# Rikorose/DeepFilterNet

Hardware: NVIDIA H100
Metric: 48kHz audio-sec/sec (batched enhance) (higher is better)
Workload: dtype f32 (bf16x3 tensor-core contractions, fp32 accumulate; DSP and gates IEEE fp32)

## Files before the change

### deepfilternet_b200/csrc/dfb_common.cuh

```cuda
#pragma once
#include <cuda_runtime.h>
#include <stdint.h>

#include <atomic>
#include <cstdarg>
#include <cstdio>
#include <mutex>
#include <string>
#include <vector>

#include "../../include/dfb200.h"

namespace dfb {

extern thread_local std::string g_err;
extern std::atomic<int64_t> g_launches;

inline int fail(int code, const char *fmt, ...) {
    char buf[512];
    va_list ap;
    va_start(ap, fmt);
    vsnprintf(buf, sizeof buf, fmt, ap);
    va_end(ap);
    g_err = buf;
    return code;
}

#define DFB_CUDA(expr)                                                                          \
    do {                                                                                        \
        cudaError_t e__ = (expr);                                                               \
        if (e__ != cudaSuccess)                                                                 \
            return dfb::fail(DFB_ERR_CUDA, "%s failed: %s (%s:%d)", #expr, cudaGetErrorString(e__), \
                             __FILE__, __LINE__);                                               \
    } while (0)

#define DFB_LAUNCH_CHECK()                                                                      \
    do {                                                                                        \
        dfb::g_launches.fetch_add(1, std::memory_order_relaxed);                                \
        cudaError_t e__ = cudaGetLastError();                                                   \
        if (e__ != cudaSuccess)                                                                 \
            return dfb::fail(DFB_ERR_CUDA, "kernel launch failed: %s (%s:%d)",                  \
                             cudaGetErrorString(e__), __FILE__, __LINE__);                      \
    } while (0)

struct ProfScope {
    int slot = -1;
    cudaStream_t s;
    ProfScope(const char *name, cudaStream_t stream);
    ~ProfScope();
};
#define DFB_PROF(name, stream) dfb::ProfScope prof_scope__(name, stream)

struct PerDeviceOnce {
    std::mutex mu;
    std::atomic<unsigned long long> done{0};
    struct Guard {
        std::unique_lock<std::mutex> lk;
        PerDeviceOnce *o = nullptr;
        unsigned long long bit = 0;
        Guard() = default;
        Guard(Guard &&g) noexcept : lk(std::move(g.lk)), o(g.o), bit(g.bit) {}
        explicit operator bool() const { return lk.owns_lock(); }
        ~Guard() { if (lk.owns_lock()) o->done.fetch_or(bit, std::memory_order_release); }
    };
    Guard first() {
        int d = 0;
        cudaGetDevice(&d);
        const unsigned long long bit = 1ull << (d & 63);
        Guard g;
        if (done.load(std::memory_order_acquire) & bit) return g;
        g.lk = std::unique_lock<std::mutex>(mu);
        if (done.load(std::memory_order_acquire) & bit) { g.lk.unlock(); g.lk.release(); return g; }
        g.o = this; g.bit = bit;
        return g;
    }
};

int use_device(int device);

struct Arena {
    char *base = nullptr;
    size_t cap = 0, off = 0;
    int reserve(size_t bytes);
    void reset() { off = 0; }
    template <typename T>
    T *take(size_t n) {
        size_t b = (n * sizeof(T) + 255) & ~size_t(255);
        if (off + b > cap) return nullptr;
        T *p = reinterpret_cast<T *>(base + off);
        off += b;
        return p;
    }
    void release();
};

constexpr int kMaxErb = 64;

struct DspTables {
    const float *window;
    const float2 *tw_a_fwd;
    const float2 *tw_a_inv;
    const float2 *tw960;
    const int *erb_off;
    const float *erb_kinv;
    const unsigned char *band_of_bin;
    float wnorm;
    int fft, hop, F, E;
};

struct RaggedRow { int64_t in_off, len, out_off, out_len, Tf; };

struct ApplyParams {
    const float2 *spec;
    const float *m;
    const float *coefs;
    float *audio;
    float2 *spec_out;
    int64_t out_stride;
    int64_t out_offset;
    int64_t out_len;
    int Tf, mode, nb_df, order, lookahead;
    int spec_T, Tv, t_first;
    int mc_T;
    int frames_per_warp;
    int pf, mask_only;
    float pf_beta;
    const float *lsnr;
    float th_min, th_erb, th_df;
    const float *alpha;
    float atten_lim;
    const float *init_tail;
    float *final_tail;
    int carry;
    const RaggedRow *rows;
    int64_t w0;
    int t_emit;
};

}

struct dfb_state;
namespace dfb {
struct AnaWindow { int t_begin, nf, out_t0, Tbuf; int64_t row_stride; const RaggedRow *rows = nullptr; };
int launch_analysis(dfb_state *st, const float *d_audio, int64_t C, int64_t T, float *d_spec, float *d_erb_db,
                    cudaStream_t s, const float *d_init_mem = nullptr, const AnaWindow *w = nullptr);
int launch_feat_norm(const float *d_erb, int E, int64_t erb_stride, const float *d_spec, int Fd, int64_t spec_stride,
                     int64_t C, int64_t Tf, float alpha, const float *d_erb_state, const float *d_unit_state,
                     float *d_feat_erb, float *d_feat_spec, cudaStream_t s, int64_t Ts = 0, float *d_erb_state_out = nullptr,
                     float *d_unit_state_out = nullptr);
int launch_apply_synthesis(dfb_state *st, const ApplyParams &p, int64_t B, cudaStream_t s);
struct GruWindow { const float *h0; float *hT; int t0, Ts; };
int launch_gru_tc(cudaStream_t s, const float *xproj, const float *whh, const float *bhh, const float *res, float *hout,
                  unsigned short *hout_hi, unsigned short *hout_lo, int B, int T, long long *dbg = nullptr, int wide = 0,
                  int planes_res = 0, const GruWindow *w = nullptr, int H = 256);
int launch_gemm_bf16x3(cudaStream_t s, const void *x_hi, const void *x_lo, int64_t ldx, const void *w_hi, const void *w_lo,
                       const float *bias, float *y, int64_t ldy, int64_t M, int N, int K);
int launch_gl_bx(cudaStream_t s, const unsigned short *x_hi, const unsigned short *x_lo, int64_t ldx, const float *w_img,
                 const float *res, int64_t ldr, float *y, int64_t ldy, unsigned short *y_hi, unsigned short *y_lo, int64_t ldp,
                 int64_t M, int G, int Ig, int Hg, int act, float oscale, float ooffset);
bool gl_bx_geometry(int G, int Ig, int Hg, int *gpc_out, int *hgp_out, int *stages_out);
int launch_df_convp_tc(cudaStream_t s, const float *c0, const float *w_sw, const float *w2, const float *bias, float *coefs, int B, int T,
                       int Fd);
int launch_to_planes(cudaStream_t s, const float *x, int64_t ldx, int64_t M, int K, unsigned short *hi, unsigned short *lo);
}

struct dfb_state {
    int device, sr, fft, hop, nb_erb, min_nb_erb_freqs;
    std::vector<int64_t> erb;
    std::vector<float> window;
    void *d_tables = nullptr;
    dfb::DspTables tb{};
    dfb::Arena arena;
    cudaStream_t stream = nullptr;
    std::vector<float> analysis_mem, synthesis_mem;
};
```

### deepfilternet_b200/csrc/dfb_gl.cu

```cuda
#include <cuda.h>
#include <cuda_bf16.h>

#include <map>
#include <mutex>
#include <tuple>

#include "dfb_common.cuh"
#include "dfb_ptx.cuh"

namespace dfb {

constexpr int kGxThreads = 288, kGxMaxStages = 6, kGxBoxBytes = 128 * 128 ;
constexpr int kGxMaxChunks = 16;

struct GlBxParams {
    const unsigned short *w_img;
    const float *res; int64_t ldr;
    float *y; int64_t ldy;
    unsigned short *y_hi, *y_lo; int64_t ldp;
    int M, G, Ig, Hg, Hgp, gpc, act, stages;
    float oscale, ooffset;
};

__device__ __forceinline__ float gx_act(float x, int act) {
    if (act == 1) return fmaxf(x, 0.f);
    if (act == 2) return gt_tanh(x);
    return x;
}

__device__ __noinline__ void gl_store_chunk(const GlBxParams &p, int c, int g0, int cpg, int64_t mrow, int lane, float a00, float a01,
                                            float a02, float a03, float a10, float a11, float a12, float a13) {
    const float a[2][4] = {{a00, a01, a02, a03}, {a10, a11, a12, a13}};
    const int gl = c / cpg;
#pragma unroll
    for (int j = 0; j < 2; j++) {
        const int n = (c - gl * cpg) * 16 + j * 8 + 2 * (lane & 3);
        if (n >= p.Hg) continue;
        const int64_t col = (int64_t)(g0 + gl) * p.Hg + n;
        float2 rv[2];
#pragma unroll
        for (int h = 0; h < 2; h++) {
            const int64_t m = mrow + 8 * h;
            rv[h] = (p.res && m < p.M) ? *reinterpret_cast<const float2 *>(p.res + m * p.ldr + col) : make_float2(0.f, 0.f);
        }
#pragma unroll
        for (int h = 0; h < 2; h++) {
            const int64_t m = mrow + 8 * h;
            if (m >= p.M) continue;
            float2 x;
            x.x = gx_act(a[j][2 * h], p.act) * p.oscale + p.ooffset + rv[h].x;
            x.y = gx_act(a[j][2 * h + 1], p.act) * p.oscale + p.ooffset + rv[h].y;
            if (p.y) *reinterpret_cast<float2 *>(p.y + m * p.ldy + col) = x;
            if (p.y_hi) {
                uint32_t hv, lv;
                bf16x2_split(x.x, x.y, hv, lv);
                *reinterpret_cast<uint32_t *>(p.y_hi + m * p.ldp + col) = hv;
                *reinterpret_cast<uint32_t *>(p.y_lo + m * p.ldp + col) = lv;
            }
        }
    }
}

__global__ void __launch_bounds__(kGxThreads, 1)
k_gl_bx(const __grid_constant__ CUtensorMap tmXhi, const __grid_constant__ CUtensorMap tmXlo, const __grid_constant__ GlBxParams p) {
    extern __shared__ __align__(1024) unsigned char gx_smem_raw[];
    const uint32_t sb = (smem_u32(gx_smem_raw) + 1023u) & ~1023u;
    const int warp = threadIdx.x >> 5, lane = threadIdx.x & 31;
    const int slice = blockIdx.x, g0 = slice * p.gpc;
    const int nch = p.gpc * p.Hgp / 16;
    const int cpg = p.Hgp / 16;
    const int nboxes = p.gpc * p.Ig / 64;
    const int ntiles = (p.M + 127) / 128;
    const uint32_t gbytes = (uint32_t)p.Ig * p.Hgp * 2;
    const uint32_t wplane = gbytes * p.gpc;
    const uint32_t lbo = (uint32_t)(p.Hgp / 8) * 128u;
    const uint32_t s_x = sb;
    const uint32_t s_w = s_x + (uint32_t)p.stages * 2 * kGxBoxBytes;
    const uint32_t s_bar = (s_w + 2 * wplane + 127u) & ~127u;
    const uint32_t b_full = s_bar, b_empty = s_bar + 8 * kGxMaxStages, b_w = b_empty + 8 * kGxMaxStages;
    if (threadIdx.x == 0) {
        for (int s = 0; s < p.stages; s++) { mbar_init_a(b_full + 8 * s, 1); mbar_init_a(b_empty + 8 * s, 8); }
        mbar_init_a(b_w, 1);
        fence_barrier_init();
        mbar_expect_tx_a(b_w, 2 * wplane);
        const unsigned char *src = reinterpret_cast<const unsigned char *>(p.w_img);
        bulk_load(s_w, src + (size_t)g0 * gbytes, wplane, b_w);
        bulk_load(s_w + wplane, src + (size_t)p.G * gbytes + (size_t)g0 * gbytes, wplane, b_w);
    }
    __syncthreads();
    if (warp == 8) {
        if (lane == 0) {
            tma_prefetch_desc(&tmXhi); tma_prefetch_desc(&tmXlo);
            const int col0 = g0 * p.Ig;
            int it = 0;
            for (int tile = blockIdx.y; tile < ntiles; tile += gridDim.y)
                for (int b = 0; b < nboxes; b++, it++) {
                    const int s = it % p.stages, n = it / p.stages;
                    if (n > 0) mbar_wait_a(b_empty + 8 * s, (uint32_t)((n - 1) & 1));
                    mbar_expect_tx_a(b_full + 8 * s, 2 * kGxBoxBytes);
                    const uint32_t dst = s_x + (uint32_t)s * 2 * kGxBoxBytes;
                    asm volatile(
                        "cp.async.bulk.tensor.2d.shared::cluster.global.mbarrier::complete_tx::bytes [%0], [%1, {%2, %3}], [%4];"
                        ::"r"(dst), "l"((uint64_t)&tmXhi), "r"(col0 + b * 64), "r"(tile * 128), "r"(b_full + 8 * s) : "memory");
                    asm volatile(
                        "cp.async.bulk.tensor.2d.shared::cluster.global.mbarrier::complete_tx::bytes [%0], [%1, {%2, %3}], [%4];"
                        ::"r"(dst + kGxBoxBytes), "l"((uint64_t)&tmXlo), "r"(col0 + b * 64), "r"(tile * 128), "r"(b_full + 8 * s) : "memory");
                }
        }
        return;
    }
    const int mat = lane >> 3, rr = lane & 7;
    mbar_wait_a(b_w, 0);
    int it = 0;
    for (int tile = blockIdx.y; tile < ntiles; tile += gridDim.y) {
        float acc[kGxMaxChunks][2][4];
#pragma unroll
        for (int c = 0; c < kGxMaxChunks; c++)
#pragma unroll
            for (int e = 0; e < 8; e++) acc[c][e >> 2][e & 3] = 0.f;
        for (int b = 0; b < nboxes; b++, it++) {
            const int s = it % p.stages, n = it / p.stages;
            mbar_wait_a(b_full + 8 * s, (uint32_t)(n & 1));
            const uint32_t xs = s_x + (uint32_t)s * 2 * kGxBoxBytes;
#pragma unroll 1
            for (int k = 0; k < 4; k++) {
                const int col = b * 64 + k * 16;
                const int gl = col / p.Ig, kk = (col - gl * p.Ig) >> 4;
                uint32_t ah[4], al[4];
                const int r = warp * 16 + rr + ((mat & 1) << 3);
                ldsm_x4(xs + sw128_off(r, 2 * k + (mat >> 1)), ah);
                ldsm_x4(xs + kGxBoxBytes + sw128_off(r, 2 * k + (mat >> 1)), al);
                const uint32_t wa = s_w + (uint32_t)gl * gbytes + (uint32_t)(2 * kk + (mat & 1)) * lbo + (uint32_t)rr * 16u;
#pragma unroll
                for (int c = 0; c < kGxMaxChunks; c++) {
                    const int cg = c - gl * cpg;
                    if (c >= nch || cg < 0 || cg >= cpg) continue;
                    const uint32_t o = wa + (uint32_t)(2 * cg + (mat >> 1)) * 128u;
                    uint32_t bh[4], bl[4];
                    ldsm_x4(o, bh);
                    ldsm_x4(o + wplane, bl);
                    mma_bf16x3(acc[c][0], ah, al, bh[0], bh[1], bl[0], bl[1]);
                    mma_bf16x3(acc[c][1], ah, al, bh[2], bh[3], bl[2], bl[3]);
                }
            }
            __syncwarp();
            if (lane == 0) mbar_arrive_a(b_empty + 8 * s);
        }
        const int64_t mrow = (int64_t)tile * 128 + warp * 16 + (lane >> 2);
#pragma unroll
        for (int c = 0; c < kGxMaxChunks; c++)
            if (c < nch)
                gl_store_chunk(p, c, g0, cpg, mrow, lane, acc[c][0][0], acc[c][0][1], acc[c][0][2], acc[c][0][3], acc[c][1][0],
                               acc[c][1][1], acc[c][1][2], acc[c][1][3]);
    }
}

__global__ void __launch_bounds__(256) k_to_planes(const float *__restrict__ x, int64_t ldx, int64_t M, int K,
                                                   unsigned short *__restrict__ hi, unsigned short *__restrict__ lo) {
    const int64_t n4 = M * (K / 4);
    for (int64_t i = (int64_t)blockIdx.x * blockDim.x + threadIdx.x; i < n4; i += (int64_t)gridDim.x * blockDim.x) {
        const int64_t m = i / (K / 4);
        const int k = (int)(i - m * (K / 4)) * 4;
        const float4 v = *reinterpret_cast<const float4 *>(x + m * ldx + k);
        uint32_t h0, l0, h1, l1;
        bf16x2_split(v.x, v.y, h0, l0);
        bf16x2_split(v.z, v.w, h1, l1);
        *reinterpret_cast<uint2 *>(hi + m * K + k) = make_uint2(h0, h1);
        *reinterpret_cast<uint2 *>(lo + m * K + k) = make_uint2(l0, l1);
    }
}

typedef CUresult (*PFN_encodeTiled_gl)(CUtensorMap *, CUtensorMapDataType, cuuint32_t, void *, const cuuint64_t *,
                                       const cuuint64_t *, const cuuint32_t *, const cuuint32_t *, CUtensorMapInterleave,
                                       CUtensorMapSwizzle, CUtensorMapL2promotion, CUtensorMapFloatOOBfill);

int cached_map_bf16(CUtensorMap *out, const void *base, int64_t rows, int64_t cols, int64_t ld, int box_rows) {
    static std::mutex mu;
    static std::map<std::tuple<int, const void *, int64_t, int64_t, int64_t, int>, CUtensorMap> cache;
    static PFN_encodeTiled_gl enc = nullptr;
    int dev = 0;
    cudaGetDevice(&dev);
    std::lock_guard<std::mutex> g(mu);
    auto key = std::make_tuple(dev, base, rows, cols, ld, box_rows);
    auto it = cache.find(key);
    if (it != cache.end()) { *out = it->second; return DFB_OK; }
    if (!enc) {
        void *fp = nullptr;
        cudaDriverEntryPointQueryResult q;
        if (cudaGetDriverEntryPoint("cuTensorMapEncodeTiled", &fp, cudaEnableDefault, &q) != cudaSuccess || q != cudaDriverEntryPointSuccess)
            return fail(DFB_ERR_CUDA, "cuTensorMapEncodeTiled entry point not available");
        enc = (PFN_encodeTiled_gl)fp;
    }
    cuuint64_t dims[2] = {(cuuint64_t)cols, (cuuint64_t)rows};
    cuuint64_t strides[1] = {(cuuint64_t)ld * 2};
    cuuint32_t box[2] = {64u, (cuuint32_t)box_rows};
    cuuint32_t estr[2] = {1, 1};
    CUtensorMap m;
    CUresult r = enc(&m, CU_TENSOR_MAP_DATA_TYPE_BFLOAT16, 2, (void *)base, dims, strides, box, estr, CU_TENSOR_MAP_INTERLEAVE_NONE,
                     CU_TENSOR_MAP_SWIZZLE_128B, CU_TENSOR_MAP_L2_PROMOTION_L2_128B, CU_TENSOR_MAP_FLOAT_OOB_FILL_NONE);
    if (r != CUDA_SUCCESS) return fail(DFB_ERR_CUDA, "cuTensorMapEncodeTiled (bf16) failed (%d)", (int)r);
    if (cache.size() > 4096) cache.clear();
    cache[key] = m;
    *out = m;
    return DFB_OK;
}

int cached_map_f32_sw128(CUtensorMap *out, const void *base, int64_t rows, int64_t cols, int64_t ld, int box_rows) {
    static std::mutex mu;
    static std::map<std::tuple<int, const void *, int64_t, int64_t, int64_t, int>, CUtensorMap> cache;
    static PFN_encodeTiled_gl enc = nullptr;
    int dev = 0;
    cudaGetDevice(&dev);
    std::lock_guard<std::mutex> g(mu);
    auto key = std::make_tuple(dev, base, rows, cols, ld, box_rows);
    auto it = cache.find(key);
    if (it != cache.end()) { *out = it->second; return DFB_OK; }
    if (!enc) {
        void *fp = nullptr;
        cudaDriverEntryPointQueryResult q;
        if (cudaGetDriverEntryPoint("cuTensorMapEncodeTiled", &fp, cudaEnableDefault, &q) != cudaSuccess || q != cudaDriverEntryPointSuccess)
            return fail(DFB_ERR_CUDA, "cuTensorMapEncodeTiled entry point not available");
        enc = (PFN_encodeTiled_gl)fp;
    }
    cuuint64_t dims[2] = {(cuuint64_t)cols, (cuuint64_t)rows};
    cuuint64_t strides[1] = {(cuuint64_t)ld * 4};
    cuuint32_t box[2] = {32u, (cuuint32_t)box_rows};
    cuuint32_t estr[2] = {1, 1};
    CUtensorMap m;
    CUresult r = enc(&m, CU_TENSOR_MAP_DATA_TYPE_FLOAT32, 2, (void *)base, dims, strides, box, estr, CU_TENSOR_MAP_INTERLEAVE_NONE,
                     CU_TENSOR_MAP_SWIZZLE_128B, CU_TENSOR_MAP_L2_PROMOTION_L2_128B, CU_TENSOR_MAP_FLOAT_OOB_FILL_NONE);
    if (r != CUDA_SUCCESS) return fail(DFB_ERR_CUDA, "cuTensorMapEncodeTiled (fp32) failed (%d)", (int)r);
    if (cache.size() > 4096) cache.clear();
    cache[key] = m;
    *out = m;
    return DFB_OK;
}

int launch_to_planes(cudaStream_t s, const float *x, int64_t ldx, int64_t M, int K, unsigned short *hi, unsigned short *lo) {
    if (K % 4 || ldx % 4) return fail(DFB_ERR_UNSUPPORTED, "to_planes: K = %d", K);
    int dev = 0, sms = 0;
    DFB_CUDA(cudaGetDevice(&dev));
    DFB_CUDA(cudaDeviceGetAttribute(&sms, cudaDevAttrMultiProcessorCount, dev));
    DFB_PROF("k_to_planes", s);
    k_to_planes<<<sms * 8, 256, 0, s>>>(x, ldx, M, K, hi, lo);
    DFB_LAUNCH_CHECK();
    return DFB_OK;
}

bool gl_bx_geometry(int G, int Ig, int Hg, int *gpc_out, int *hgp_out, int *stages_out) {
    if (Ig % 16 || Hg % 4 || G < 1) return false;
    const int Hgp = (Hg + 15) / 16 * 16;
    if (Hgp > 256) return false;
    int best = 0;
    for (int gpc = 1; gpc <= G; gpc++) {
        if (G % gpc) continue;
        if (gpc * Hgp > 256 || (gpc * Hgp) % 32) continue;
        if ((gpc * Ig) % 64) continue;
        if ((size_t)gpc * Ig * Hgp * 4 > 100 * 1024) continue;
        best = gpc;
    }
    if (!best) return false;
    const int w = best * Ig * Hgp * 4;
    int stages = (227 * 1024 - 2048 - w - 256) / (2 * kGxBoxBytes);
    if (stages > kGxMaxStages) stages = kGxMaxStages;
    if (stages < 2) return false;
    *gpc_out = best; *hgp_out = Hgp; *stages_out = stages;
    return true;
}

int launch_gl_bx(cudaStream_t s, const unsigned short *x_hi, const unsigned short *x_lo, int64_t ldx, const float *w_img,
                 const float *res, int64_t ldr, float *y, int64_t ldy, unsigned short *y_hi, unsigned short *y_lo, int64_t ldp,
                 int64_t M, int G, int Ig, int Hg, int act, float oscale, float ooffset) {
    int gpc = 0, Hgp = 0, stages = 0;
    if (!gl_bx_geometry(G, Ig, Hg, &gpc, &Hgp, &stages) || M <= 0 || M > 0x7fffffff || (ldx % 8) || ((uintptr_t)x_hi & 15) ||
        ((uintptr_t)x_lo & 15) || (y && ((ldy % 4) || ((uintptr_t)y & 15))) || (res && ((ldr % 4) || ((uintptr_t)res & 15))) ||
        (y_hi && ((ldp % 4) || ((uintptr_t)y_hi & 7) || ((uintptr_t)y_lo & 7))))
        return DFB_ERR_UNSUPPORTED;
    CUtensorMap mh, ml;
    int rc;
    if ((rc = cached_map_bf16(&mh, x_hi, M, (int64_t)G * Ig, ldx, 128)) || (rc = cached_map_bf16(&ml, x_lo, M, (int64_t)G * Ig, ldx, 128)))
        return rc;
    GlBxParams p{reinterpret_cast<const unsigned short *>(w_img), res, ldr, y, ldy, y_hi, y_lo, ldp,
                 (int)M, G, Ig, Hg, Hgp, gpc, act, stages, oscale, ooffset};
    const int smem = 1024 + stages * 2 * kGxBoxBytes + gpc * Ig * Hgp * 4 + 128 + 256;
    static PerDeviceOnce attr_once;
    if (auto once_guard = attr_once.first())
        DFB_CUDA(cudaFuncSetAttribute(k_gl_bx, cudaFuncAttributeMaxDynamicSharedMemorySize, 227 * 1024));
    int dev = 0, sms = 0;
    DFB_CUDA(cudaGetDevice(&dev));
    DFB_CUDA(cudaDeviceGetAttribute(&sms, cudaDevAttrMultiProcessorCount, dev));
    const int slices = G / gpc, ntiles = (int)((M + 127) / 128);
    int groups = sms / slices;
    if (groups < 1) groups = 1;
    if (groups > ntiles) groups = ntiles;
    DFB_PROF("k_gl_bx", s);
    k_gl_bx<<<dim3((unsigned)slices, (unsigned)groups), kGxThreads, smem, s>>>(mh, ml, p);
    DFB_LAUNCH_CHECK();
    return DFB_OK;
}

}
```

### deepfilternet_b200/csrc/dfb_model.cu

```cuda
#include <cooperative_groups.h>
#include <cuda_bf16.h>

#include <algorithm>
#include <cmath>
#include <cstring>
#include <functional>
#include <map>
#include <string>

#include "dfb_common.cuh"
#include "dfb_dwpw.cuh"
#include "dfb_ptx.cuh"

namespace cg = cooperative_groups;

namespace dfb {


enum Act { ACT_NONE = 0, ACT_RELU = 1, ACT_TANH = 2, ACT_SIGMOID = 3 };

__device__ __forceinline__ float act_apply(float x, int act) {
    switch (act) {
        case ACT_RELU: return fmaxf(x, 0.f);
        case ACT_TANH: return tanhf(x);
// ... 736 lines not shown
                                int n_tensors, const int64_t *erb_widths) {
    if (!out || !cfg || !tensors) return fail(DFB_ERR_INVALID, "null argument");
    *out = nullptr;
    if (cfg->conv_ch != kCh) return fail(DFB_ERR_UNSUPPORTED, "conv_ch = %d (built kernels: 64)", cfg->conv_ch);
    if (cfg->model_kind < 1 || cfg->model_kind > 3) return fail(DFB_ERR_UNSUPPORTED, "model_kind %d", cfg->model_kind);
    if (cfg->model_kind == 1 && (cfg->emb_hidden != cfg->df_hidden || cfg->emb_hidden != cfg->nb_erb / 4 * kCh || cfg->conv_kt != 2 ||
                                 cfg->inp_kt != 2 || cfg->df_order != 5))
        return fail(DFB_ERR_UNSUPPORTED, "DeepFilterNet v1: only the shipped topology is built (hidden = conv_ch * nb_erb / 4, kt 2, order 5)");
    if (cfg->conv_kt < 1 || cfg->conv_kt > 2 || cfg->inp_kt < 1 || cfg->inp_kt > 3)
        return fail(DFB_ERR_UNSUPPORTED, "conv kernel time taps (%d, %d) unsupported", cfg->conv_kt, cfg->inp_kt);
    if ((cfg->emb_hidden != 256 && cfg->emb_hidden != 512) || (cfg->df_hidden != 256 && cfg->df_hidden != 512))
        return fail(DFB_ERR_UNSUPPORTED, "GRU hidden sizes (%d, %d): built kernels cover 256 and 512", cfg->emb_hidden,
                    cfg->df_hidden);
    if (cfg->nb_erb % 8 || cfg->nb_erb > 64 || cfg->nb_df % 8 || cfg->nb_df > 128 || 2 * cfg->df_order > kMaxO2)
        return fail(DFB_ERR_UNSUPPORTED, "nb_erb / nb_df / df_order outside the built kernels");
    int rc = use_device(device);
    if (rc) return rc;
    dfb_model *m = new dfb_model();
    m->device = device;
    m->cfg = *cfg;
    if (erb_widths) m->erb_widths.assign(erb_widths, erb_widths + cfg->nb_erb);
    if (const char *e = getenv("DFB_DEVICE_CHUNKS")) m->dev_chunks = atoi(e) > 0 ? atoi(e) : 0;
    if (const char *e = getenv("DFB_HOST_CHUNKS")) m->host_chunks = atoi(e) > 0 ? atoi(e) : 1;
    if (const char *e = getenv("DFB_LANES")) m->n_lanes = atoi(e) == 1 ? 1 : 2;
    if (const char *e = getenv("DFB_MAX_WORKSPACE_MB")) {
        const long long mb = atoll(e);
        if (mb > 0) m->max_workspace = (size_t)mb << 20;
    }
    size_t total = 0;
    for (int i = 0; i < n_tensors; i++) total += ((size_t)tensors[i].numel * 4 + 255) & ~size_t(255);
    if (cudaMalloc(&m->slab, total + 256) != cudaSuccess) {
        delete m;
        return fail(DFB_ERR_OOM, "cudaMalloc(%zu) for weights failed", total);
    }
    size_t off = 0;
    std::vector<float> tmp;
    for (int i = 0; i < n_tensors; i++) {
        const dfb_tensor &tt = tensors[i];
        if (!tt.name || !tt.data || tt.numel <= 0) { dfb_model_free(m); return fail(DFB_ERR_INVALID, "bad tensor %d", i); }
        float *dst = (float *)((char *)m->slab + off);
        if (cudaMemcpy(dst, tt.data, (size_t)tt.numel * 4, cudaMemcpyHostToDevice) != cudaSuccess) {
            dfb_model_free(m);
            return fail(DFB_ERR_CUDA, "weight upload failed");
        }
        m->t[tt.name] = {dst, tt.numel};
        off += ((size_t)tt.numel * 4 + 255) & ~size_t(255);
    }
    int prio_least = 0, prio_greatest = 0;
    cudaDeviceGetStreamPriorityRange(&prio_least, &prio_greatest);
    int prio_enc = prio_greatest + 1;
    if (prio_enc > prio_least) prio_enc = prio_least;
    bool ok = cudaStreamCreateWithFlags(&m->stream, cudaStreamNonBlocking) == cudaSuccess &&
              cudaStreamCreateWithFlags(&m->h2d, cudaStreamNonBlocking) == cudaSuccess &&
              cudaStreamCreateWithFlags(&m->d2h, cudaStreamNonBlocking) == cudaSuccess;
    for (auto &L : m->lanes) {
        ok = ok && cudaStreamCreateWithPriority(&L.main, cudaStreamNonBlocking, prio_enc) == cudaSuccess &&
             cudaStreamCreateWithPriority(&L.hi, cudaStreamNonBlocking, prio_enc) == cudaSuccess &&
             cudaStreamCreateWithPriority(&L.aux, cudaStreamNonBlocking, prio_enc) == cudaSuccess &&
             cudaStreamCreateWithPriority(&L.dhi, cudaStreamNonBlocking, prio_greatest) == cudaSuccess &&
             cudaStreamCreateWithPriority(&L.daux, cudaStreamNonBlocking, prio_greatest) == cudaSuccess &&
             cudaStreamCreateWithPriority(&L.low, cudaStreamNonBlocking, prio_least) == cudaSuccess;
        for (cudaEvent_t *e : {&L.ev_fork, &L.ev_join, &L.ev_fork_enc, &L.ev_join_enc, &L.ev_in, &L.ev_out, &L.ev_c0, &L.ev_convp,
                               &L.ev_skip, &L.ev_done})
            ok = ok && cudaEventCreateWithFlags(e, cudaEventDisableTiming) == cudaSuccess;
    }
    if (!ok) {
        dfb_model_free(m);
        return fail(DFB_ERR_CUDA, "stream creation failed");
    }
    *out = m;
    return DFB_OK;
}

extern "C" void dfb_model_free(dfb_model *m) {
    if (!m) return;
    cudaSetDevice(m->device);
    m->arena.release();
    m->arena1.release();
    m->aux_arena.release();
    if (m->h2d) cudaStreamDestroy(m->h2d);
    if (m->d2h) cudaStreamDestroy(m->d2h);
    if (m->slab) cudaFree(m->slab);
    if (m->stream) cudaStreamDestroy(m->stream);
    for (auto &L : m->lanes) {
        for (cudaStream_t st : {L.main, L.hi, L.aux, L.dhi, L.daux, L.low})
            if (st) cudaStreamDestroy(st);
        for (cudaEvent_t e : {L.ev_fork, L.ev_join, L.ev_fork_enc, L.ev_join_enc, L.ev_in, L.ev_out, L.ev_c0, L.ev_convp, L.ev_skip, L.ev_done})
            if (e) cudaEventDestroy(e);
    }
    delete m;
}

extern "C" int dfb_debug_gru_timing(dfb_model *m, int steps, long long *h_out) {
    if (!m) return fail(DFB_ERR_INVALID, "null model");
    cudaSetDevice(m->device);
    if (h_out && m->gru_dbg) {
        DFB_CUDA(cudaDeviceSynchronize());
        DFB_CUDA(cudaMemcpy(h_out, m->gru_dbg, sizeof(long long) * 8 * steps, cudaMemcpyDeviceToHost));
    }
    if (m->gru_dbg) { cudaFree(m->gru_dbg); m->gru_dbg = nullptr; }
    if (steps > 0 && !h_out) {
        DFB_CUDA(cudaMalloc(&m->gru_dbg, sizeof(long long) * 8 * steps));
        DFB_CUDA(cudaMemset(m->gru_dbg, 0, sizeof(long long) * 8 * steps));
    }
    return DFB_OK;
}

extern "C" int dfb_model_set_precision(dfb_model *m, int mode) {
    if (!m || mode < 0 || mode > 15 || (mode & 1)) return fail(DFB_ERR_INVALID, "precision mode out of range (bit 0 is reserved)");
    m->gru_tc = (mode >> 1) & 1;
    m->proj_tc = (mode >> 2) & 1;
    m->conv_tc = (mode >> 3) & 1;
    return DFB_OK;
}

extern "C" int64_t dfb_model_debug_fetch(dfb_model *m, const char *name, float *h_out, int64_t max_numel) {
    if (!m || !name || !h_out) return fail(DFB_ERR_INVALID, "null argument");
    auto it = m->dbg.find(name);
    if (it == m->dbg.end()) return fail(DFB_ERR_INVALID, "no activation named '%s'", name);
    int64_t n = it->second.second < max_numel ? it->second.second : max_numel;
    cudaSetDevice(m->device);
    if (cudaDeviceSynchronize() != cudaSuccess ||
        cudaMemcpy(h_out, it->second.first, (size_t)n * 4, cudaMemcpyDeviceToHost) != cudaSuccess)
        return fail(DFB_ERR_CUDA, "debug fetch failed: %s", cudaGetErrorString(cudaGetLastError()));
    return n;
}

extern "C" int64_t dfb_model_workspace_bytes(const dfb_model *m) { return m ? (int64_t)m->arena.cap : 0; }

namespace {

int run_gl(cudaStream_t s, const float *x, int64_t ldx, const float *w, const float *bias, const float *res,
           int64_t ldr, float *y, int64_t ldy, int64_t M, int G, int I, int Hh, int act, float oscale = 1.f,
           float ooffset = 0.f, unsigned short *y_hi = nullptr, unsigned short *y_lo = nullptr) {
    GlParams p{x, ldx, w, bias, res, ldr, y, ldy, M, G, I / G, Hh / G, act, oscale, ooffset, y_hi, y_lo};
    if ((p.Ig % 4) || (ldx % 4)) return fail(DFB_ERR_UNSUPPORTED, "grouped linear: K not a multiple of 4");
    if (G > 1 && (p.Hg % 4)) return fail(DFB_ERR_UNSUPPORTED, "grouped linear: group width %d not a multiple of 4", p.Hg);
    int tiles = (p.Hg + kGlBN - 1) / kGlBN;
    int gpc = (p.Hg < kGlBN && kGlBN % p.Hg == 0) ? (kGlBN / p.Hg < G ? kGlBN / p.Hg : G) : 1;
    dim3 grid((unsigned)((M + kGlBM - 1) / kGlBM), (unsigned)(((G + gpc - 1) / gpc) * tiles));
    static const bool detail = getenv("DFB_PROF_DETAIL") && atoi(getenv("DFB_PROF_DETAIL"));
    char name[64];
    if (detail) snprintf(name, sizeof name, "k_grouped_linear[%dx%d/%d]", I, Hh, G);
    else snprintf(name, sizeof name, "%s", p.G == 1 && p.bias && p.Hg >= 512 ? "k_grouped_linear[gru_proj]" : "k_grouped_linear");
    DFB_PROF(name, s);
    k_grouped_linear<<<grid, 256, 0, s>>>(p);
    DFB_LAUNCH_CHECK();
    return DFB_OK;
}

template <int H, int C>
int launch_gru_t(cudaStream_t s, const GruParams &p, int ngroups) {
    constexpr int smem = (2 * kGruMaxBc * (H + 4) + 3 * (H / C) * (kGruMaxBc + 1)) * 4;
    static PerDeviceOnce attr_once;
    if (auto once_guard = attr_once.first()) {
        if (C > 8) DFB_CUDA(cudaFuncSetAttribute(k_gru<H, C>, cudaFuncAttributeNonPortableClusterSizeAllowed, 1));
        DFB_CUDA(cudaFuncSetAttribute(k_gru<H, C>, cudaFuncAttributeMaxDynamicSharedMemorySize, smem));
    }
    cudaLaunchConfig_t cfg{};
    cfg.gridDim = dim3((unsigned)(ngroups * C));
    cfg.blockDim = dim3(kGruThreads);
    cfg.dynamicSmemBytes = smem;
    cfg.stream = s;
    cudaLaunchAttribute at[1];
    at[0].id = cudaLaunchAttributeClusterDimension;
    at[0].val.clusterDim.x = C; at[0].val.clusterDim.y = 1; at[0].val.clusterDim.z = 1;
    cfg.attrs = at; cfg.numAttrs = 1;
    GruParams pp = p;
    DFB_PROF("k_gru", s);
    DFB_CUDA(cudaLaunchKernelEx(&cfg, k_gru<H, C>, pp));
    g_launches.fetch_add(1, std::memory_order_relaxed);
    return DFB_OK;
}

int pick_bc(int B, int max_clusters) {
    int bc = (B + max_clusters - 1) / max_clusters;
    bc = ((bc + kGruSB - 1) / kGruSB) * kGruSB;
    if (bc < kGruSB) bc = kGruSB;
    if (bc > kGruMaxBc) bc = kGruMaxBc;
    return bc;
}

int run_gru(dfb_model *m, cudaStream_t s, const char *name, int layers, int H, const float *x, int in_dim,
            const float *res_last, float *y, float *xproj, float *tmp_h, int B, int T,
            unsigned short *x_hi = nullptr, unsigned short *x_lo = nullptr, unsigned short *pl_hi = nullptr,
            unsigned short *pl_lo = nullptr, int wide = 0, unsigned short *out_hi = nullptr, unsigned short *out_lo = nullptr,
            bool *out_planes_ok = nullptr, const GruChunk *ck = nullptr) {
    if (out_planes_ok) *out_planes_ok = false;
    const int t0 = ck ? ck->t0 : 0, Tn = T - t0;
    const int64_t M = (int64_t)B * T;
    const float *cur_in = x;
    int cur_dim = in_dim;
    const bool tc_gru = m->gru_tc && (H == 256 || H == 512);
    const bool tc_proj = m->proj_tc && tc_gru && x_hi && pl_hi && cur_dim % 64 == 0;
    const unsigned short *cur_hi = x_hi, *cur_lo = x_lo;
    for (int l = 0; l < layers; l++) {
        std::string base = std::string(name) + ".l" + std::to_string(l);
        const float *w_ih_t, *w_hh, *b_ih, *b_hh;
        int rc;
        if ((rc = need(m, (base + ".w_ih_t").c_str(), (int64_t)3 * H * cur_dim, &w_ih_t))) return rc;
        if ((rc = need(m, (base + ".w_hh").c_str(), (int64_t)3 * H * H, &w_hh))) return rc;
        if ((rc = need(m, (base + ".b_ih").c_str(), 3 * H, &b_ih))) return rc;
        if ((rc = need(m, (base + ".b_hh").c_str(), 3 * H, &b_hh))) return rc;
        if (tc_proj) {
            const float *w_hi, *w_lo;
            if ((rc = need(m, (base + ".w_ih_hi").c_str(), (int64_t)3 * H * cur_dim / 2, &w_hi)) ||
                (rc = need(m, (base + ".w_ih_lo").c_str(), (int64_t)3 * H * cur_dim / 2, &w_lo)))
                return rc;
            rc = launch_gemm_bf16x3(s, cur_hi, cur_lo, cur_dim, w_hi, w_lo, b_ih, xproj, 3 * H, M, 3 * H, cur_dim);
        } else {
            rc = run_gl(s, cur_in, cur_dim, w_ih_t, b_ih, nullptr, 0, xproj, 3 * H, M, 1, cur_dim, 3 * H, ACT_NONE);
        }
        if (rc) return rc;
        float *dst = (l == layers - 1) ? y : tmp_h;
        float *hs = ck && ck->h ? ck->h + (int64_t)l * ck->Bs * H : nullptr;
        GruWindow gw{ck && ck->have_state ? hs : nullptr, hs, t0, T};
        GruParams p{xproj, w_hh, b_hh, (l == layers - 1) ? res_last : nullptr, dst, B, Tn, 0, m->gru_dbg, gw.h0, gw.hT, t0, T};
        if (tc_gru) {
            const bool last = l == layers - 1;
            const bool planes = last ? out_hi != nullptr : tc_proj;
            rc = launch_gru_tc(s, xproj, w_hh, b_hh, last ? res_last : nullptr, dst, planes ? (last ? out_hi : pl_hi) : nullptr,
                               planes ? (last ? out_lo : pl_lo) : nullptr, B, Tn, m->gru_dbg, wide, last ? 1 : 0, &gw, H);
            if (last && planes && out_planes_ok) *out_planes_ok = true;
            cur_hi = pl_hi; cur_lo = pl_lo;
        } else if (H == 256) {
            int sms = 0;
            DFB_CUDA(cudaDeviceGetAttribute(&sms, cudaDevAttrMultiProcessorCount, m->device));
            p.Bc = pick_bc(B, sms / 4);
            rc = launch_gru_t<256, 4>(s, p, (B + p.Bc - 1) / p.Bc);
        } else {
            p.Bc = pick_bc(B, 8);
            rc = launch_gru_t<512, 16>(s, p, (B + p.Bc - 1) / p.Bc);
        }
        if (rc) return rc;
        cur_in = dst;
        cur_dim = H;
    }
    return DFB_OK;
}

}
namespace dfb {
template <int MODE>
int launch_dwpw_tc(cudaStream_t s, DwPwParams p, const float *w_sw, int B);
}
namespace {

template <int MODE>
int run_dwpw(cudaStream_t s, DwPwParams p, int B, const float *w_sw = nullptr) {
    if (w_sw) return launch_dwpw_tc<MODE>(s, p, w_sw, B);
    static PerDeviceOnce attr_once;
    const int smem = (kCh * kCh + 128 * kLdA) * 4;
    if (auto once_guard = attr_once.first()) {
        DFB_CUDA(cudaFuncSetAttribute(k_dwpw<MODE>, cudaFuncAttributeMaxDynamicSharedMemorySize, smem));
    }
    p.NF = 128 / p.Fout;
    if (p.NF < 1) p.NF = 1;
    if (p.NF * p.Fout > 128 || (p.NF * p.Fout) % 4) return fail(DFB_ERR_UNSUPPORTED, "dwpw tile: Fout = %d", p.Fout);
    dim3 grid((unsigned)((p.T + p.NF - 1) / p.NF), (unsigned)B);
    DFB_PROF(MODE == DW_DF0 ? "k_dwpw[df_conv0]" : "k_dwpw", s);
    k_dwpw<MODE><<<grid, 256, smem, s>>>(p);
    DFB_LAUNCH_CHECK();
    return DFB_OK;
}

}

struct FwdBufs {
    float *e0, *e1, *e2, *e3, *c0, *c1, *emb_in, *emb, *g_a, *g_b, *g_h, *xproj, *dec_emb, *d3, *d2, *d1, *dfc;
    unsigned short *ga_hi, *ga_lo, *gh_hi, *gh_lo;
    float *g_a2, *g_h2, *xproj2, *dfskip;
    unsigned short *ga2_hi, *ga2_lo, *gh2_hi, *gh2_lo;
    unsigned short *c1_hi, *c1_lo, *embin_hi, *embin_lo, *gb_hi, *gb_lo, *emb_hi, *emb_lo, *dfc_hi, *dfc_lo;
};

struct FwdBufsV1 {
    float *e0, *e1, *e2, *e3, *c0, *c1, *c1g, *cemb, *emb, *xproj, *xproj2, *y[3], *embo, *dec_old, *dec, *p3, *p2, *p1, *p0, *d3, *d2, *d1,
        *z[2], *dfc;
    unsigned short *emb_hi, *emb_lo, *y_hi[3], *y_lo[3], *embo_hi, *embo_lo, *z_hi[2], *z_lo[2], *dfc_hi, *dfc_lo, *scr_hi, *scr_lo;
};
static size_t fwd_plan_v1(const dfb_model_config &c, size_t M, Arena *a, FwdBufsV1 *f) {
    const int E = c.nb_erb, Fd = c.nb_df, H = c.emb_hidden;
    size_t bytes = 0;
    auto take = [&](size_t n) -> float * {
        bytes += (n * 4 + 255) & ~size_t(255);
        return a ? a->take<float>(n) : nullptr;
    };
    auto take16 = [&](size_t n) { return reinterpret_cast<unsigned short *>(take((n + 1) / 2)); };
    FwdBufsV1 t{};
    t.e0 = take(M * E * kCh); t.e1 = take(M * (E / 2) * kCh); t.e2 = take(M * (E / 4) * kCh); t.e3 = take(M * (E / 4) * kCh);
    t.c0 = take(M * Fd * kCh); t.c1 = take(M * (Fd / 2) * kCh); t.c1g = take(M * (Fd / 2) * kCh);
    t.cemb = take(M * H); t.emb = take(M * H); t.xproj = take(M * 3 * H); t.xproj2 = take(M * 3 * H);
    for (int i = 0; i < 3; i++) { t.y[i] = take(M * H); t.y_hi[i] = take16(M * H); t.y_lo[i] = take16(M * H); }
    for (int i = 0; i < 2; i++) { t.z[i] = take(M * H); t.z_hi[i] = take16(M * H); t.z_lo[i] = take16(M * H); }
    t.embo = take(M * H); t.dec_old = take(M * H); t.dec = take(M * H); t.dfc = take(M * H);
    t.p3 = take(M * (E / 4) * kCh); t.p2 = take(M * (E / 4) * kCh); t.p1 = take(M * (E / 2) * kCh); t.p0 = take(M * E * kCh);
    t.d3 = take(M * (E / 4) * kCh); t.d2 = take(M * (E / 2) * kCh); t.d1 = take(M * E * kCh);
    t.emb_hi = take16(M * H); t.emb_lo = take16(M * H); t.embo_hi = take16(M * H); t.embo_lo = take16(M * H);
    t.dfc_hi = take16(M * H); t.dfc_lo = take16(M * H); t.scr_hi = take16(M * H); t.scr_lo = take16(M * H);
    if (f) *f = t;
    return bytes + 4096;
}

static size_t fwd_plan(const dfb_model_config &c, size_t M, Arena *a, FwdBufs *f) {
    if (c.model_kind == 1 && !a) return fwd_plan_v1(c, M, nullptr, nullptr);
    const int E = c.nb_erb, Fd = c.nb_df, H = c.emb_hidden, Hd = c.df_hidden;
    const int ED = E / 4 * kCh;
    const int emb_in_dim = c.enc_concat ? 2 * ED : ED;
    const int emb_dim = c.model_kind == 2 ? H : ED;
    const int Hmax = H > Hd ? H : Hd;
    size_t bytes = 0;
    auto take = [&](size_t n) -> float * {
        bytes += (n * 4 + 255) & ~size_t(255);
        return a ? a->take<float>(n) : nullptr;
    };
    FwdBufs t{};
    t.e0 = take(M * E * kCh); t.e1 = take(M * (E / 2) * kCh); t.e2 = take(M * (E / 4) * kCh);
    t.emb_in = take(M * emb_in_dim);
    t.e3 = c.enc_concat ? t.emb_in : take(M * ED);
    t.c0 = take(M * Fd * kCh); t.c1 = take(M * (Fd / 2) * kCh);
    t.emb = take(M * emb_dim);
    t.g_a = take(M * Hmax); t.g_b = take(M * Hmax); t.g_h = take(M * Hmax);
    t.xproj = take(M * 3 * Hmax);
    t.dec_emb = take(M * ED); t.d3 = take(M * ED); t.d2 = take(M * (E / 2) * kCh);
    t.d1 = take(M * E * kCh); t.dfc = take(M * Hmax);
    t.ga_hi = reinterpret_cast<unsigned short *>(take(M * Hmax / 2)); t.ga_lo = reinterpret_cast<unsigned short *>(take(M * Hmax / 2));
    t.gh_hi = reinterpret_cast<unsigned short *>(take(M * Hmax / 2)); t.gh_lo = reinterpret_cast<unsigned short *>(take(M * Hmax / 2));
    t.g_a2 = take(M * Hmax); t.g_h2 = take(M * Hmax); t.xproj2 = take(M * 3 * Hmax); t.dfskip = take(M * Hmax);
    t.ga2_hi = reinterpret_cast<unsigned short *>(take(M * Hmax / 2)); t.ga2_lo = reinterpret_cast<unsigned short *>(take(M * Hmax / 2));
    t.gh2_hi = reinterpret_cast<unsigned short *>(take(M * Hmax / 2)); t.gh2_lo = reinterpret_cast<unsigned short *>(take(M * Hmax / 2));
    auto take16 = [&](size_t n) { return reinterpret_cast<unsigned short *>(take((n + 1) / 2)); };
    t.c1_hi = take16(M * (Fd / 2) * kCh); t.c1_lo = take16(M * (Fd / 2) * kCh);
    t.embin_hi = take16(M * emb_in_dim); t.embin_lo = take16(M * emb_in_dim);
    t.gb_hi = take16(M * Hmax); t.gb_lo = take16(M * Hmax);
    t.emb_hi = take16(M * emb_dim); t.emb_lo = take16(M * emb_dim);
    t.dfc_hi = take16(M * Hmax); t.dfc_lo = take16(M * Hmax);
    if (f) *f = t;
    return bytes + 4096;
}

struct ChunkCtx {
    int Rc;
    int Tsx, Tx;
    float *h_enc, *h_erb, *h_df;
    bool have_state;
    float *dec_tail;
    int dec_tail_n;
    int lane;
    cudaEvent_t wait_dec;
    int Bs;
    const RaggedRow *rows;
    int64_t W0;
};
constexpr int kHalo = 8;

static int forward_impl(dfb_model *m, Arena &arena, const float *d_feat_erb, const float *d_feat_spec, int B, int T,
                        float *d_m, float *d_coefs, float *d_lsnr, float *d_alpha, cudaStream_t s, ChunkCtx *cx = nullptr);

extern "C" int dfb_model_forward(dfb_model *m, const float *d_feat_erb, const float *d_feat_spec, int64_t B64,
                                 int64_t T64, float *d_m, float *d_coefs, float *d_lsnr, float *d_alpha,
                                 void *stream) {
    if (!m || !d_feat_erb || !d_feat_spec || !d_m || !d_coefs) return fail(DFB_ERR_INVALID, "null argument");
    if (B64 <= 0 || T64 <= 0) return DFB_OK;
    if (B64 > 65535) return fail(DFB_ERR_INVALID, "more than 65535 streams per call");
    DFB_CUDA(cudaSetDevice(m->device));
    int rc = m->arena.reserve(fwd_plan(m->cfg, (size_t)B64 * T64, nullptr, nullptr));
    if (rc) return rc;
    m->arena.reset();
    rc = forward_impl(m, m->arena, d_feat_erb, d_feat_spec, (int)B64, (int)T64, d_m, d_coefs, d_lsnr, d_alpha,
                      (cudaStream_t)stream);
    m->arena.reset();
    return rc;
}

static int forward_body(dfb_model *m, Arena &arena, const float *d_feat_erb, const float *d_feat_spec, int B, int T,
                        float *d_m, float *d_coefs, float *d_lsnr, float *d_alpha, cudaStream_t s_in, ChunkCtx *cx);

static int forward_v1(dfb_model *m, Arena &arena, const float *d_feat_erb, const float *d_feat_spec, int B, int T,
                      float *d_m, float *d_coefs, float *d_lsnr, float *d_alpha, cudaStream_t s_in, ChunkCtx *cx);

static int forward_impl(dfb_model *m, Arena &arena, const float *d_feat_erb, const float *d_feat_spec, int B, int T,
                        float *d_m, float *d_coefs, float *d_lsnr, float *d_alpha, cudaStream_t s_in, ChunkCtx *cx) {
    const int rc = m->cfg.model_kind == 1
        ? forward_v1(m, arena, d_feat_erb, d_feat_spec, B, T, d_m, d_coefs, d_lsnr, d_alpha, s_in, cx)
        : forward_body(m, arena, d_feat_erb, d_feat_spec, B, T, d_m, d_coefs, d_lsnr, d_alpha, s_in, cx);
    if (rc) cudaDeviceSynchronize();
    return rc;
}

static int forward_body(dfb_model *m, Arena &arena, const float *d_feat_erb, const float *d_feat_spec, int B, int T,
                        float *d_m, float *d_coefs, float *d_lsnr, float *d_alpha, cudaStream_t s_in, ChunkCtx *cx) {
    const dfb_model_config &c = m->cfg;
    const int Tsx = cx ? cx->Tsx : T, Tx = cx ? cx->Tx : T;
    GruChunk ck_enc{cx ? cx->h_enc : nullptr, cx && cx->have_state, cx ? cx->Rc : 0, cx ? cx->Bs : B};
    GruChunk ck_erb{cx ? cx->h_erb : nullptr, cx && cx->have_state, cx ? cx->Rc : 0, cx ? cx->Bs : B};
    GruChunk ck_df{cx ? cx->h_df : nullptr, cx && cx->have_state, cx ? cx->Rc : 0, cx ? cx->Bs : B};
    const RaggedRow *rows = cx ? cx->rows : nullptr;
    const int64_t W0 = cx ? cx->W0 : 0;
    static const bool serial = getenv("DFB_SERIAL") && atoi(getenv("DFB_SERIAL"));
    dfb_model::Lane &L = m->lanes[cx ? cx->lane : 0];
    cudaStream_t s = serial ? s_in : L.hi;
    cudaStream_t sl = serial ? s_in : L.low;
    if (!serial) {
        DFB_CUDA(cudaEventRecord(L.ev_in, s_in));
        DFB_CUDA(cudaStreamWaitEvent(s, L.ev_in, 0));
    }
    auto finish = [&]() -> int {
        DFB_CUDA(cudaStreamWaitEvent(s, L.ev_join, 0));
        if (!serial) {
            DFB_CUDA(cudaEventRecord(L.ev_out, s));
            DFB_CUDA(cudaStreamWaitEvent(s_in, L.ev_out, 0));
        }
        return DFB_OK;
    };
    const int64_t M = (int64_t)B * T;
    const int E = c.nb_erb, Fd = c.nb_df, H = c.emb_hidden, Hd = c.df_hidden;
    const int ED = E / 4 * kCh;
    const int emb_in_dim = c.enc_concat ? 2 * ED : ED;
    const int emb_dim = c.model_kind == 2 ? H : ED;
    int rc;
    FwdBufs f{};
    fwd_plan(c, (size_t)M, &arena, &f);
    if (!f.gh2_lo || !f.dfskip || !f.dfc_lo) return fail(DFB_ERR_OOM, "forward workspace exhausted for %lld frames", (long long)M);
    m->dbg.clear();
    m->dbg["e0"] = {f.e0, M * E * kCh}; m->dbg["e1"] = {f.e1, M * (E / 2) * kCh}; m->dbg["e2"] = {f.e2, M * (E / 4) * kCh};
    m->dbg["e3"] = {f.e3, c.enc_concat ? M * emb_in_dim : M * ED}; m->dbg["c0"] = {f.c0, M * Fd * kCh};
    m->dbg["c1"] = {f.c1, M * (Fd / 2) * kCh}; m->dbg["emb_in"] = {f.emb_in, M * emb_in_dim};
    m->dbg["emb"] = {f.emb, M * emb_dim}; m->dbg["dec_emb"] = {f.dec_emb, M * ED}; m->dbg["d3"] = {f.d3, M * ED};
    m->dbg["d2"] = {f.d2, M * (E / 2) * kCh}; m->dbg["d1"] = {f.d1, M * E * kCh}; m->dbg["dfc"] = {f.dfc, M * Hd};
    m->dbg["g_a"] = {f.g_a, M * (H > Hd ? H : Hd)}; m->dbg["g_b"] = {f.g_b, M * (H > Hd ? H : Hd)};
    m->dbg["xproj"] = {f.xproj, M * 3 * (H > Hd ? H : Hd)};
    const int64_t e3_fs = c.enc_concat ? 2 * ED : ED;
    struct Pl { unsigned short *hi, *lo; int64_t ld; bool ok; };
    Pl pl_c1{f.c1_hi, f.c1_lo, (int64_t)Fd / 2 * kCh, false}, pl_embin{f.embin_hi, f.embin_lo, emb_in_dim, false},
       pl_gb{f.gb_hi, f.gb_lo, H, false}, pl_emb{f.emb_hi, f.emb_lo, emb_dim, false}, pl_dfc{f.dfc_hi, f.dfc_lo, Hd, false},
       pl_ga{f.ga_hi, f.ga_lo, H, false}, pl_ga2{f.ga2_hi, f.ga2_lo, Hd, false};
    const bool gl_tc = m->conv_tc != 0;
    auto ensure_planes = [&](cudaStream_t st, const float *x, int64_t ldx, int K, Pl &pl) -> int {
        if (pl.ok) return DFB_OK;
        if (pl.ld != K) return fail(DFB_ERR_INVALID, "plane pitch mismatch");
        int r = launch_to_planes(st, x, ldx, M, K, pl.hi, pl.lo);
        if (!r) pl.ok = true;
        return r;
    };
    auto gl = [&](cudaStream_t st, const char *wname, const float *x, int64_t ldx, Pl *xin, int G, int I, int Hh, int act,
                  const float *res, int64_t ldr, float *y, int64_t ldy, Pl *yout, int64_t ycol = 0) -> int {
        const float *w;
        int r;
        if ((r = need(m, wname, (int64_t)I * Hh / G, &w))) return r;
        unsigned short *yh = yout ? yout->hi + ycol : nullptr, *yl = yout ? yout->lo + ycol : nullptr;
        const std::string bx = std::string(wname) + "_bx";
        int gpc, hgp, stages;
        if (gl_tc && xin && m->get(bx) && gl_bx_geometry(G, I / G, Hh / G, &gpc, &hgp, &stages)) {
            if ((r = ensure_planes(st, x, ldx, I, *xin))) return r;
            r = launch_gl_bx(st, xin->hi, xin->lo, xin->ld, m->get(bx), res, ldr, y, ldy, yh, yl, yout ? yout->ld : 0, M, G, I / G,
                             Hh / G, act, 1.f, 0.f);
            if (r != DFB_ERR_UNSUPPORTED) {
                if (!r && yout && (ycol == 0 || true)) yout->ok = true;
                return r;
            }
        }
        const bool ffma_planes = yout && yout->ld == ldy;
        r = run_gl(st, x, ldx, w, nullptr, res, ldr, y, ldy, M, G, I, Hh, act, 1.f, 0.f, ffma_planes ? yh : nullptr, ffma_planes ? yl : nullptr);
        if (!r && yout) yout->ok = ffma_planes;
        return r;
    };

    {
        const float *w, *bb;
        if ((rc = need(m, "enc.erb_conv0.w", c.inp_kt * 3 * kCh, &w)) || (rc = need(m, "enc.erb_conv0.b", kCh, &bb))) return rc;
        dim3 grid((unsigned)((T + kInFrames - 1) / kInFrames), (unsigned)B);
        int smem = (kInFrames + c.inp_kt - 1) * (E + 2) * 4;
        DFB_PROF("k_conv_in[erb_conv0]", s);
        k_conv_in<1><<<grid, 256, smem, s>>>(d_feat_erb, w, bb, f.e0, T, E, c.inp_kt, c.conv_lookahead, Tsx, Tx, 0, rows, W0);
        DFB_LAUNCH_CHECK();
    }
    const float *pw_sw = nullptr;
    auto blk = [&](const char *name, DwPwParams &p) -> int {
        std::string n(name);
        int r;
        if ((r = need(m, (n + ".dw").c_str(), -1, &p.dw)) || (r = need(m, (n + ".pw").c_str(), kCh * kCh, &p.pw)) ||
            (r = need(m, (n + ".b").c_str(), kCh, &p.bias)))
            return r;
        pw_sw = nullptr;
        if (m->conv_tc && (r = need(m, (n + ".pw_sw").c_str(), kCh * kCh, &pw_sw))) return r;
        return DFB_OK;
    };
    cudaStream_t sa = serial ? s : L.aux;
    DFB_CUDA(cudaEventRecord(L.ev_fork_enc, s));
    DFB_CUDA(cudaStreamWaitEvent(sa, L.ev_fork_enc, 0));
    auto mk = [&](const float *in, int Fin, int64_t in_fs, float *out, int Fout, int64_t out_fs, int kt) {
        DwPwParams p{};
        p.in = in; p.Fin = Fin; p.in_fs = in_fs; p.out = out; p.Fout = Fout; p.out_fs = out_fs; p.kt = kt; p.T = T;
        p.lookahead = 0;
        return p;
    };
    {
        DwPwParams p{};
        {
            const float *w, *bb;
            if ((rc = need(m, "enc.df_conv0.w", c.inp_kt * 3 * 2 * kCh, &w)) || (rc = need(m, "enc.df_conv0.b", kCh, &bb))) return rc;
            dim3 grid((unsigned)((T + kInFrames - 1) / kInFrames), (unsigned)B);
            int smem = (kInFrames + c.inp_kt - 1) * (Fd + 2) * 2 * 4;
            DFB_PROF("k_conv_in[df_conv0]", sa);
            k_conv_in<2><<<grid, 256, smem, sa>>>(d_feat_spec, w, bb, f.c0, T, Fd, c.inp_kt, c.conv_lookahead, Tsx, Tx, 0, rows, W0);
            DFB_LAUNCH_CHECK();
            DFB_CUDA(cudaEventRecord(L.ev_c0, sa));
        }
        p = mk(f.c0, Fd, (int64_t)Fd * kCh, f.c1, Fd / 2, (int64_t)Fd / 2 * kCh, c.conv_kt);
        if ((rc = blk("enc.df_conv1", p))) return rc;
        if (pw_sw && gl_tc) {
            p.out = nullptr; p.out_hi = pl_c1.hi; p.out_lo = pl_c1.lo; pl_c1.ok = true;
            m->dbg.erase("c1");
        }
        if ((rc = run_dwpw<DW_S2>(sa, p, B, pw_sw))) return rc;
        DFB_CUDA(cudaEventRecord(L.ev_join_enc, sa));
        DFB_CUDA(cudaStreamWaitEvent(sl, L.ev_c0, 0));
        const int O2 = 2 * c.df_order;
        const float *w1, *w2, *bb;
        if ((rc = need(m, "df_dec.df_convp.w1", (int64_t)c.df_pathway_kt * O2 * (kCh / 2), &w1)) ||
            (rc = need(m, "df_dec.df_convp.w2", O2 * O2, &w2)) || (rc = need(m, "df_dec.df_convp.b", O2, &bb)))
            return rc;
        if (c.df_order != 5 || c.df_pathway_kt != 5)
            return fail(DFB_ERR_UNSUPPORTED, "df_order %d / df_pathway_kernel_size_t %d (built kernels: 5, 5)", c.df_order,
                        c.df_pathway_kt);
        if (Fd % 2) return fail(DFB_ERR_UNSUPPORTED, "df pathway conv: odd nb_df");
        dim3 grid((unsigned)((Fd + 2 * kCpWarps - 1) / (2 * kCpWarps)), (unsigned)((T + kCpChunk - 1) / kCpChunk), (unsigned)B);
        static const bool convp_ffma = getenv("DFB_CONVP_FFMA") && atoi(getenv("DFB_CONVP_FFMA"));
        const float *w_sw = (m->conv_tc && !convp_ffma) ? m->get("df_dec.df_convp.w_sw") : nullptr;
        if (w_sw) {
            if ((rc = launch_df_convp_tc(sl, f.c0, w_sw, w2, bb, d_coefs, B, T, Fd))) return rc;
        } else {
            DFB_PROF("k_df_convp", sl);
            const int smem = kCpWarps * kCpSlots * (512 + 8);
            k_df_convp<5, 5, 3><<<grid, 32 * kCpWarps, smem, sl>>>(f.c0, w1, w2, bb, d_coefs, T, Fd);
            DFB_LAUNCH_CHECK();
        }
        DFB_CUDA(cudaEventRecord(L.ev_convp, sl));
    }
    {
        DwPwParams p = mk(f.e0, E, (int64_t)E * kCh, f.e1, E / 2, (int64_t)E / 2 * kCh, c.conv_kt);
        if ((rc = blk("enc.erb_conv1", p)) || (rc = run_dwpw<DW_S2>(s, p, B, pw_sw))) return rc;
        p = mk(f.e1, E / 2, (int64_t)E / 2 * kCh, f.e2, E / 4, (int64_t)E / 4 * kCh, c.conv_kt);
        if ((rc = blk("enc.erb_conv2", p)) || (rc = run_dwpw<DW_S2>(s, p, B, pw_sw))) return rc;
        p = mk(f.e2, E / 4, (int64_t)E / 4 * kCh, f.e3, E / 4, e3_fs, c.conv_kt);
        if ((rc = blk("enc.erb_conv3", p))) return rc;
        if (pw_sw && gl_tc && c.enc_concat) { p.out_hi = pl_embin.hi; p.out_lo = pl_embin.lo; }
        if ((rc = run_dwpw<DW_S1>(s, p, B, pw_sw))) return rc;

    }
    DFB_CUDA(cudaStreamWaitEvent(s, L.ev_join_enc, 0));
    {
        const int I = Fd / 2 * kCh;
        const bool e3_planes = pw_sw && gl_tc && c.enc_concat;
        if (c.enc_concat) {
            rc = gl(s, "enc.df_fc_emb.gl", f.c1, I, &pl_c1, c.g_df_fc_emb, I, ED, ACT_RELU, nullptr, 0, f.emb_in + ED, emb_in_dim,
                    &pl_embin, ED);
            pl_embin.ok = pl_embin.ok && e3_planes;
        } else {
            rc = gl(s, "enc.df_fc_emb.gl", f.c1, I, &pl_c1, c.g_df_fc_emb, I, ED, ACT_RELU, f.e3, ED, f.emb_in, emb_in_dim, &pl_embin);
        }
        if (rc) return rc;
    }
    {
        if ((rc = gl(s, "enc.emb_gru.in.gl", f.emb_in, emb_in_dim, &pl_embin, c.g_enc_in, emb_in_dim, H, ACT_RELU, nullptr, 0, f.g_a, H,
                     &pl_ga))) return rc;
        float *gout = c.g_enc_out ? f.g_b : f.emb;
        Pl &pl_gout = c.g_enc_out ? pl_gb : pl_emb;
        if ((rc = run_gru(m, s, "enc.emb_gru", c.enc_gru_layers, H, f.g_a, H, nullptr, gout, f.xproj, f.g_h, B, T, f.ga_hi, f.ga_lo,
                          f.gh_hi, f.gh_lo, 0, gl_tc ? pl_gout.hi : nullptr, gl_tc ? pl_gout.lo : nullptr, &pl_gout.ok, cx ? &ck_enc : nullptr))) return rc;
        if (c.g_enc_out) {
            if ((rc = gl(s, "enc.emb_gru.out.gl", f.g_b, H, &pl_gb, c.g_enc_out, H, ED, ACT_RELU, nullptr, 0, f.emb, emb_dim, &pl_emb)))
                return rc;
        }
        if (gl_tc && (rc = ensure_planes(s, f.emb, emb_dim, emb_dim, pl_emb))) return rc;
        if (d_lsnr) {
            const float *lw, *lb;
            if ((rc = need(m, "enc.lsnr.w", emb_dim, &lw)) || (rc = need(m, "enc.lsnr.b", 1, &lb))) return rc;
            if ((rc = run_gl(s, f.emb, emb_dim, lw, lb, nullptr, 0, d_lsnr, 1, M, 1, emb_dim, 1, ACT_SIGMOID, c.lsnr_scale, c.lsnr_offset))) return rc;
        }
    }
    DFB_CUDA(cudaEventRecord(L.ev_fork, s));
    if (!serial) { s = L.dhi; sa = L.daux; DFB_CUDA(cudaStreamWaitEvent(s, L.ev_fork, 0)); }
    DFB_CUDA(cudaStreamWaitEvent(sa, L.ev_fork, 0));
    if (cx && cx->wait_dec) {
        DFB_CUDA(cudaStreamWaitEvent(s, cx->wait_dec, 0));
        DFB_CUDA(cudaStreamWaitEvent(sa, cx->wait_dec, 0));
    }
    static const char *wide_env = getenv("DFB_WIDE_BRANCH");
    const int wide_df = !wide_env || !strcmp(wide_env, "df") || !strcmp(wide_env, "both");
    const int wide_erb = wide_env && (!strcmp(wide_env, "erb") || !strcmp(wide_env, "both"));
    const bool early_skip = c.g_df_skip && c.model_kind != 2;
    if (early_skip) {
        if ((rc = gl(s, "df_dec.df_skip.gl", f.emb, emb_dim, &pl_emb, c.g_df_skip, emb_dim, Hd, ACT_NONE, nullptr, 0, f.dfskip, Hd, nullptr)))
            return rc;
        DFB_CUDA(cudaEventRecord(L.ev_skip, s));
    }
    {
        cudaStream_t s = sa;
        if ((rc = gl(s, "df_dec.df_gru.in.gl", f.emb, emb_dim, &pl_emb, c.g_df_in, emb_dim, Hd, ACT_RELU, nullptr, 0, f.g_a2, Hd, &pl_ga2)))
            return rc;
        const float *res = c.model_kind == 2 ? f.g_a2 : (early_skip ? f.dfskip : nullptr);
        if (early_skip) DFB_CUDA(cudaStreamWaitEvent(s, L.ev_skip, 0));
        if ((rc = run_gru(m, s, "df_dec.df_gru", c.df_gru_layers, Hd, f.g_a2, Hd, res, f.dfc, f.xproj2, f.g_h2, B, T, f.ga2_hi, f.ga2_lo,
                          f.gh2_hi, f.gh2_lo, wide_df, gl_tc ? pl_dfc.hi : nullptr, gl_tc ? pl_dfc.lo : nullptr, &pl_dfc.ok, cx ? &ck_df : nullptr))) return rc;
        if (c.g_df_skip && !early_skip) {
            if ((rc = gl(s, "df_dec.df_skip.gl", f.emb, emb_dim, &pl_emb, c.g_df_skip, emb_dim, Hd, ACT_NONE, f.dfc, Hd, f.dfc, Hd, nullptr)))
                return rc;
            pl_dfc.ok = false;
        }
        if (d_alpha && c.model_kind == 2) {
            const float *aw, *ab;
            if ((rc = need(m, "df_dec.df_fc_a.w", Hd, &aw)) || (rc = need(m, "df_dec.df_fc_a.b", 1, &ab))) return rc;
            if ((rc = run_gl(s, f.dfc, Hd, aw, ab, nullptr, 0, d_alpha, 1, M, 1, Hd, 1, ACT_SIGMOID))) return rc;
        }
        const int O2 = 2 * c.df_order;
        DFB_CUDA(cudaStreamWaitEvent(s, L.ev_convp, 0));
        if ((rc = gl(s, "df_dec.df_out.gl", f.dfc, Hd, &pl_dfc, c.g_df_out, Hd, Fd * O2, ACT_TANH, d_coefs, (int64_t)Fd * O2, d_coefs,
                     (int64_t)Fd * O2, nullptr))) return rc;
    }
    DFB_CUDA(cudaEventRecord(L.ev_join, sa));
    {
        if ((rc = gl(s, "erb_dec.emb_gru.in.gl", f.emb, emb_dim, &pl_emb, c.g_erb_in, emb_dim, H, ACT_RELU, nullptr, 0, f.g_a, H, &pl_ga)))
            return rc;
        const float *res = c.model_kind == 2 ? f.g_a : nullptr;
        pl_gb.ok = false;
        if ((rc = run_gru(m, s, "erb_dec.emb_gru", c.erb_gru_layers, H, f.g_a, H, res, f.g_b, f.xproj, f.g_h, B, T, f.ga_hi, f.ga_lo,
                          f.gh_hi, f.gh_lo, wide_erb, gl_tc ? pl_gb.hi : nullptr, gl_tc ? pl_gb.lo : nullptr, &pl_gb.ok, cx ? &ck_erb : nullptr))) return rc;
        if ((rc = gl(s, "erb_dec.emb_gru.out.gl", f.g_b, H, &pl_gb, c.g_erb_out, H, ED, ACT_RELU, nullptr, 0, f.dec_emb, ED, nullptr)))
            return rc;
        if (cx && cx->dec_tail && c.conv_kt > 1) {
            const size_t fb = sizeof(float) * ED;
            const int nl = cx->Rc < cx->dec_tail_n ? cx->Rc : cx->dec_tail_n;
            if (cx->have_state && nl > 0)
                DFB_CUDA(cudaMemcpy2DAsync(f.dec_emb + (size_t)(cx->Rc - nl) * ED, fb * T, cx->dec_tail + (size_t)(kHalo - nl) * ED,
                                           fb * kHalo, fb * nl, B, cudaMemcpyDeviceToDevice, s));
            const int ns = T < kHalo ? T : kHalo;
            DFB_CUDA(cudaMemcpy2DAsync(cx->dec_tail + (size_t)(kHalo - ns) * ED, fb * kHalo, f.dec_emb + (size_t)(T - ns) * ED, fb * T,
                                       fb * ns, B, cudaMemcpyDeviceToDevice, s));
            cx->dec_tail_n = ns;
        }
        auto path = [&](DwPwParams &p, const char *pn, const float *pt, int64_t pfs) -> int {
            std::string n(pn);
            p.path = pt; p.path_fs = pfs;
            int r;
            if ((r = need(m, (n + ".s").c_str(), kCh, &p.ps)) || (r = need(m, (n + ".b").c_str(), kCh, &p.pb))) return r;
            return DFB_OK;
        };
        DwPwParams p = mk(f.dec_emb, E / 4, ED, f.d3, E / 4, ED, c.conv_kt);
        if ((rc = blk("erb_dec.convt3", p)) || (rc = path(p, "erb_dec.conv3p", f.e3, e3_fs)) || (rc = run_dwpw<DW_S1>(s, p, B, pw_sw))) return rc;
        p = mk(f.d3, E / 4, ED, f.d2, E / 2, (int64_t)E / 2 * kCh, 1);
        if ((rc = blk("erb_dec.convt2", p)) || (rc = path(p, "erb_dec.conv2p", f.e2, (int64_t)E / 4 * kCh)) || (rc = run_dwpw<DW_T2>(s, p, B, pw_sw))) return rc;
        const float *ps, *pb, *w, *bb;
        if ((rc = need(m, "erb_dec.conv0p.s", kCh, &ps)) || (rc = need(m, "erb_dec.conv0p.b", kCh, &pb)) ||
            (rc = need(m, "erb_dec.conv0_out.w", c.conv_kt * 3 * kCh, &w)) || (rc = need(m, "erb_dec.conv0_out.b", 1, &bb)))
            return rc;
        p = mk(f.d2, E / 2, (int64_t)E / 2 * kCh, f.d1, E, (int64_t)E * kCh, 1);
        if ((rc = blk("erb_dec.convt1", p)) || (rc = path(p, "erb_dec.conv1p", f.e1, (int64_t)E / 2 * kCh))) return rc;
        const bool fused_mask = pw_sw && c.conv_kt == 1 && 128 % E == 0;
        if (fused_mask) {
            p.mk_e0 = f.e0; p.mk_ps = ps; p.mk_pb = pb; p.mk_w = w; p.mk_bias = bb; p.mk_out = d_m;
            p.out = nullptr;
            m->dbg.erase("d1");
        }
        if ((rc = run_dwpw<DW_T2>(s, p, B, pw_sw))) return rc;
        if (fused_mask) return finish();
        static PerDeviceOnce attr_once;
        int smem = (kMaskWarps * 2 * (E + 2) * kMaskLd + c.conv_kt * 3 * kCh) * 4;
        if (auto once_guard = attr_once.first()) {
            DFB_CUDA(cudaFuncSetAttribute(k_mask_out, cudaFuncAttributeMaxDynamicSharedMemorySize,
                                          (kMaskWarps * 2 * (64 + 2) * kMaskLd + 2 * 3 * kCh) * 4));
        }
        int per_cta = kMaskWarps * kMaskChunk;
        dim3 grid((unsigned)((T + per_cta - 1) / per_cta), (unsigned)B);
        DFB_PROF("k_mask_out", s);
        k_mask_out<<<grid, 32 * kMaskWarps, smem, s>>>(f.e0, f.d1, ps, pb, w, bb, d_m, T, E, c.conv_kt);
        DFB_LAUNCH_CHECK();
    }
    return finish();
}

static int forward_v1(dfb_model *m, Arena &arena, const float *d_feat_erb, const float *d_feat_spec, int B, int T,
                      float *d_m, float *d_coefs, float *d_lsnr, float *d_alpha, cudaStream_t s_in, ChunkCtx *cx) {
    const dfb_model_config &c = m->cfg;
    if (cx && (cx->Rc != 0 || cx->have_state)) return fail(DFB_ERR_UNSUPPORTED, "DeepFilterNet v1 runs as one window per signal");
    const int Tsx = cx ? cx->Tsx : T, Tx = cx ? cx->Tx : T;
    static const bool serial = getenv("DFB_SERIAL") && atoi(getenv("DFB_SERIAL"));
    dfb_model::Lane &L = m->lanes[cx ? cx->lane : 0];
    cudaStream_t s = serial ? s_in : L.hi, sa = serial ? s_in : L.aux;
    if (!serial) {
        DFB_CUDA(cudaEventRecord(L.ev_in, s_in));
        DFB_CUDA(cudaStreamWaitEvent(s, L.ev_in, 0));
    }
    const int64_t M = (int64_t)B * T;
    const int E = c.nb_erb, Fd = c.nb_df, H = c.emb_hidden, O2 = 2 * c.df_order, kt = c.conv_kt;
    int rc;
    FwdBufsV1 f{};
    fwd_plan_v1(c, (size_t)M, &arena, &f);
    if (!f.scr_lo) return fail(DFB_ERR_OOM, "forward workspace exhausted for %lld frames", (long long)M);
    m->dbg.clear();
    m->dbg["e0"] = {f.e0, M * E * kCh}; m->dbg["e1"] = {f.e1, M * (E / 2) * kCh}; m->dbg["e2"] = {f.e2, M * (E / 4) * kCh};
    m->dbg["e3"] = {f.e3, M * (E / 4) * kCh}; m->dbg["c0"] = {f.c0, M * Fd * kCh}; m->dbg["c1"] = {f.c1, M * (Fd / 2) * kCh};
    m->dbg["cemb"] = {f.cemb, M * H}; m->dbg["emb_in"] = {f.emb, M * H}; m->dbg["emb"] = {f.embo, M * H};
    m->dbg["dec_emb"] = {f.dec, M * H}; m->dbg["d3"] = {f.d3, M * (E / 4) * kCh}; m->dbg["d2"] = {f.d2, M * (E / 2) * kCh};
    m->dbg["d1"] = {f.d1, M * E * kCh}; m->dbg["dfc"] = {f.dfc, M * H}; m->dbg["y0"] = {f.y[0], M * H};
    const bool tc = m->conv_tc != 0;
    const float *ones, *zeros;
    if ((rc = need(m, "v1.ones", kCh, &ones)) || (rc = need(m, "v1.zeros", kCh, &zeros))) return rc;
    auto table = [&](const char *name, int n, const int **out) -> int {
        const float *t;
        int r = need(m, name, n, &t);
        *out = reinterpret_cast<const int *>(t);
        return r;
    };
    const int *idx_c1, *idx_e3, *idx_shuf, *idx_id, *idx_dec, *idx_gshuf;
    if ((rc = table("v1.idx_c1", Fd / 2 * kCh, &idx_c1)) || (rc = table("v1.idx_e3", H, &idx_e3)) || (rc = table("v1.idx_shuf", H, &idx_shuf)) ||
        (rc = table("v1.idx_id", H, &idx_id)) || (rc = table("v1.idx_dec", H, &idx_dec)) || (rc = table("v1.idx_gshuf", H, &idx_gshuf)))
        return rc;
    auto gather = [&](cudaStream_t st, int n, const float *const *src, const int64_t *ld, const int *const *idx, int K, int relu,
                      float *out, unsigned short *hi, unsigned short *lo) -> int {
        GatherParams g{};
        for (int i = 0; i < n; i++) { g.src[i] = src[i]; g.ld[i] = ld[i]; g.idx[i] = idx[i]; }
        g.n = n; g.out = out; g.ldo = K; g.hi = hi; g.lo = lo; g.ldp = K; g.K = K; g.relu = relu;
        DFB_PROF("k_gather_sum", st);
        k_gather_sum<<<(unsigned)M, 256, 0, st>>>(g);
        DFB_LAUNCH_CHECK();
        return DFB_OK;
    };
    auto block = [&](cudaStream_t st, const char *name, int mode, const float *in, int Fin, float *out, int Fout, int bkt, int la,
                     const float *path) -> int {
        DwPwParams p{};
        std::string n(name);
        int r;
        if ((r = need(m, (n + ".dw").c_str(), bkt * 3 * kCh, &p.dw)) || (r = need(m, (n + ".pw").c_str(), kCh * kCh, &p.pw)) ||
            (r = need(m, (n + ".b").c_str(), kCh, &p.bias)))
            return r;
        p.in = in; p.Fin = Fin; p.in_fs = (int64_t)Fin * kCh; p.out = out; p.Fout = Fout; p.out_fs = (int64_t)Fout * kCh; p.kt = bkt; p.T = T;
        p.lookahead = la;
        if (path) { p.path = path; p.path_fs = p.in_fs; p.ps = ones; p.pb = zeros; }
        const float *w_sw = nullptr;
        if (tc && la == 0 && !(mode == DW_T2 && bkt != 1) && (r = need(m, (n + ".pw_sw").c_str(), kCh * kCh, &w_sw))) return r;
        if (mode == DW_S1) return run_dwpw<DW_S1>(st, p, B, w_sw);
        if (mode == DW_S2) return run_dwpw<DW_S2>(st, p, B, w_sw);
        return run_dwpw<DW_T2>(st, p, B, w_sw);
    };
    DFB_CUDA(cudaEventRecord(L.ev_fork_enc, s));
    DFB_CUDA(cudaStreamWaitEvent(sa, L.ev_fork_enc, 0));
    {
        const float *w, *bb;
        if ((rc = need(m, "enc.erb_conv0.w", c.inp_kt * 3 * kCh, &w)) || (rc = need(m, "enc.erb_conv0.b", kCh, &bb))) return rc;
        dim3 grid((unsigned)((T + kInFrames - 1) / kInFrames), (unsigned)B);
        const int la = c.conv_lookahead > 0 ? 1 : 0;
        {
            DFB_PROF("k_conv_in[erb_conv0]", s);
            k_conv_in<1><<<grid, 256, (kInFrames + c.inp_kt - 1) * (E + 2) * 4, s>>>(d_feat_erb, w, bb, f.e0, T, E, c.inp_kt, la, Tsx, Tx, -la,
                                                                                      nullptr, 0);
            DFB_LAUNCH_CHECK();
        }
        if ((rc = need(m, "enc.df_conv0.w", c.inp_kt * 3 * 2 * kCh, &w)) || (rc = need(m, "enc.df_conv0.b", kCh, &bb))) return rc;
        DFB_PROF("k_conv_in[df_conv0]", sa);
        k_conv_in<2><<<grid, 256, (kInFrames + c.inp_kt - 1) * (Fd + 2) * 2 * 4, sa>>>(d_feat_spec, w, bb, f.c0, T, Fd, c.inp_kt, c.conv_lookahead,
                                                                                      Tsx, Tx, -c.conv_lookahead, nullptr, 0);
        DFB_LAUNCH_CHECK();
    }
    if ((rc = block(sa, "enc.df_conv1", DW_S2, f.c0, Fd, f.c1, Fd / 2, kt, 0, nullptr))) return rc;
    {
        const float *src[1] = {f.c1}; const int64_t ld[1] = {(int64_t)Fd / 2 * kCh}; const int *ix[1] = {idx_c1};
        if ((rc = gather(sa, 1, src, ld, ix, Fd / 2 * kCh, 0, f.c1g, nullptr, nullptr))) return rc;
        const float *w, *bb;
        const int I = Fd / 2 * kCh;
        if ((rc = need(m, "enc.df_fc_emb.gl", (int64_t)I * H / c.g_df_fc_emb, &w)) || (rc = need(m, "enc.df_fc_emb.bias", H, &bb))) return rc;
        if ((rc = run_gl(sa, f.c1g, I, w, bb, nullptr, 0, f.cemb, H, M, c.g_df_fc_emb, I, H, ACT_NONE))) return rc;
    }
    DFB_CUDA(cudaEventRecord(L.ev_join_enc, sa));
    if ((rc = block(s, "enc.erb_conv1", DW_S2, f.e0, E, f.e1, E / 2, kt, c.conv_lookahead > 1 ? 1 : 0, nullptr)) ||
        (rc = block(s, "enc.erb_conv2", DW_S2, f.e1, E / 2, f.e2, E / 4, kt, c.conv_lookahead > 2 ? 1 : 0, nullptr)) ||
        (rc = block(s, "enc.erb_conv3", DW_S1, f.e2, E / 4, f.e3, E / 4, kt, 0, nullptr)))
        return rc;
    DFB_CUDA(cudaStreamWaitEvent(s, L.ev_join_enc, 0));
    {
        const float *src[2] = {f.e3, f.cemb}; const int64_t ld[2] = {H, H}; const int *ix[2] = {idx_e3, idx_shuf};
        if ((rc = gather(s, 2, src, ld, ix, H, 0, f.emb, f.emb_hi, f.emb_lo))) return rc;
    }
    auto ggru = [&](cudaStream_t st, const char *name, int layers, const float *x, unsigned short *x_hi, unsigned short *x_lo, float **y,
                    unsigned short **y_hi, unsigned short **y_lo, float *xproj, float *hbase, float *out, unsigned short *out_hi,
                    unsigned short *out_lo) -> int {
        const float *cur = x;
        unsigned short *ch = x_hi, *cl = x_lo;
        for (int l = 0; l < layers; l++) {
            const std::string nm = std::string(name) + ".g" + std::to_string(l);
            GruChunk ck{hbase ? hbase + (int64_t)l * B * H : nullptr, false, 0, B};
            bool ok = false;
            int r = run_gru(m, st, nm.c_str(), 1, H, cur, H, nullptr, y[l], xproj, nullptr, B, T, ch, cl, f.scr_hi, f.scr_lo, 0, y_hi[l], y_lo[l], &ok,
                            hbase ? &ck : nullptr);
            if (r) return r;
            cur = y[l]; ch = y_hi[l]; cl = y_lo[l];
        }
        const float *src[3]; int64_t ld[3]; const int *ix[3];
        for (int l = 0; l < layers; l++) { src[l] = y[l]; ld[l] = H; ix[l] = l == layers - 1 ? idx_id : idx_gshuf; }
        return gather(st, layers, src, ld, ix, H, 0, out, out_hi, out_lo);
    };
    if (c.enc_gru_layers > 3 || c.df_gru_layers > 2) return fail(DFB_ERR_UNSUPPORTED, "DeepFilterNet v1: more GRU layers than built (3 / 2)");
    if ((rc = ggru(s, "enc.emb_gru", c.enc_gru_layers, f.emb, f.emb_hi, f.emb_lo, f.y, f.y_hi, f.y_lo, f.xproj, cx ? cx->h_enc : nullptr, f.embo,
                   f.embo_hi, f.embo_lo)))
        return rc;
    if (d_lsnr) {
        const float *lw, *lb;
        if ((rc = need(m, "enc.lsnr.w", H, &lw)) || (rc = need(m, "enc.lsnr.b", 1, &lb))) return rc;
        if ((rc = run_gl(s, f.embo, H, lw, lb, nullptr, 0, d_lsnr, 1, M, 1, H, 1, ACT_SIGMOID, c.lsnr_scale, c.lsnr_offset))) return rc;
    }
    DFB_CUDA(cudaEventRecord(L.ev_fork, s));
    if (!serial) { s = L.dhi; sa = L.daux; DFB_CUDA(cudaStreamWaitEvent(s, L.ev_fork, 0)); }
    DFB_CUDA(cudaStreamWaitEvent(sa, L.ev_fork, 0));
    {
        if ((rc = ggru(sa, "df_dec.df_gru", c.df_gru_layers, f.embo, f.embo_hi, f.embo_lo, f.z, f.z_hi, f.z_lo, f.xproj2, cx ? cx->h_df : nullptr, f.dfc,
                       f.dfc_hi, f.dfc_lo)))
            return rc;
        if (d_alpha) {
            const float *aw, *ab;
            if ((rc = need(m, "df_dec.df_fc_a.w", H, &aw)) || (rc = need(m, "df_dec.df_fc_a.b", 1, &ab))) return rc;
            if ((rc = run_gl(sa, f.dfc, H, aw, ab, nullptr, 0, d_alpha, 1, M, 1, H, 1, ACT_SIGMOID))) return rc;
        }
        const float *w_t, *bb, *w_hi, *w_lo;
        const int N = Fd * O2;
        if ((rc = need(m, "df_dec.df_fc_out.w_t", (int64_t)H * N, &w_t)) || (rc = need(m, "df_dec.df_fc_out.b", N, &bb))) return rc;
        rc = DFB_ERR_UNSUPPORTED;
        if (m->proj_tc && m->get("df_dec.df_fc_out.w_hi")) {
            if ((rc = need(m, "df_dec.df_fc_out.w_hi", (int64_t)H * N / 2, &w_hi)) || (rc = need(m, "df_dec.df_fc_out.w_lo", (int64_t)H * N / 2, &w_lo))) return rc;
            rc = launch_gemm_bf16x3(sa, f.dfc_hi, f.dfc_lo, H, w_hi, w_lo, bb, d_coefs, N, M, N, H);
        }
        if (rc == DFB_ERR_UNSUPPORTED) rc = run_gl(sa, f.dfc, H, w_t, bb, nullptr, 0, d_coefs, N, M, 1, H, N, ACT_NONE);
        if (rc) return rc;
        const float *pw, *pb;
        if ((rc = need(m, "df_dec.df_convp.w", kCh * O2, &pw)) || (rc = need(m, "df_dec.df_convp.b", O2, &pb))) return rc;
        const long long rows = (long long)M * Fd;
        DFB_PROF("k_convp_v1", sa);
        k_convp_v1<10><<<(unsigned)((rows + 127) / 128), 128, 0, sa>>>(f.c0, pw, pb, d_coefs, rows);
        DFB_LAUNCH_CHECK();
    }
    DFB_CUDA(cudaEventRecord(L.ev_join, sa));
    {
        const float *w, *bb;
        if ((rc = need(m, "erb_dec.fc_emb.gl", (int64_t)H * H / c.g_erb_in, &w)) || (rc = need(m, "erb_dec.fc_emb.bias", H, &bb))) return rc;
        if ((rc = run_gl(s, f.embo, H, w, bb, nullptr, 0, f.dec_old, H, M, c.g_erb_in, H, H, ACT_RELU))) return rc;
        const float *src[1] = {f.dec_old}; const int64_t ld[1] = {H}; const int *ix[1] = {idx_dec};
        if ((rc = gather(s, 1, src, ld, ix, H, 0, f.dec, nullptr, nullptr))) return rc;
        if ((rc = block(s, "erb_dec.conv3p", DW_S1, f.e3, E / 4, f.p3, E / 4, 1, 0, nullptr)) ||
            (rc = block(s, "erb_dec.conv2p", DW_S1, f.e2, E / 4, f.p2, E / 4, 1, 0, nullptr)) ||
            (rc = block(s, "erb_dec.conv1p", DW_S1, f.e1, E / 2, f.p1, E / 2, 1, 0, nullptr)) ||
            (rc = block(s, "erb_dec.conv0p", DW_S1, f.e0, E, f.p0, E, 1, 0, nullptr)))
            return rc;
        if ((rc = block(s, "erb_dec.convt3", DW_S1, f.dec, E / 4, f.d3, E / 4, kt, 0, f.p3)) ||
            (rc = block(s, "erb_dec.convt2", DW_T2, f.d3, E / 4, f.d2, E / 2, kt, 0, f.p2)) ||
            (rc = block(s, "erb_dec.convt1", DW_T2, f.d2, E / 2, f.d1, E, kt, 0, f.p1)))
            return rc;
        if ((rc = need(m, "erb_dec.conv0_out.w", kt * 3 * kCh, &w)) || (rc = need(m, "erb_dec.conv0_out.b", 1, &bb))) return rc;
        static PerDeviceOnce attr_once;
        const int smem = (kMaskWarps * 2 * (E + 2) * kMaskLd + kt * 3 * kCh) * 4;
        if (auto once_guard = attr_once.first()) {
            DFB_CUDA(cudaFuncSetAttribute(k_mask_out, cudaFuncAttributeMaxDynamicSharedMemorySize, (kMaskWarps * 2 * (64 + 2) * kMaskLd + 2 * 3 * kCh) * 4));
        }
        const int per_cta = kMaskWarps * kMaskChunk;
        dim3 grid((unsigned)((T + per_cta - 1) / per_cta), (unsigned)B);
        DFB_PROF("k_mask_out", s);
        k_mask_out<<<grid, 32 * kMaskWarps, smem, s>>>(f.p0, f.d1, ones, zeros, w, bb, d_m, T, E, kt);
        DFB_LAUNCH_CHECK();
    }
    DFB_CUDA(cudaStreamWaitEvent(s, L.ev_join, 0));
    if (!serial) {
        DFB_CUDA(cudaEventRecord(L.ev_out, s));
        DFB_CUDA(cudaStreamWaitEvent(s_in, L.ev_out, 0));
    }
    return DFB_OK;
}

extern "C" int dfb_model_set_chunking(dfb_model *m, int device_chunks, int host_chunks, int lanes) {
    if (!m || device_chunks < 0 || host_chunks < 1 || lanes < 1 || lanes > 2) return fail(DFB_ERR_INVALID, "bad chunking parameters");
    m->dev_chunks = device_chunks; m->host_chunks = host_chunks; m->n_lanes = lanes;
    return DFB_OK;
}

static int check_state(const dfb_model *m, const dfb_state *st) {
    if (m->device != st->device) return fail(DFB_ERR_INVALID, "model and state live on different devices");
    if (st->tb.E != m->cfg.nb_erb)
        return fail(DFB_ERR_INVALID, "DF state has %d ERB bands, the model was built for %d", st->tb.E, m->cfg.nb_erb);
    if (!m->erb_widths.empty())
        for (int i = 0; i < m->cfg.nb_erb; i++)
            if (m->erb_widths[i] != st->erb[i])
                return fail(DFB_ERR_INVALID, "DF state's ERB band %d is %lld bins wide, the model was built for %lld", i,
                            (long long)st->erb[i], (long long)m->erb_widths[i]);
    return DFB_OK;
}

static int apply_mode(const dfb_model *m) { return m->cfg.model_kind == 3 ? 1 : 2; }
static void apply_options(const dfb_model *m, dfb::ApplyParams &p) {
    p.pf = m->post_filter; p.pf_beta = m->pf_beta; p.mask_only = m->mask_only;
}

extern "C" int dfb_model_set_options(dfb_model *m, int post_filter, float pf_beta, int mask_only) {
    if (!m) return fail(DFB_ERR_INVALID, "null model");
    m->post_filter = post_filter ? 1 : 0;
    m->pf_beta = pf_beta;
    m->mask_only = mask_only ? 1 : 0;
    return DFB_OK;
}

static int apply_impl(dfb_model *m, dfb_state *st, const float *d_spec, const float *d_m, const float *d_coefs, const float *d_alpha,
                      int64_t B, int64_t T, float *d_spec_e, void *stream);
extern "C" int dfb_apply(dfb_model *m, dfb_state *st, const float *d_spec, const float *d_m, const float *d_coefs,
                         int64_t B, int64_t T, float *d_spec_e, void *stream) {
    if (m && m->cfg.model_kind == 1 && !m->mask_only)
        return fail(DFB_ERR_UNSUPPORTED, "DeepFilterNet v1 blends with df_alpha: use dfb_model_forward_full / dfb_enhance");
    return apply_impl(m, st, d_spec, d_m, d_coefs, nullptr, B, T, d_spec_e, stream);
}
static int apply_impl(dfb_model *m, dfb_state *st, const float *d_spec, const float *d_m, const float *d_coefs, const float *d_alpha,
                      int64_t B, int64_t T, float *d_spec_e, void *stream) {
    if (!m || !st || !d_spec || !d_m || !d_coefs || !d_spec_e) return fail(DFB_ERR_INVALID, "null argument");
    if (int rcs = check_state(m, st)) return rcs;
    DFB_CUDA(cudaSetDevice(m->device));
    dfb::ApplyParams p{};
    p.spec = (const float2 *)d_spec; p.m = d_m; p.coefs = d_coefs; p.audio = nullptr; p.spec_out = (float2 *)d_spec_e;
    p.Tf = (int)T; p.mode = apply_mode(m); p.nb_df = m->cfg.nb_df; p.order = m->cfg.df_order; p.lookahead = m->cfg.df_lookahead;
    p.alpha = d_alpha;
    apply_options(m, p);
    return launch_apply_synthesis(st, p, B, (cudaStream_t)stream);
}

extern "C" int dfb_model_forward_full(dfb_model *m, dfb_state *st, const float *d_spec, const float *d_feat_erb,
                                      const float *d_feat_spec, int64_t B, int64_t T, float *d_spec_e, float *d_m,
                                      float *d_lsnr, float *d_coefs, float *d_alpha, void *stream) {
    if (!m || !st || !d_spec || !d_feat_erb || !d_feat_spec || !d_spec_e) return fail(DFB_ERR_INVALID, "null argument");
    if (int rcs = check_state(m, st)) return rcs;
    DFB_CUDA(cudaSetDevice(m->device));
    const int64_t M = B * T;
    const int O2 = 2 * m->cfg.df_order;
    if (B <= 0 || T <= 0) return DFB_OK;
    if (B > 65535) return fail(DFB_ERR_INVALID, "more than 65535 streams per call");
    size_t extra = ((size_t)M * m->cfg.nb_erb + (size_t)M * m->cfg.nb_df * O2 + (size_t)M) * 4 + 8192;
    int rc = m->arena.reserve(fwd_plan(m->cfg, (size_t)M, nullptr, nullptr) + extra);
    if (rc) return rc;
    m->arena.reset();
    float *mm = d_m ? d_m : m->arena.take<float>((size_t)M * m->cfg.nb_erb);
    float *cc = d_coefs ? d_coefs : m->arena.take<float>((size_t)M * m->cfg.nb_df * O2);
    float *aa = d_alpha;
    if (!aa && m->cfg.model_kind == 1) aa = m->arena.take<float>((size_t)M);
    rc = forward_impl(m, m->arena, d_feat_erb, d_feat_spec, (int)B, (int)T, mm, cc, d_lsnr, aa, (cudaStream_t)stream);
    if (rc) { m->arena.reset(); return rc; }
    rc = apply_impl(m, st, d_spec, mm, cc, m->cfg.model_kind == 1 ? aa : nullptr, B, T, d_spec_e, stream);
    m->arena.reset();
    return rc;
}

extern "C" int64_t dfb_enhance_out_len(const dfb_state *st, int64_t T, int pad) {
    if (!st) return -1;
    return pad ? T : (T / st->hop) * st->hop;
}

extern "C" int dfb_model_set_max_workspace(dfb_model *m, int64_t bytes) {
    if (!m || bytes <= 0) return fail(DFB_ERR_INVALID, "bad workspace cap");
    m->max_workspace = (size_t)bytes;
    return DFB_OK;
}


struct StreamState {
    int B = 0;
    int64_t a1 = 0, d1 = 0, e1 = 0;
    bool started = false, dnn_started = false;
    float *slab = nullptr;
    float *ana_mem = nullptr;
    float *erb_state = nullptr, *unit_state = nullptr;
    float *h_enc = nullptr, *h_erb = nullptr, *h_df = nullptr;
    float *t_spec = nullptr, *t_fe = nullptr, *t_fs = nullptr;
    float *t_m = nullptr, *t_c = nullptr;
    float *t_l = nullptr;
    float *t_dec = nullptr;
    int n_feat = 0, n_mc = 0, n_dec = 0;
};
constexpr int kMcTail = 6;

struct ChunkGeom { int Lmax, lag, Hf; };
static ChunkGeom chunk_geom(const dfb_model_config &c) {
    ChunkGeom g;
    g.Lmax = c.conv_lookahead > c.df_lookahead ? c.conv_lookahead : c.df_lookahead;
    g.lag = c.model_kind != 3 ? c.df_lookahead : 0;
    g.Hf = kHalo + g.Lmax;
    return g;
}

static size_t state_floats(const dfb_model_config &c, const dfb_state *st, int B, size_t off[16]) {
    const ChunkGeom g = chunk_geom(c);
    const int E = c.nb_erb, Fd = c.nb_df, O2 = 2 * c.df_order, F = st->tb.F, ED = E / 4 * kCh;
    size_t n = 0;
    auto add = [&](int i, size_t k) { off[i] = n; n += (k + 63) & ~size_t(63); };
    add(0, (size_t)B * st->hop); add(1, (size_t)B * E); add(2, (size_t)B * Fd);
    add(3, (size_t)c.enc_gru_layers * B * c.emb_hidden); add(4, (size_t)c.erb_gru_layers * B * c.emb_hidden);
    add(5, (size_t)c.df_gru_layers * B * c.df_hidden);
    add(6, (size_t)B * g.Hf * 2 * F); add(7, (size_t)B * g.Hf * E); add(8, (size_t)B * g.Hf * 2 * Fd);
    add(9, (size_t)B * kMcTail * E); add(10, (size_t)B * kMcTail * Fd * O2);
    add(11, c.conv_kt > 1 ? (size_t)B * kHalo * ED : 0);
    add(12, (size_t)B * kMcTail);
    return n;
}
static void state_bind(StreamState &S, float *base, const size_t off[16], int B) {
    S.B = B; S.slab = base;
    S.ana_mem = base + off[0]; S.erb_state = base + off[1]; S.unit_state = base + off[2];
    S.h_enc = base + off[3]; S.h_erb = base + off[4]; S.h_df = base + off[5];
    S.t_spec = base + off[6]; S.t_fe = base + off[7]; S.t_fs = base + off[8];
    S.t_m = base + off[9]; S.t_c = base + off[10]; S.t_dec = base + off[11]; S.t_l = base + off[12];
    S.a1 = S.d1 = S.e1 = 0; S.started = S.dnn_started = false; S.n_feat = S.n_mc = S.n_dec = 0;
}

static int save_tail(cudaStream_t s, const float *buf, int T, size_t fe, int n, float *tail, int cap, int B) {
    if (n <= 0) return DFB_OK;
    DFB_CUDA(cudaMemcpy2DAsync(tail + (size_t)(cap - n) * fe, sizeof(float) * fe * cap, buf + (size_t)(T - n) * fe, sizeof(float) * fe * T,
                               sizeof(float) * fe * n, B, cudaMemcpyDeviceToDevice, s));
    return DFB_OK;
}
static int load_tail(cudaStream_t s, float *buf, int T, size_t fe, int n, const float *tail, int cap, int dst_t, int B) {
    if (n <= 0) return DFB_OK;
    DFB_CUDA(cudaMemcpy2DAsync(buf + (size_t)dst_t * fe, sizeof(float) * fe * T, tail + (size_t)(cap - n) * fe, sizeof(float) * fe * cap,
                               sizeof(float) * fe * n, B, cudaMemcpyDeviceToDevice, s));
    return DFB_OK;
}

static size_t chunk_bytes_per_stream(const dfb_model_config &c, const dfb_state *st, int Tw) {
    const ChunkGeom g = chunk_geom(c);
    const int E = c.nb_erb, Fd = c.nb_df, O2 = 2 * c.df_order, F = st->tb.F;
    return (size_t)(Tw + g.Lmax) * (2 * F + E + 2 * Fd) * 4 + (size_t)Tw * (E + (size_t)Fd * O2 + 2) * 4 + fwd_plan(c, (size_t)Tw, nullptr, nullptr) +
           16384;
}

struct ChunkIO {
    const float *audio; int64_t audio_T, audio_stride;
    int64_t audio_frame0;
    const float *init_mem;
    float *out; int64_t out_stride, out_len;
    int64_t out_sample0;
    float atten_lim;
    const float *lsnr_th;
    const RaggedRow *rows = nullptr;
    int nb = 0;
};

static int run_chunk(dfb_model *m, dfb_state *st, StreamState &S, const ChunkIO &io, int64_t a1n, int64_t d1n, int64_t e1n,
                     cudaStream_t s, int lane = 0, bool pipelined = false) {
    Arena &arena = lane ? m->arena1 : m->arena;
    dfb_model::Lane &L = m->lanes[lane], &P = m->lanes[lane ^ 1];
    const bool have_prev = pipelined && S.started;
    if (have_prev) DFB_CUDA(cudaStreamWaitEvent(s, P.ev_fork, 0));
    const dfb_model_config &c = m->cfg;
    const ChunkGeom g = chunk_geom(c);
    const int B = io.nb > 0 ? io.nb : S.B, E = c.nb_erb, Fd = c.nb_df, O2 = 2 * c.df_order, F = st->tb.F, hop = st->hop;
    const int64_t W0 = S.d1 > kHalo ? S.d1 - kHalo : 0;
    const int Rc = (int)(S.d1 - W0), Tw = (int)(d1n - W0), Tsb = Tw + g.Lmax;
    const int n_hist = (int)(S.a1 - W0);
    const int n_new = (int)(a1n - S.a1), Tv = (int)(a1n - W0);
    if (Tw < Rc || n_hist < 0 || n_hist > S.n_feat || Tv > Tsb || Tsb <= 0)
        return fail(DFB_ERR_INVALID, "inconsistent chunk geometry");
    const bool run_dnn = d1n > S.d1;
    int rc;
    arena.reset();
    float *spec = arena.take<float>((size_t)B * Tsb * F * 2 + 2);
    float *fe = arena.take<float>((size_t)B * Tsb * E);
    float *fs = arena.take<float>((size_t)B * Tsb * Fd * 2);
    float *mm = arena.take<float>((size_t)B * (Tw + 1) * E);
    float *cc = arena.take<float>((size_t)B * (Tw + 1) * Fd * O2);
    float *ll = io.lsnr_th ? arena.take<float>((size_t)B * (Tw + 1)) : nullptr;
    float *aa = c.model_kind == 1 ? arena.take<float>((size_t)B * (Tw + 1)) : nullptr;
    if (!cc || (c.model_kind == 1 && !aa)) return fail(DFB_ERR_OOM, "chunk workspace exhausted");
    if ((rc = load_tail(s, spec, Tsb, (size_t)2 * F, n_hist, S.t_spec, g.Hf, 0, B)) || (rc = load_tail(s, fe, Tsb, E, n_hist, S.t_fe, g.Hf, 0, B)) ||
        (rc = load_tail(s, fs, Tsb, (size_t)2 * Fd, n_hist, S.t_fs, g.Hf, 0, B)))
        return rc;
    if (n_new > 0) {
        AnaWindow w{(int)(S.a1 - io.audio_frame0), n_new, n_hist, Tsb, io.audio_stride, io.rows};
        if ((rc = launch_analysis(st, io.audio, B, io.audio_T, spec, fe, s, io.init_mem, &w))) return rc;
        if ((rc = launch_feat_norm(fe + (size_t)n_hist * E, E, E, spec + (size_t)n_hist * 2 * F, Fd, F, B, n_new, c.norm_alpha,
                                   S.started ? S.erb_state : nullptr, S.started ? S.unit_state : nullptr, fe + (size_t)n_hist * E,
                                   fs + (size_t)n_hist * 2 * Fd, s, Tsb, S.erb_state, S.unit_state)))
            return rc;
    }
    {
        const int nf = Tv < g.Hf ? Tv : g.Hf;
        const size_t fes[3] = {(size_t)2 * F, (size_t)E, (size_t)2 * Fd};
        float *bufs[3] = {spec, fe, fs}, *tails[3] = {S.t_spec, S.t_fe, S.t_fs};
        for (int i = 0; i < 3; i++)
            DFB_CUDA(cudaMemcpy2DAsync(tails[i] + (size_t)(g.Hf - nf) * fes[i], sizeof(float) * fes[i] * g.Hf,
                                       bufs[i] + (size_t)(Tv - nf) * fes[i], sizeof(float) * fes[i] * Tsb, sizeof(float) * fes[i] * nf, B,
                                       cudaMemcpyDeviceToDevice, s));
        S.n_feat = nf;
    }
    if (run_dnn) {
    ChunkCtx cx{Rc, Tsb, Tv, S.h_enc, S.h_erb, S.h_df, S.dnn_started, c.conv_kt > 1 ? S.t_dec : nullptr, S.n_dec, lane,
                have_prev ? P.ev_done : nullptr, S.B, io.rows, W0};
    if ((rc = forward_impl(m, arena, fe, fs, B, Tw, mm, cc, ll, aa, s, &cx))) return rc;
    S.n_dec = cx.dec_tail_n;
    S.dnn_started = true;
    if (Rc > 0 && S.n_mc > 0) {
        const int n = S.n_mc < Rc ? S.n_mc : Rc;
        if ((rc = load_tail(s, mm, Tw, E, n, S.t_m, kMcTail, Rc - n, B)) || (rc = load_tail(s, cc, Tw, (size_t)Fd * O2, n, S.t_c, kMcTail, Rc - n, B)))
            return rc;
        if (ll && (rc = load_tail(s, ll, Tw, 1, n, S.t_l, kMcTail, Rc - n, B))) return rc;
    }
    }
    if (run_dnn && (e1n > S.e1 || io.rows)) {
        dfb::ApplyParams p{};
        p.spec = (const float2 *)spec; p.m = mm; p.coefs = cc; p.audio = io.out; p.spec_out = nullptr;
        p.out_stride = io.out_stride; p.out_len = io.out_len;
        p.out_offset = io.out_sample0 - W0 * hop;
        p.Tf = (int)(e1n - W0); p.spec_T = Tsb; p.Tv = Tv; p.mc_T = Tw; p.t_first = (int)(S.e1 - W0);
        p.mode = apply_mode(m); p.nb_df = Fd; p.order = c.df_order; p.lookahead = c.df_lookahead;
        p.atten_lim = io.atten_lim;
        p.alpha = aa;
        apply_options(m, p);
        if (ll) { p.lsnr = ll; p.th_min = io.lsnr_th[0]; p.th_erb = io.lsnr_th[1]; p.th_df = io.lsnr_th[2]; }
        if (io.rows) { p.rows = io.rows; p.w0 = W0; p.t_emit = p.Tf; p.Tf = Tw; }
        if ((rc = launch_apply_synthesis(st, p, B, s))) return rc;
    }
    {
        if (run_dnn) {
            const int nm = Tw < kMcTail ? Tw : kMcTail;
            if ((rc = save_tail(s, mm, Tw, E, nm, S.t_m, kMcTail, B)) || (rc = save_tail(s, cc, Tw, (size_t)Fd * O2, nm, S.t_c, kMcTail, B))) return rc;
            if (ll && (rc = save_tail(s, ll, Tw, 1, nm, S.t_l, kMcTail, B))) return rc;
            S.n_mc = nm;
        }
    }
    if (pipelined) {
        if (!run_dnn) DFB_CUDA(cudaEventRecord(L.ev_fork, s));
        DFB_CUDA(cudaEventRecord(L.ev_done, s));
    }
    S.a1 = a1n; S.d1 = d1n; if (run_dnn) S.e1 = e1n;
    S.started = true;
    return DFB_OK;
}

static int pick_chunk(const dfb_model *m, const dfb_state *st, int64_t B, int64_t Tf, int min_chunks, size_t cap) {
    const size_t per_frame = chunk_bytes_per_stream(m->cfg, st, 1024) / 1024 + 1;
    const ChunkGeom g = chunk_geom(m->cfg);
    int64_t tw = (int64_t)(cap / ((size_t)B * per_frame)) - g.Lmax - 8;
    int64_t tc = tw - kHalo;
    if (tc > Tf) tc = Tf;
    if (min_chunks > 1 && Tf >= (int64_t)min_chunks * 64) {
        const int64_t t2 = (Tf + min_chunks - 1) / min_chunks;
        if (t2 < tc) tc = t2;
    }
    if (m->cfg.model_kind == 1) return tw >= Tf ? (int)Tf : 0;
    if (tc < 1) return 0;
    if (tc < Tf && tc < 32) return 0;
    return (int)tc;
}
struct ChunkHooks {
    std::function<int(int64_t x0, int64_t x1, int64_t na, cudaStream_t cs)> before;
    std::function<int(int64_t y0, int64_t y1, int64_t d1, int64_t na, cudaStream_t cs)> after;
};

static int enhance_group(dfb_model *m, dfb_state *st, const float *d_x, float *d_out, const RaggedRow *rows, const int64_t *tfs,
                         int64_t nb, int pad, float lim, int tc, bool pipelined, cudaStream_t s, const ChunkHooks *hooks) {
    const dfb_model_config &c = m->cfg;
    const ChunkGeom g = chunk_geom(c);
    const int hop = st->hop, fft = st->fft;
    const int64_t Tf = tfs[0];
    size_t off[16];
    const size_t nstate = state_floats(c, st, (int)nb, off);
    float *slab = m->aux_arena.take<float>(nstate);
    if (!slab) return fail(DFB_ERR_OOM, "stream state arena exhausted");
    StreamState S;
    state_bind(S, slab, off, (int)nb);
    int rc = DFB_OK;
    const int64_t delay = pad ? fft - hop : 0;
    if (tc >= Tf) pipelined = false;
    cudaEvent_t ev_call = nullptr;
    if (pipelined) {
        DFB_CUDA(cudaEventCreateWithFlags(&ev_call, cudaEventDisableTiming));
        DFB_CUDA(cudaEventRecord(ev_call, s));
        DFB_CUDA(cudaStreamWaitEvent(m->lanes[0].main, ev_call, 0));
        DFB_CUDA(cudaStreamWaitEvent(m->lanes[1].main, ev_call, 0));
    }
    int chunk = 0, last_lane = 0;
    const bool taper = hooks && pipelined && tc < Tf && tc >= 64;
    while (S.d1 < Tf) {
        int64_t step = tc;
        if (taper) {
            const int64_t left = Tf - S.d1;
            if (chunk == 0) step = tc / 2;
            else if (left <= tc + tc / 2 && left - tc / 2 >= tc / 4) step = left - tc / 2;
        }
        const int64_t d1n = S.d1 + step < Tf ? S.d1 + step : Tf;
        const int64_t a1n = d1n + g.Lmax < Tf ? d1n + g.Lmax : Tf;
        const int64_t e1n = d1n == Tf ? Tf : d1n - g.lag;
        const int lane = pipelined ? (chunk & 1) : 0;
        cudaStream_t cs = pipelined ? m->lanes[lane].main : s;
        int64_t na = nb;
        while (na > 1 && tfs[na - 1] <= S.d1) na--;
        if (hooks && S.a1 < a1n && (rc = hooks->before(S.a1 * hop, a1n * hop, na, cs))) break;
        const int64_t e0 = S.e1;
        ChunkIO io{d_x, Tf * hop, Tf * hop, 0, nullptr, d_out, 0, 0, delay, lim, nullptr, rows, (int)na};
        if ((rc = run_chunk(m, st, S, io, a1n, d1n, e1n > S.e1 ? e1n : S.e1, cs, lane, pipelined))) break;
        if (hooks && (rc = hooks->after(e0 * hop > delay ? e0 * hop - delay : 0, S.e1 * hop - delay, d1n, na, cs))) break;
        last_lane = lane;
        chunk++;
    }
    if (pipelined) {
        if (chunk > 0) cudaStreamWaitEvent(s, m->lanes[last_lane].ev_done, 0);
        if (chunk > 1) cudaStreamWaitEvent(s, m->lanes[last_lane ^ 1].ev_done, 0);
        if (rc) cudaDeviceSynchronize();
        cudaEventDestroy(ev_call);
    }
    return rc;
}

static int enhance_plan(dfb_model *m, dfb_state *st, int64_t B, int64_t Tf, int min_chunks, int64_t *group_out, int *tc_out,
                        bool *pipelined_out) {
    static const bool serial = getenv("DFB_SERIAL") && atoi(getenv("DFB_SERIAL"));
    const bool pipelined = m->n_lanes == 2 && !serial && min_chunks > 1 && Tf >= (int64_t)min_chunks * 64;
    const size_t cap = pipelined ? m->max_workspace / 2 : m->max_workspace;
    int64_t group = B > 65535 ? 65535 : B;
    int tc = 0;
    while ((tc = pick_chunk(m, st, group, Tf, min_chunks, cap)) == 0) {
        if (group == 1) return fail(DFB_ERR_OOM, "workspace cap of %zu bytes is too small for a single stream", m->max_workspace);
        group = (group + 1) / 2;
    }
    *group_out = group; *tc_out = tc; *pipelined_out = pipelined && tc < Tf;
    const ChunkGeom g = chunk_geom(m->cfg);
    const size_t bytes = chunk_bytes_per_stream(m->cfg, st, tc + kHalo) * (size_t)group + ((size_t)g.Lmax << 10) + (2 << 20);
    int rc = m->arena.reserve(bytes);
    if (!rc && *pipelined_out) rc = m->arena1.reserve(bytes);
    return rc;
}


static int ragged_plan(const dfb_state *st, int64_t in_numel, const int64_t *in_offsets, const int64_t *lengths, int64_t B, int pad,
                       int64_t out_numel, const int64_t *out_offsets, std::vector<RaggedRow> &rows) {
    if (!in_offsets || !lengths || !out_offsets) return fail(DFB_ERR_INVALID, "null argument");
    if (B <= 0) return fail(DFB_ERR_INVALID, "empty batch");
    rows.resize((size_t)B);
    for (int64_t b = 0; b < B; b++) {
        const int64_t len = lengths[b], io = in_offsets[b], oo = out_offsets[b];
        if (len <= 0) return fail(DFB_ERR_INVALID, "stream %lld has length %lld", (long long)b, (long long)len);
        const int64_t tf = (pad ? len + st->fft : len) / st->hop, ol = dfb_enhance_out_len(st, len, pad);
        if (tf <= 0) return fail(DFB_ERR_INVALID, "stream %lld is shorter than one hop", (long long)b);
        if (io < 0 || io > in_numel - len)
            return fail(DFB_ERR_INVALID, "stream %lld reaches outside the input (%lld samples)", (long long)b, (long long)in_numel);
        if (oo < 0 || oo > out_numel - ol)
            return fail(DFB_ERR_INVALID, "stream %lld reaches outside the output (%lld samples)", (long long)b, (long long)out_numel);
        rows[(size_t)b] = RaggedRow{io, len, oo, ol, tf};
    }
    return DFB_OK;
}

struct StreamCopy { int64_t dst_off, src_off, end; };
template <class At>
static int copy_streams(float *dst, const float *src, int64_t x0, int64_t n, At at, cudaMemcpyKind kind, cudaStream_t s) {
    constexpr int64_t kMaxPitch = INT32_MAX / sizeof(float);
    for (int64_t i = 0, j; i < n; i = j) {
        const StreamCopy a = at(i);
        const int64_t w = a.end - x0;
        int64_t dp = 0, sp = 0;
        for (j = i + 1; j < n; j++) {
            const StreamCopy b = at(j), p = at(j - 1);
            if (b.end != a.end) break;
            if (j == i + 1) {
                dp = b.dst_off - a.dst_off; sp = b.src_off - a.src_off;
                if (dp < w || sp < w || dp > kMaxPitch || sp > kMaxPitch) break;
            } else if (b.dst_off - p.dst_off != dp || b.src_off - p.src_off != sp) break;
        }
        if (w <= 0) continue;
        if (j - i == 1) DFB_CUDA(cudaMemcpyAsync(dst + a.dst_off + x0, src + a.src_off + x0, sizeof(float) * w, kind, s));
        else DFB_CUDA(cudaMemcpy2DAsync(dst + a.dst_off + x0, sizeof(float) * dp, src + a.src_off + x0, sizeof(float) * sp,
                                        sizeof(float) * w, (size_t)(j - i), kind, s));
    }
    return DFB_OK;
}

static int enhance_rows(dfb_model *m, dfb_state *st, std::vector<RaggedRow> &rows, const float *src, float *dst, int pad,
                        float atten_lim_db, bool host, cudaStream_t s) {
    std::stable_sort(rows.begin(), rows.end(), [](const RaggedRow &a, const RaggedRow &b) { return a.Tf > b.Tf; });
    const int64_t B = (int64_t)rows.size();
    std::vector<int64_t> tfs((size_t)B);
    int64_t true_frames = 0;
    for (int64_t i = 0; i < B; i++) { tfs[i] = rows[i].Tf; true_frames += tfs[i]; }
    int min_chunks = m->host_chunks;
    if (!host) {
        min_chunks = m->dev_chunks > 0 ? m->dev_chunks : (B <= 8 ? 3 : (B <= 256 ? 2 : 1));
        if (m->dev_chunks == 0 && (double)B * tfs[0] > 1.1 * (double)true_frames && min_chunks < 4) min_chunks = 4;
    }
    int64_t group = 0;
    int tc = 0;
    bool pipelined = false;
    int rc = enhance_plan(m, st, B, tfs[0], min_chunks, &group, &tc, &pipelined);
    if (rc) return rc;
    size_t off[16];
    if ((rc = m->aux_arena.reserve(state_floats(m->cfg, st, (int)group, off) * sizeof(float) + (size_t)group * sizeof(RaggedRow) + 8192)))
        return rc;
    auto group_end = [&](int64_t b0) {
        int64_t b1 = B - b0 < group ? B : b0 + group;
        if (m->cfg.model_kind == 1)
            for (int64_t i = b0 + 1; i < b1; i++)
                if (tfs[i] != tfs[b0]) { b1 = i; break; }
        return b1;
    };
    std::vector<RaggedRow> drows(rows);
    float *d_in = nullptr, *d_out = nullptr;
    if (host) {
        int64_t n_in = 0, n_out = 0;
        for (int64_t b0 = 0, b1; b0 < B; b0 = b1) {
            b1 = group_end(b0);
            int64_t gi = 0, go = 0;
            for (int64_t i = b0; i < b1; i++) {
                drows[i].in_off = gi; drows[i].out_off = go;
                gi += rows[i].len; go += rows[i].out_len;
            }
            n_in = std::max(n_in, gi); n_out = std::max(n_out, go);
        }
        if ((rc = st->arena.reserve(sizeof(float) * (size_t)(n_in + n_out) + 4096))) return rc;
        st->arena.reset();
        d_in = st->arena.take<float>((size_t)n_in); d_out = st->arena.take<float>((size_t)n_out);
    }
    const float lim = (atten_lim_db > 0.f) ? powf(10.f, -atten_lim_db / 20.f) : 0.f;
    cudaStream_t sc = host ? m->stream : s, sh = m->h2d, sd = m->d2h;
    std::vector<cudaEvent_t> evs;
    auto order = [&](cudaStream_t from, cudaStream_t to) -> int {
        cudaEvent_t e = nullptr;
        DFB_CUDA(cudaEventCreateWithFlags(&e, cudaEventDisableTiming));
        evs.push_back(e);
        DFB_CUDA(cudaEventRecord(e, from));
        DFB_CUDA(cudaStreamWaitEvent(to, e, 0));
        return DFB_OK;
    };
    for (int64_t b0 = 0, b1; b0 < B && !rc; b0 = b1) {
        b1 = group_end(b0);
        const RaggedRow *hr = rows.data() + b0, *dr = drows.data() + b0;
        const int64_t *tf = tfs.data() + b0;
        ChunkHooks hooks;
        hooks.before = [&](int64_t x0, int64_t x1, int64_t na, cudaStream_t cs) -> int {
            const int r = copy_streams(d_in, src, x0, na, [&](int64_t i) {
                return StreamCopy{dr[i].in_off, hr[i].in_off, std::min(x1, hr[i].len)};
            }, cudaMemcpyHostToDevice, sh);
            return r ? r : order(sh, cs);
        };
        hooks.after = [&](int64_t y0, int64_t y1, int64_t d1, int64_t na, cudaStream_t cs) -> int {
            if (const int r = order(cs, sd)) return r;
            return copy_streams(dst, d_out, y0, na, [&](int64_t i) {
                return StreamCopy{hr[i].out_off, dr[i].out_off, tf[i] <= d1 ? hr[i].out_len : std::min(y1, hr[i].out_len)};
            }, cudaMemcpyDeviceToHost, sd);
        };
        if (host && ((rc = order(sd, sc)) || (rc = order(sc, sh)))) break;
        m->aux_arena.reset();
        RaggedRow *d_rows = m->aux_arena.take<RaggedRow>((size_t)(b1 - b0));
        DFB_CUDA(cudaMemcpyAsync(d_rows, dr, sizeof(RaggedRow) * (b1 - b0), cudaMemcpyHostToDevice, sc));
        rc = enhance_group(m, st, host ? d_in : src, host ? d_out : dst, d_rows, tf, b1 - b0, pad, lim, tc, pipelined, sc,
                           host ? &hooks : nullptr);
    }
    if (host) {
        const cudaError_t e1 = cudaStreamSynchronize(sc), e2 = cudaStreamSynchronize(sd), e3 = cudaStreamSynchronize(sh);
        const cudaError_t e = e1 != cudaSuccess ? e1 : (e2 != cudaSuccess ? e2 : e3);
        if (!rc && e != cudaSuccess) rc = fail(DFB_ERR_CUDA, "enhance_host failed: %s", cudaGetErrorString(e));
    }
    for (cudaEvent_t e : evs) cudaEventDestroy(e);
    m->arena.reset();
    m->arena1.reset();
    return rc;
}

static int equal_rows(const dfb_state *st, int64_t B, int64_t T, int pad, std::vector<RaggedRow> &rows) {
    const int64_t Tf = (pad ? T + st->fft : T) / st->hop, out_len = dfb_enhance_out_len(st, T, pad);
    if (Tf <= 0) return fail(DFB_ERR_INVALID, "input shorter than one hop");
    rows.resize((size_t)B);
    for (int64_t b = 0; b < B; b++) rows[(size_t)b] = RaggedRow{b * T, T, b * out_len, out_len, Tf};
    return DFB_OK;
}

extern "C" int dfb_enhance(dfb_model *m, dfb_state *st, const float *d_audio, int64_t B, int64_t T, int pad,
                           float atten_lim_db, float *d_out, void *stream) {
    if (!m || !st || !d_audio || !d_out) return fail(DFB_ERR_INVALID, "null argument");
    if (B <= 0 || T <= 0) return fail(DFB_ERR_INVALID, "empty input");
    if (int rcs = check_state(m, st)) return rcs;
    std::vector<RaggedRow> rows;
    if (int rc = equal_rows(st, B, T, pad, rows)) return rc;
    DFB_CUDA(cudaSetDevice(m->device));
    return enhance_rows(m, st, rows, d_audio, d_out, pad, atten_lim_db, false, (cudaStream_t)stream);
}

extern "C" int dfb_enhance_host(dfb_model *m, dfb_state *st, const float *h_audio, int64_t B, int64_t T, int pad,
                                float atten_lim_db, float *h_out) {
    if (!m || !st || !h_audio || !h_out) return fail(DFB_ERR_INVALID, "null argument");
    if (B <= 0 || T <= 0) return fail(DFB_ERR_INVALID, "empty input");
    if (int rcs = check_state(m, st)) return rcs;
    std::vector<RaggedRow> rows;
    if (int rc = equal_rows(st, B, T, pad, rows)) return rc;
    DFB_CUDA(cudaSetDevice(m->device));
    return enhance_rows(m, st, rows, h_audio, h_out, pad, atten_lim_db, true, nullptr);
}

extern "C" int dfb_enhance_ragged(dfb_model *m, dfb_state *st, const float *d_audio, int64_t in_numel, const int64_t *in_offsets,
                                  const int64_t *lengths, int64_t B, int pad, float atten_lim_db, float *d_out, int64_t out_numel,
                                  const int64_t *out_offsets, void *stream) {
    if (!m || !st || !d_audio || !d_out) return fail(DFB_ERR_INVALID, "null argument");
    if (int rcs = check_state(m, st)) return rcs;
    std::vector<RaggedRow> rows;
    if (int rc = ragged_plan(st, in_numel, in_offsets, lengths, B, pad, out_numel, out_offsets, rows)) return rc;
    DFB_CUDA(cudaSetDevice(m->device));
    return enhance_rows(m, st, rows, d_audio, d_out, pad, atten_lim_db, false, (cudaStream_t)stream);
}

extern "C" int dfb_enhance_ragged_host(dfb_model *m, dfb_state *st, const float *h_audio, int64_t in_numel, const int64_t *in_offsets,
                                       const int64_t *lengths, int64_t B, int pad, float atten_lim_db, float *h_out, int64_t out_numel,
                                       const int64_t *out_offsets) {
    if (!m || !st || !h_audio || !h_out) return fail(DFB_ERR_INVALID, "null argument");
    if (int rcs = check_state(m, st)) return rcs;
    std::vector<RaggedRow> rows;
    if (int rc = ragged_plan(st, in_numel, in_offsets, lengths, B, pad, out_numel, out_offsets, rows)) return rc;
    DFB_CUDA(cudaSetDevice(m->device));
    return enhance_rows(m, st, rows, h_audio, h_out, pad, atten_lim_db, true, nullptr);
}

struct dfb_stream {
    dfb_model *m;
    dfb_state *st;
    int B;
    float lim;
    StreamState S;
    float *slab = nullptr;
    bool gating = false;
    float th[3] = {-10.f, 30.f, 20.f};
    float *stage_in = nullptr, *stage_out = nullptr;
    size_t stage_cap = 0;
};

extern "C" int dfb_stream_create(dfb_stream **out, dfb_model *m, dfb_state *st, int64_t B, float atten_lim_db) {
    if (!out || !m || !st || B <= 0 || B > 65535) return fail(DFB_ERR_INVALID, "bad argument");
    *out = nullptr;
    if (int rcs = check_state(m, st)) return rcs;
    if (m->cfg.model_kind == 1)
        return fail(DFB_ERR_UNSUPPORTED, "DeepFilterNet v1 runs as one window per signal (forward_v1): no frame-incremental API");
    DFB_CUDA(cudaSetDevice(m->device));
    dfb_stream *h = new dfb_stream();
    h->m = m; h->st = st; h->B = (int)B;
    h->lim = (atten_lim_db > 0.f) ? powf(10.f, -atten_lim_db / 20.f) : 0.f;
    size_t off[16];
    const size_t n = state_floats(m->cfg, st, (int)B, off);
    if (cudaMalloc(&h->slab, n * sizeof(float)) != cudaSuccess) { delete h; return fail(DFB_ERR_OOM, "stream state allocation failed"); }
    cudaMemset(h->slab, 0, n * sizeof(float));
    state_bind(h->S, h->slab, off, (int)B);
    *out = h;
    return DFB_OK;
}

extern "C" void dfb_stream_free(dfb_stream *h) {
    if (!h) return;
    cudaSetDevice(h->m->device);
    if (h->slab) cudaFree(h->slab);
    if (h->stage_in) cudaFree(h->stage_in);
    if (h->stage_out) cudaFree(h->stage_out);
    delete h;
}

extern "C" int dfb_stream_reset(dfb_stream *h) {
    if (!h) return fail(DFB_ERR_INVALID, "null stream");
    size_t off[16];
    state_floats(h->m->cfg, h->st, h->B, off);
    state_bind(h->S, h->slab, off, h->B);
    return DFB_OK;
}

extern "C" int dfb_stream_set_lsnr_thresholds(dfb_stream *h, int enable, float min_db_thresh, float max_db_erb_thresh,
                                              float max_db_df_thresh) {
    if (!h) return fail(DFB_ERR_INVALID, "null stream");
    if (enable && h->m->cfg.model_kind != 3) return fail(DFB_ERR_UNSUPPORTED, "LSNR stage gating: DeepFilterNet3 topologies only");
    h->gating = enable != 0;
    h->th[0] = min_db_thresh; h->th[1] = max_db_erb_thresh; h->th[2] = max_db_df_thresh;
    return DFB_OK;
}

extern "C" int64_t dfb_stream_latency_frames(const dfb_stream *h) {
    if (!h) return -1;
    const ChunkGeom g = chunk_geom(h->m->cfg);
    return g.Lmax + g.lag;
}
extern "C" int64_t dfb_stream_frame_length(const dfb_stream *h) { return h ? h->st->hop : -1; }

static int stream_step(dfb_stream *h, const float *d_in, int64_t n, bool flush, float *d_out, cudaStream_t s) {
    dfb_model *m = h->m;
    dfb_state *st = h->st;
    StreamState &S = h->S;
    const ChunkGeom g = chunk_geom(m->cfg);
    const int hop = st->hop, B = h->B;
    const int64_t Ltot = g.Lmax + g.lag;
    const int64_t n_out = flush ? Ltot : n;
    const int64_t a0 = S.a1, a1n = a0 + (flush ? 0 : n);
    int64_t d1n = flush ? a1n : a1n - g.Lmax, e1n = flush ? a1n : d1n - g.lag;
    if (d1n < S.d1) d1n = S.d1;
    if (e1n < S.e1) e1n = S.e1;
    const int64_t W0 = S.d1 > kHalo ? S.d1 - kHalo : 0;
    const int Tw = (int)(d1n - W0);
    int rc = m->arena.reserve(chunk_bytes_per_stream(m->cfg, st, Tw + 1) * (size_t)B + (2 << 20));
    if (rc) return rc;
    const int64_t f0 = (flush ? S.a1 : a0) - Ltot;
    if (f0 < 0 || e1n <= S.e1) DFB_CUDA(cudaMemsetAsync(d_out, 0, sizeof(float) * B * n_out * hop, s));
    ChunkIO io{d_in, (flush ? 0 : n) * hop, (flush ? 0 : n) * hop, a0, S.started ? S.ana_mem : nullptr, d_out, n_out * hop, n_out * hop,
               f0 * hop, h->lim, h->gating ? h->th : nullptr};
    if (!flush && a1n > a0) {
        if (!S.started) DFB_CUDA(cudaMemsetAsync(S.ana_mem, 0, sizeof(float) * B * hop, s));
        io.init_mem = S.ana_mem;
    }
    if ((rc = run_chunk(m, st, S, io, a1n, d1n, e1n, s))) return rc;
    if (!flush)
        DFB_CUDA(cudaMemcpy2DAsync(S.ana_mem, sizeof(float) * hop, d_in + (n - 1) * hop, sizeof(float) * n * hop, sizeof(float) * hop, B,
                                   cudaMemcpyDeviceToDevice, s));
    m->arena.reset();
    return DFB_OK;
}

extern "C" int dfb_stream_process(dfb_stream *h, const float *d_in, int64_t n_frames, float *d_out, void *stream) {
    if (!h || !d_in || !d_out || n_frames <= 0) return fail(DFB_ERR_INVALID, "bad argument");
    DFB_CUDA(cudaSetDevice(h->m->device));
    return stream_step(h, d_in, n_frames, false, d_out, (cudaStream_t)stream);
}

extern "C" int dfb_stream_flush(dfb_stream *h, float *d_out, void *stream) {
    if (!h || !d_out) return fail(DFB_ERR_INVALID, "bad argument");
    DFB_CUDA(cudaSetDevice(h->m->device));
    if (dfb_stream_latency_frames(h) == 0) return DFB_OK;
    return stream_step(h, nullptr, 0, true, d_out, (cudaStream_t)stream);
}

extern "C" int dfb_stream_process_host(dfb_stream *h, const float *h_in, int64_t n_frames, float *h_out) {
    if (!h || !h_out || (h_in && n_frames <= 0)) return fail(DFB_ERR_INVALID, "bad argument");
    DFB_CUDA(cudaSetDevice(h->m->device));
    const bool flush = h_in == nullptr;
    const int64_t nf = flush ? dfb_stream_latency_frames(h) : n_frames;
    if (nf == 0) return DFB_OK;
    const size_t bytes = sizeof(float) * (size_t)h->B * nf * h->st->hop;
    if (bytes > h->stage_cap) {
        if (h->stage_in) cudaFree(h->stage_in);
        if (h->stage_out) cudaFree(h->stage_out);
        h->stage_in = h->stage_out = nullptr; h->stage_cap = 0;
        if (cudaMalloc(&h->stage_in, bytes) != cudaSuccess || cudaMalloc(&h->stage_out, bytes) != cudaSuccess)
            return fail(DFB_ERR_OOM, "stream staging allocation failed");
        h->stage_cap = bytes;
    }
    cudaStream_t s = h->m->stream;
    if (!flush) DFB_CUDA(cudaMemcpyAsync(h->stage_in, h_in, bytes, cudaMemcpyHostToDevice, s));
    int rc = stream_step(h, h->stage_in, nf, flush, h->stage_out, s);
    if (rc) return rc;
    DFB_CUDA(cudaMemcpyAsync(h_out, h->stage_out, bytes, cudaMemcpyDeviceToHost, s));
    DFB_CUDA(cudaStreamSynchronize(s));
    return DFB_OK;
}
```

### deepfilternet_b200/csrc/dfb_tc.cu

```cuda
#include <cooperative_groups.h>
#include <atomic>
#include <map>
#include <mutex>
#include <cuda.h>
#include <cuda_bf16.h>

#include "dfb_common.cuh"
#include "dfb_dwpw.cuh"
#include "dfb_ptx.cuh"

namespace dfb {

constexpr int kBxBM = 128, kBxBN = 128, kBxBK = 64, kBxStages = 3, kBxThreads = 288;
constexpr int kBxBox = 128 * 128;

struct BxSmem {
    alignas(1024) unsigned char x[kBxStages][2][kBxBox];
    alignas(1024) unsigned char w[kBxStages][2][kBxBox];
    alignas(8) uint64_t full[kBxStages];
    uint64_t empty[kBxStages];
};

__global__ void __launch_bounds__(kBxThreads, 1)
k_gemm_bf16x3(const __grid_constant__ CUtensorMap tmXhi, const __grid_constant__ CUtensorMap tmXlo,
              const __grid_constant__ CUtensorMap tmWhi, const __grid_constant__ CUtensorMap tmWlo,
              const float *__restrict__ bias, float *__restrict__ Y, int64_t ldy, int M, int K, int nslices) {
    extern __shared__ __align__(1024) unsigned char tc_smem_raw[];
    BxSmem &sm = *reinterpret_cast<BxSmem *>(((uintptr_t)tc_smem_raw + 1023) & ~uintptr_t(1023));
    const int warp = threadIdx.x >> 5, lane = threadIdx.x & 31;
    const int n0 = (int)(blockIdx.x % nslices) * kBxBN, m0 = (int)(blockIdx.x / nslices) * kBxBM;
    const int nkb = K / kBxBK;
    if (threadIdx.x == 0) {
        for (int s = 0; s < kBxStages; s++) { mbar_init(&sm.full[s], 1); mbar_init(&sm.empty[s], 8); }
        fence_barrier_init();
    }
    __syncthreads();
    if (warp == 8) {
        if (lane == 0) {
            tma_prefetch_desc(&tmXhi); tma_prefetch_desc(&tmXlo); tma_prefetch_desc(&tmWhi); tma_prefetch_desc(&tmWlo);
            for (int kb = 0; kb < nkb; kb++) {
                const int s = kb % kBxStages, n = kb / kBxStages;
                if (n > 0) mbar_wait(&sm.empty[s], (n - 1) & 1);
                mbar_expect_tx(&sm.full[s], 4 * kBxBox);
                tma_load_2d(sm.x[s][0], &tmXhi, kb * kBxBK, m0, &sm.full[s]);
                tma_load_2d(sm.x[s][1], &tmXlo, kb * kBxBK, m0, &sm.full[s]);
                tma_load_2d(sm.w[s][0], &tmWhi, kb * kBxBK, n0, &sm.full[s]);
                tma_load_2d(sm.w[s][1], &tmWlo, kb * kBxBK, n0, &sm.full[s]);
            }
        }
        return;
    }
    const int wm = (warp & 3) * 32, wn = (warp >> 2) * 64;
    float acc[2][8][4];
#pragma unroll
    for (int a = 0; a < 2; a++)
#pragma unroll
        for (int b = 0; b < 8; b++)
#pragma unroll
            for (int c = 0; c < 4; c++) acc[a][b][c] = 0.f;
    for (int kb = 0; kb < nkb; kb++) {
        const int s = kb % kBxStages;
        mbar_wait(&sm.full[s], (kb / kBxStages) & 1);
        warp_mma_sw128_k64<2>(smem_u32(sm.x[s][0]), smem_u32(sm.x[s][1]), smem_u32(sm.w[s][0]), smem_u32(sm.w[s][1]), wm, wn, acc);
        __syncwarp();
        if (lane == 0) mbar_arrive(&sm.empty[s]);
    }
#pragma unroll
    for (int nt = 0; nt < 8; nt++) {
        const int n = n0 + wn + 8 * nt + 2 * (lane & 3);
        const float2 bn = bias ? make_float2(__ldg(bias + n), __ldg(bias + n + 1)) : make_float2(0.f, 0.f);
#pragma unroll
        for (int mt = 0; mt < 2; mt++)
#pragma unroll
            for (int h = 0; h < 2; h++) {
                const int m = m0 + wm + 16 * mt + (lane >> 2) + 8 * h;
                if (m < M)
                    *reinterpret_cast<float2 *>(Y + (int64_t)m * ldy + n) =
                        make_float2(acc[mt][nt][2 * h] + bn.x, acc[mt][nt][2 * h + 1] + bn.y);
            }
    }
}

constexpr int kDxThreads = 256;
constexpr uint32_t kDxW = 32768, kDxRaw = 49152, kDxTail = 64 * 4 + 32;


template <int MODE, int KT, int PATH, int MASK>
__global__ void __launch_bounds__(kDxThreads, 2)
k_dwpw_bx(DwPwParams p, const float *__restrict__ w_sw ) {
    extern __shared__ __align__(1024) unsigned char tc_smem_raw[];
    const uint32_t sb = smem_u32(tc_smem_raw);
    if (sb & 1023u) __trap();
    const int tid = threadIdx.x, warp = tid >> 5, lane = tid & 31;
    const int b = blockIdx.y, t0 = blockIdx.x * p.NF;
    const int nf = min(p.NF, p.T - t0);
    const int R = nf * p.Fout;
    const int tq0 = t0 - (KT - 1);
    const uint32_t fbytes = (uint32_t)p.Fin * kCh * 4;
    const uint32_t raw_in = sb + kDxRaw, raw_path = raw_in + (uint32_t)(p.NF + KT - 1) * fbytes;
    const uint32_t raw_e0 = raw_in + (uint32_t)(p.NF + KT - 1) * fbytes * (PATH ? 2u : 1u);
    const uint32_t obytes = (uint32_t)p.Fout * kCh * 4;
    const uint32_t tail = raw_e0 + (MASK ? (uint32_t)p.NF * obytes : 0u);
    const uint32_t s_bias = tail, bar_raw = tail + 264;
    const uint32_t s_mask = raw_in;
    if (tid == 0) {
        mbar_init_a(bar_raw, 1);
        fence_barrier_init();
        const int ta = max(tq0, 0), tb = t0 + nf;
        mbar_expect_tx_a(bar_raw, (uint32_t)(tb - ta) * fbytes * (PATH ? 2u : 1u) + 2u * kCh * 128u + (MASK ? (uint32_t)nf * obytes : 0u));
        if (MASK)
            for (int t = t0; t < tb; t++)
                bulk_load(raw_e0 + (uint32_t)(t - t0) * obytes, p.mk_e0 + ((int64_t)b * p.T + t) * p.Fout * kCh, obytes, bar_raw);
        for (int t = ta; t < tb; t++) {
            bulk_load(raw_in + (uint32_t)(t - tq0) * fbytes, p.in + ((int64_t)b * p.T + t) * p.in_fs, fbytes, bar_raw);
            if (PATH) bulk_load(raw_path + (uint32_t)(t - tq0) * fbytes, p.path + ((int64_t)b * p.T + t) * p.path_fs, fbytes, bar_raw);
        }
        bulk_load(sb + kDxW, w_sw, 2 * kCh * 128, bar_raw);
    }
    if (tid < kCh / 4) sts128(s_bias + tid * 16, __ldg(reinterpret_cast<const float4 *>(p.bias) + tid));
    const int cq = tid & 15, slot = tid >> 4;
    float4 wd[KT][3], ps4, pb4;
#pragma unroll
    for (int dt = 0; dt < KT; dt++)
#pragma unroll
        for (int df = 0; df < 3; df++) wd[dt][df] = __ldg(reinterpret_cast<const float4 *>(p.dw + (dt * 3 + df) * kCh) + cq);
    if (PATH) {
        ps4 = __ldg(reinterpret_cast<const float4 *>(p.ps) + cq);
        pb4 = __ldg(reinterpret_cast<const float4 *>(p.pb) + cq);
    }
    int fr = (8 * slot * p.fo_magic) >> 16, fo = 8 * slot - fr * p.Fout;
    __syncthreads();
    mbar_wait_a(bar_raw, 0);
    auto rd = [&](uint32_t a) -> float4 {
        float4 x = lds128(a);
        if (PATH) {
            const float4 e = lds128(a + (raw_path - raw_in));
            x.x += fmaxf(fmaf(e.x, ps4.x, pb4.x), 0.f); x.y += fmaxf(fmaf(e.y, ps4.y, pb4.y), 0.f);
            x.z += fmaxf(fmaf(e.z, ps4.z, pb4.z), 0.f); x.w += fmaxf(fmaf(e.w, ps4.w, pb4.w), 0.f);
        }
        return x;
    };
    const float4 zero4 = make_float4(0.f, 0.f, 0.f, 0.f);
#pragma unroll
    for (int i = 0; i < 8; i++) {
        const int r = 8 * slot + i;
        float4 acc = zero4;
        if (r < R) {
#pragma unroll
            for (int dt = 0; dt < KT; dt++) {
                if (KT > 1 && tq0 + fr + dt < 0) continue;
                const uint32_t fb = raw_in + (uint32_t)(fr + dt) * fbytes + cq * 16;
                if (MODE == DW_S1) {
                    const uint32_t a = fb + (uint32_t)fo * 256;
                    if (fo > 0) acc = f4_fma(rd(a - 256), wd[dt][0], acc);
                    acc = f4_fma(rd(a), wd[dt][1], acc);
                    if (fo + 1 < p.Fin) acc = f4_fma(rd(a + 256), wd[dt][2], acc);
                } else if (MODE == DW_S2) {
                    const uint32_t a = fb + (uint32_t)fo * 512;
                    if (fo > 0) acc = f4_fma(rd(a - 256), wd[dt][0], acc);
                    acc = f4_fma(rd(a), wd[dt][1], acc);
                    acc = f4_fma(rd(a + 256), wd[dt][2], acc);
                } else {
                    const uint32_t a = fb + (uint32_t)(fo >> 1) * 256;
                    if ((fo & 1) == 0) {
                        acc = f4_fma(rd(a), wd[dt][1], acc);
                    } else {
                        acc = f4_fma(rd(a), wd[dt][2], acc);
                        if ((fo >> 1) + 1 < p.Fin) acc = f4_fma(rd(a + 256), wd[dt][0], acc);
                    }
                }
            }
        }
        uint32_t h0, l0, h1, l1;
        bf16x2_split(acc.x, acc.y, h0, l0);
        bf16x2_split(acc.z, acc.w, h1, l1);
        const uint32_t off = sb + sw128_off(r, cq >> 1) + (cq & 1) * 8;
        sts64(off, h0, h1);
        sts64(off + 16384, l0, l1);
        if (++fo == p.Fout) { fo = 0; fr++; }
    }
    __syncthreads();
    if (MASK && tid >= 64 && tid < 64 + 80) {
        const int i = tid - 64;
        const float4 *src = i < 16 ? reinterpret_cast<const float4 *>(p.mk_ps) + i
                          : i < 32 ? reinterpret_cast<const float4 *>(p.mk_pb) + (i - 16)
                                   : reinterpret_cast<const float4 *>(p.mk_w) + (i - 32);
        sts128(s_mask + i * 16, __ldg(src));
    }
    float acc[1][8][4];
#pragma unroll
    for (int nt = 0; nt < 8; nt++)
#pragma unroll
        for (int c = 0; c < 4; c++) acc[0][nt][c] = 0.f;
    warp_mma_sw128_k64<1>(sb, sb + 16384, sb + kDxW, sb + kDxW + 8192, warp * 16, 0, acc);
    __syncthreads();
#pragma unroll
    for (int nt = 0; nt < 8; nt++) {
        const int c = 8 * nt + 2 * (lane & 3);
        float b0, b1;
        asm volatile("ld.shared.v2.f32 {%0, %1}, [%2];" : "=f"(b0), "=f"(b1) : "r"(s_bias + 4 * c));
#pragma unroll
        for (int h = 0; h < 2; h++) {
            const int r = warp * 16 + (lane >> 2) + 8 * h;
            asm volatile("st.shared.v2.f32 [%0], {%1, %2};" ::"r"(sb + r * 256 + (((c >> 2) ^ (r & 15)) << 4) + (c & 3) * 4),
                         "f"(fmaxf(acc[0][nt][2 * h] + b0, 0.f)), "f"(fmaxf(acc[0][nt][2 * h + 1] + b1, 0.f)) : "memory");
        }
    }
    __syncthreads();
    if (MASK) {
        const int j = tid & 15, r0 = 8 * slot;
        const int fr = (r0 * p.fo_magic) >> 16, f0 = r0 - fr * p.Fout;
        const float4 s4 = lds128(s_mask + j * 16), b4 = lds128(s_mask + 256 + j * 16);
        const float4 w0 = lds128(s_mask + 512 + j * 16), w1 = lds128(s_mask + 512 + 256 + j * 16), w2 = lds128(s_mask + 512 + 512 + j * 16);
        float part[8];
#pragma unroll
        for (int i = 0; i < 8; i++) part[i] = 0.f;
        if (r0 < R) {
#pragma unroll
            for (int i = -1; i <= 8; i++) {
                const int f2 = f0 + i, r2 = r0 + i;
                if (f2 < 0 || f2 >= p.Fout) continue;
                const float4 d = lds128(sb + r2 * 256 + ((j ^ (r2 & 15)) << 4));
                const float4 e = lds128(raw_e0 + r2 * 256 + j * 16);
                float4 x;
                x.x = fmaxf(fmaf(e.x, s4.x, b4.x), 0.f) + d.x; x.y = fmaxf(fmaf(e.y, s4.y, b4.y), 0.f) + d.y;
                x.z = fmaxf(fmaf(e.z, s4.z, b4.z), 0.f) + d.z; x.w = fmaxf(fmaf(e.w, s4.w, b4.w), 0.f) + d.w;
                if (i + 1 < 8) part[i + 1 < 0 ? 0 : i + 1] += x.x * w0.x + x.y * w0.y + x.z * w0.z + x.w * w0.w;
                if (i >= 0 && i < 8) part[i < 0 ? 0 : (i > 7 ? 7 : i)] += x.x * w1.x + x.y * w1.y + x.z * w1.z + x.w * w1.w;
                if (i - 1 >= 0) part[i - 1 > 7 ? 7 : i - 1] += x.x * w2.x + x.y * w2.y + x.z * w2.z + x.w * w2.w;
            }
        }
#pragma unroll
        for (int i = 0; i < 8; i++) {
            float v = part[i];
            v += __shfl_xor_sync(0xffffffffu, v, 1);
            v += __shfl_xor_sync(0xffffffffu, v, 2);
            v += __shfl_xor_sync(0xffffffffu, v, 4);
            v += __shfl_xor_sync(0xffffffffu, v, 8);
            part[i] = v;
        }
        if (r0 < R && j < 8) {
            float z = part[0];
#pragma unroll
            for (int i = 1; i < 8; i++) z = j == i ? part[i] : z;
            z += __ldg(p.mk_bias);
            p.mk_out[((int64_t)b * p.T + t0 + fr) * p.Fout + f0 + j] = 1.f / (1.f + expf(-z));
        }
    }
    if (p.out || p.out_hi) {
        const int j = tid & 15;
        int fr2 = (8 * slot * p.fo_magic) >> 16, fo2 = 8 * slot - fr2 * p.Fout;
        int64_t off = ((int64_t)b * p.T + t0 + fr2) * p.out_fs + fo2 * kCh + j * 4;
#pragma unroll
        for (int i = 0; i < 8; i++) {
            const int r = 8 * slot + i;
            if (r < R) {
                const float4 v = lds128(sb + r * 256 + ((j ^ (r & 15)) << 4));
                if (p.out) *reinterpret_cast<float4 *>(p.out + off) = v;
                if (p.out_hi) {
                    uint32_t h0, l0, h1, l1;
                    bf16x2_split(v.x, v.y, h0, l0);
                    bf16x2_split(v.z, v.w, h1, l1);
                    *reinterpret_cast<uint2 *>(p.out_hi + off) = make_uint2(h0, h1);
                    *reinterpret_cast<uint2 *>(p.out_lo + off) = make_uint2(l0, l1);
                }
            }
            off += kCh;
            if (++fo2 == p.Fout) { fo2 = 0; off += p.out_fs - (int64_t)p.Fout * kCh; }
        }
    }
}

template <int MODE, int KT, int PATH, int MASK = 0>
static int launch_dwpw_bx(cudaStream_t s, const DwPwParams &p, const float *w_sw, int B) {
    static int attr_smem[64] = {0};
    int dev = 0;
    cudaGetDevice(&dev);
    dev &= 63;
    const int raw = (p.NF + KT - 1) * p.Fin * kCh * 4 * (PATH ? 2 : 1) + (MASK ? p.NF * p.Fout * kCh * 4 : 0);
    const int smem = (int)kDxRaw + raw + (int)kDxTail;
    if (smem > 227 * 1024) return fail(DFB_ERR_UNSUPPORTED, "dwpw tile needs %d bytes of shared memory", smem);
    if (smem > attr_smem[dev]) {
        DFB_CUDA(cudaFuncSetAttribute(k_dwpw_bx<MODE, KT, PATH, MASK>, cudaFuncAttributeMaxDynamicSharedMemorySize, smem));
        attr_smem[dev] = smem;
    }
    dim3 grid((unsigned)((p.T + p.NF - 1) / p.NF), (unsigned)B);
    DFB_PROF("k_dwpw_bx", s);
    k_dwpw_bx<MODE, KT, PATH, MASK><<<grid, kDxThreads, smem, s>>>(p, w_sw);
    DFB_LAUNCH_CHECK();
    return DFB_OK;
}

template <int MODE>
int launch_dwpw_tc(cudaStream_t s, DwPwParams p, const float *w_sw, int B) {
    p.NF = 128 / p.Fout;
    if (p.NF < 1) p.NF = 1;
    if (p.NF * p.Fout > 128) return fail(DFB_ERR_UNSUPPORTED, "dwpw tile: Fout = %d", p.Fout);
    p.fo_magic = (65536 + p.Fout - 1) / p.Fout;
    for (int r = 0; r < 128; r++)
        if (((r * p.fo_magic) >> 16) != r / p.Fout) return fail(DFB_ERR_UNSUPPORTED, "dwpw tile: Fout = %d", p.Fout);
    if ((p.in_fs * 4) % 16 || (p.path && (p.path_fs * 4) % 16)) return fail(DFB_ERR_UNSUPPORTED, "dwpw: unaligned frame stride");
    const bool path = p.path != nullptr;
    if (MODE == DW_S1) {
        if (p.kt == 1) return path ? launch_dwpw_bx<DW_S1, 1, 1>(s, p, w_sw, B) : launch_dwpw_bx<DW_S1, 1, 0>(s, p, w_sw, B);
        if (p.kt == 2) return path ? launch_dwpw_bx<DW_S1, 2, 1>(s, p, w_sw, B) : launch_dwpw_bx<DW_S1, 2, 0>(s, p, w_sw, B);
    } else if (MODE == DW_S2 && !path) {
        if (p.kt == 1) return launch_dwpw_bx<DW_S2, 1, 0>(s, p, w_sw, B);
        if (p.kt == 2) return launch_dwpw_bx<DW_S2, 2, 0>(s, p, w_sw, B);
    } else if (MODE == DW_T2 && path && p.kt == 1) {
        if (p.mk_e0) {
            return launch_dwpw_bx<DW_T2, 1, 1, 1>(s, p, w_sw, B);
        }
        return launch_dwpw_bx<DW_T2, 1, 1>(s, p, w_sw, B);
    }
    return fail(DFB_ERR_UNSUPPORTED, "dwpw tensor-core path: mode %d kt %d path %d", MODE, p.kt, (int)path);
}
template int launch_dwpw_tc<DW_S1>(cudaStream_t, DwPwParams, const float *, int);
template int launch_dwpw_tc<DW_S2>(cudaStream_t, DwPwParams, const float *, int);
template int launch_dwpw_tc<DW_T2>(cudaStream_t, DwPwParams, const float *, int);

constexpr int kCvThreads = 256, kCvOut = 124, kCvYld = 51 , kCvBins = 8;
constexpr uint32_t kCvW = 32768, kCvRawOff = 49152, kCvYs = kCvRawOff + 32768, kCvTail = kCvYs + 128 * kCvYld * 4;

struct CvParams {
    const float *w_sw;
    const float *w2;
    const float *bias;
    float *coefs;
    int T, Fd;
};

template <int ORDER, int KTP>
__global__ void __launch_bounds__(kCvThreads, 2) k_df_convp_tc(const __grid_constant__ CUtensorMap tmC0, CvParams p) {
    constexpr int O2 = 2 * ORDER, NY = KTP * ORDER;
    extern __shared__ __align__(1024) unsigned char tc_smem_raw[];
    const uint32_t sb = (smem_u32(tc_smem_raw) + 1023u) & ~1023u;
    const int tid = threadIdx.x, warp = tid >> 5, lane = tid & 31;
    const int f_begin = blockIdx.x * kCvBins, f_end = min(f_begin + kCvBins, p.Fd);
    const int b = blockIdx.z, t0 = blockIdx.y * kCvOut, r0 = t0 - (KTP - 1);
    const uint32_t s_w2 = sb + kCvTail, bar_raw = s_w2 + 512, bar_w = bar_raw + 16;
    const int row = b * p.T + r0;
    auto load_bin = [&](int f) {
        mbar_expect_tx_a(bar_raw, 32768);
        asm volatile("cp.async.bulk.tensor.2d.shared::cluster.global.mbarrier::complete_tx::bytes [%0], [%1, {%2, %3}], [%4];"
                     ::"r"(sb + kCvRawOff), "l"((uint64_t)&tmC0), "r"(f * 64), "r"(row), "r"(bar_raw) : "memory");
        asm volatile("cp.async.bulk.tensor.2d.shared::cluster.global.mbarrier::complete_tx::bytes [%0], [%1, {%2, %3}], [%4];"
                     ::"r"(sb + kCvRawOff + 16384), "l"((uint64_t)&tmC0), "r"(f * 64 + 32), "r"(row), "r"(bar_raw) : "memory");
    };
    if (tid == 0) {
        mbar_init_a(bar_raw, 1);
        mbar_init_a(bar_w, 1);
        fence_barrier_init();
        mbar_expect_tx_a(bar_w, 16384);
        bulk_load(sb + kCvW, p.w_sw, 16384, bar_w);
        load_bin(f_begin);
    }
    for (int i = tid; i < O2 * O2 + O2; i += kCvThreads)
        asm volatile("st.shared.f32 [%0], %1;" ::"r"(s_w2 + 4 * i), "f"(i < O2 * O2 ? __ldg(p.w2 + i) : __ldg(p.bias + i - O2 * O2)) : "memory");
    __syncthreads();
    mbar_wait_a(bar_w, 0);
    const int r = tid & 127, half = tid >> 7;
    const bool zero = r0 + r < 0;
    for (int f = f_begin, it = 0; f < f_end; f++, it++) {
        const uint32_t par = (uint32_t)(it & 1);
        mbar_wait_a(bar_raw, par);
        {
            const uint32_t src = sb + kCvRawOff + (uint32_t)half * 16384u + (uint32_t)r * 128u;
            float4 xs[8];
#pragma unroll
            for (int c = 0; c < 8; c++) xs[c] = lds128(src + (uint32_t)((c ^ (r & 7)) << 4));
#pragma unroll
            for (int c = 0; c < 8; c++) {
                float4 x = xs[c];
                if (zero) x = make_float4(0.f, 0.f, 0.f, 0.f);
                uint32_t h0, l0, h1, l1;
                bf16x2_split(x.x, x.y, h0, l0);
                bf16x2_split(x.z, x.w, h1, l1);
                const int cq = half * 8 + c;
                const uint32_t off = sb + sw128_off(r, cq >> 1) + (cq & 1) * 8;
                sts64(off, h0, h1);
                sts64(off + 16384, l0, l1);
            }
        }
        fence_proxy_async();
        __syncthreads();
        if (tid == 0 && f + 1 < f_end) load_bin(f + 1);
        {
            float acc[1][8][4];
#pragma unroll
            for (int nt = 0; nt < 8; nt++)
#pragma unroll
                for (int c = 0; c < 4; c++) acc[0][nt][c] = 0.f;
            warp_mma_sw128_k64<1>(sb, sb + 16384, sb + kCvW, sb + kCvW + 8192, warp * 16, 0, acc);
#pragma unroll
            for (int nt = 0; nt < 8; nt++)
#pragma unroll
                for (int e = 0; e < 4; e++) {
                    const int n = 8 * nt + 2 * (lane & 3) + (e & 1), g = n >> 5, j = n & 31;
                    const int rr = warp * 16 + (lane >> 2) + 8 * (e >> 1);
                    if (j < NY)
                        asm volatile("st.shared.f32 [%0], %1;" ::"r"(sb + kCvYs + (uint32_t)(rr * kCvYld + g * NY + j) * 4u), "f"(acc[0][nt][e]) : "memory");
                }
        }
        __syncthreads();
        if (tid < 128) {
            const int t = r0 + tid;
            if (tid >= KTP - 1 && tid < KTP - 1 + kCvOut && t < p.T) {
                float z[O2];
#pragma unroll
                for (int g = 0; g < 2; g++)
#pragma unroll
                    for (int o = 0; o < ORDER; o++) {
                        float a = 0.f;
#pragma unroll
                        for (int dt = 0; dt < KTP; dt++) {
                            float y;
                            asm volatile("ld.shared.f32 %0, [%1];" : "=f"(y) : "r"(sb + kCvYs + (uint32_t)((tid - (KTP - 1) + dt) * kCvYld + g * NY + dt * ORDER + o) * 4u));
                            a += y;
                        }
                        z[g * ORDER + o] = a;
                    }
                float outv[O2];
#pragma unroll
                for (int qo = 0; qo < O2; qo++) {
                    float a;
                    asm volatile("ld.shared.f32 %0, [%1];" : "=f"(a) : "r"(s_w2 + 4 * (O2 * O2 + qo)));
#pragma unroll
                    for (int k = 0; k < O2; k++) {
                        float w;
                        asm volatile("ld.shared.f32 %0, [%1];" : "=f"(w) : "r"(s_w2 + 4 * (k * O2 + qo)));
                        a = fmaf(z[k], w, a);
                    }
                    outv[qo] = fmaxf(a, 0.f);
                }
                float *dst = p.coefs + (((int64_t)b * p.T + t) * p.Fd + f) * O2;
#pragma unroll
                for (int qo = 0; qo < O2; qo += 2) *reinterpret_cast<float2 *>(dst + qo) = make_float2(outv[qo], outv[qo + 1]);
            }
        }
    }
}

namespace cg = cooperative_groups;

constexpr int kGtU = 32, kGtRows = 3 * kGtU;
template <int NS, int HH>
struct GtCfg {
    static constexpr int kC = HH / kGtU;
    static constexpr int kKS = HH / 128;
    static constexpr int kMmaWarps = 6 * kKS;
    static constexpr int kGateThreads = 16 * NS;
    static constexpr int kThreads = kGateThreads > 32 * kMmaWarps ? kGateThreads : 32 * kMmaWarps;
    static constexpr int kLbo = (NS / 8) * 256;
    static constexpr int kSbo = 256;
    static constexpr int kPlane = 128;
    static constexpr int kPiece = 4 * kLbo;
    static constexpr int kBuf = (HH / 8) * kLbo;
    static constexpr int kPreLd = NS + 1;
};

template <int NS, int HH>
struct GruTcSmem {
    alignas(1024) unsigned char h[2][GtCfg<NS, HH>::kBuf];
    alignas(128) unsigned char wlo[kGtRows * HH * 2];
    float pre[GtCfg<NS, HH>::kKS][kGtRows][GtCfg<NS, HH>::kPreLd];
    alignas(8) uint64_t bar_h[2];
};

struct GruTcParams {
    const float *xproj;
    const float *whh;
    const float *bhh;
    const float *res;
    float *hout;
    unsigned short *hout_hi, *hout_lo;
    int planes_res;
    const float *h0;
    float *hT;
    int t0, Ts;
    int B, T, Bc;
    long long *dbg;
    unsigned char *xbuf;
};

template <int NS, int HH, int XG>
__global__ void __launch_bounds__(GtCfg<NS, HH>::kThreads, 1) k_gru_tc(GruTcParams p) {
    using Cfg = GtCfg<NS, HH>;
    constexpr int kGtThreads = Cfg::kThreads, kGtH = HH, kGtC = Cfg::kC, NT = NS / 8;
    extern __shared__ __align__(1024) unsigned char tc_smem_raw[];
    GruTcSmem<NS, HH> &sm = *reinterpret_cast<GruTcSmem<NS, HH> *>(((uintptr_t)tc_smem_raw + 1023) & ~uintptr_t(1023));
    cg::cluster_group cluster = cg::this_cluster();
    const int rank = (int)cluster.block_rank();
    const int group = blockIdx.x / kGtC;
    const int b0 = group * p.Bc;
    const int nb = min(p.Bc, p.B - b0);
    const int tid = threadIdx.x, warp = tid >> 5, lane = tid & 31;
    const int H = kGtH, T = p.T;
    for (int i = tid; i < (int)sizeof(sm.h) / 16; i += kGtThreads) reinterpret_cast<uint4 *>(&sm.h[0][0])[i] = make_uint4(0, 0, 0, 0);
    if (tid == 0) {
        mbar_init(&sm.bar_h[0], XG ? 1 : 2);
        mbar_init(&sm.bar_h[1], XG ? 1 : 2);
        fence_barrier_init();
    }
    if (p.h0) {
        __syncthreads();
        for (int i = tid; i < nb * (kGtH / 2); i += kGtThreads) {
            const int s = i / (kGtH / 2), gu = (i - s * (kGtH / 2)) * 2;
            const float2 hv = *reinterpret_cast<const float2 *>(p.h0 + (int64_t)(b0 + s) * kGtH + gu);
            unsigned short h0b, l0b, h1b, l1b;
            bf16_split(hv.x, h0b, l0b);
            bf16_split(hv.y, h1b, l1b);
            const uint32_t off = (uint32_t)((gu >> 3) * Cfg::kLbo + (s >> 3) * Cfg::kSbo + (s & 7) * 16 + (gu & 7) * 2);
            *reinterpret_cast<uint32_t *>(sm.h[0] + off) = h0b | (uint32_t)h1b << 16;
            *reinterpret_cast<uint32_t *>(sm.h[0] + off + Cfg::kPlane) = l0b | (uint32_t)l1b << 16;
        }
    }
    const bool mma_warp = warp < Cfg::kMmaWarps;
    const int mt = warp % 6, kq = warp / 6;
    uint32_t wa[8][4];
    const uint32_t wlo = smem_u32(sm.wlo);
    if (mma_warp) {
#pragma unroll
        for (int ks = 0; ks < 8; ks++)
#pragma unroll
            for (int e = 0; e < 4; e++) {
                const int rho = 16 * mt + (lane >> 2) + 8 * (e & 1), k = 128 * kq + 16 * ks + 2 * (lane & 3) + 8 * (e >> 1);
                const int gate = rho / kGtU, u = rho - gate * kGtU;
                const float2 w = *reinterpret_cast<const float2 *>(p.whh + ((int64_t)gate * H + rank * kGtU + u) * H + k);
                uint32_t hi, lo;
                bf16x2_split(w.x, w.y, hi, lo);
                wa[ks][e] = hi;
                asm volatile("st.shared.b32 [%0], %1;" ::"r"(wlo + (uint32_t)rho * (HH * 2) + ((((k >> 3) ^ (rho & 7))) << 4) + (k & 7) * 2),
                             "r"(lo) : "memory");
            }
    }
    fence_proxy_async();
    __syncthreads();
    cluster.sync();
    const uint32_t step_bytes = (uint32_t)((kGtC - (XG ? 0 : 1)) * Cfg::kPiece);

    const int up = tid & 15, s = tid >> 4;
    const bool gate_thread = tid < Cfg::kGateThreads;
    const bool active = gate_thread && s < nb;
    const int gu = rank * kGtU + 2 * up;
    float hprev0 = 0.f, hprev1 = 0.f;
    float2 bhr = make_float2(0.f, 0.f), bhz = bhr, bhn = bhr;
    if (active) {
        if (p.h0) {
            const float2 hv = *reinterpret_cast<const float2 *>(p.h0 + (int64_t)(b0 + s) * H + gu);
            hprev0 = hv.x; hprev1 = hv.y;
        }
        bhr = *reinterpret_cast<const float2 *>(p.bhh + gu);
        bhz = *reinterpret_cast<const float2 *>(p.bhh + H + gu);
        bhn = *reinterpret_cast<const float2 *>(p.bhh + 2 * H + gu);
    }
    const uint32_t hoff = (uint32_t)((gu >> 3) * Cfg::kLbo + (s >> 3) * Cfg::kSbo + (s & 7) * 16 + (gu & 7) * 2);
    const uint32_t piece0 = (uint32_t)(rank * Cfg::kPiece);
    const bool dbg_on = p.dbg && blockIdx.x == 0 && tid == 0;
    const int mat = lane >> 3, rr = lane & 7;
    for (int t = 0; t < T; t++) {
        const int cur = t & 1;
        if (dbg_on) p.dbg[t * 8 + 0] = clock64();
        if (tid == 0 && t + 1 < T) mbar_expect_tx(&sm.bar_h[cur ^ 1], step_bytes);
        float2 xr = make_float2(0.f, 0.f), xz = xr, xn = xr;
        if (active) {
            const float *xp = p.xproj + ((int64_t)(b0 + s) * p.Ts + p.t0 + t) * (3 * H) + gu;
            xr = *reinterpret_cast<const float2 *>(xp);
            xz = *reinterpret_cast<const float2 *>(xp + H);
            xn = *reinterpret_cast<const float2 *>(xp + 2 * H);
            if (t + 3 < T && (up & 7) == 0) {
                const float *xq = xp + 3 * (3 * H);
                asm volatile("prefetch.global.L2 [%0];" ::"l"(xq));
                asm volatile("prefetch.global.L2 [%0];" ::"l"(xq + H));
                asm volatile("prefetch.global.L2 [%0];" ::"l"(xq + 2 * H));
            }
        }
        if (t > 0) mbar_wait(&sm.bar_h[cur], (uint32_t)(((t - 1) >> 1) & 1));
        if (dbg_on) p.dbg[t * 8 + 1] = clock64();
        if (mma_warp) {
            float acc[NT][4];
#pragma unroll
            for (int n = 0; n < NT; n++) acc[n][0] = acc[n][1] = acc[n][2] = acc[n][3] = 0.f;
            const uint32_t hb = smem_u32(sm.h[cur]);
#pragma unroll
            for (int ks = 0; ks < 8; ks++) {
                const int k = 128 * kq + 16 * ks;
                uint32_t al[4];
                {
                    const int r = 16 * mt + rr + ((mat & 1) << 3);
                    ldsm_x4(wlo + (uint32_t)r * (HH * 2) + ((((k >> 3) + (mat >> 1)) ^ (r & 7)) << 4), al);
                }
#pragma unroll
                for (int n = 0; n < NT; n++) {
                    uint32_t b[4];
                    ldsm_x4(hb + (uint32_t)(((k >> 3) + (mat & 1)) * Cfg::kLbo + n * Cfg::kSbo + (mat >> 1) * Cfg::kPlane + rr * 16), b);
                    mma_bf16x3(acc[n], wa[ks], al, b[0], b[1], b[2], b[3]);
                }
            }
#pragma unroll
            for (int n = 0; n < NT; n++)
#pragma unroll
                for (int e = 0; e < 4; e++)
                    sm.pre[kq][16 * mt + (lane >> 2) + 8 * (e >> 1)][8 * n + 2 * (lane & 3) + (e & 1)] = acc[n][e];
        }
        __syncthreads();
        if (dbg_on) p.dbg[t * 8 + 2] = clock64();
        uint32_t vhi = 0, vlo = 0;
        if (active) {
            const int u0 = 2 * up;
            float a[6];
#pragma unroll
            for (int g = 0; g < 3; g++) {
                float s0 = 0.f, s1 = 0.f;
#pragma unroll
                for (int q = 0; q < Cfg::kKS; q++) { s0 += sm.pre[q][g * kGtU + u0][s]; s1 += sm.pre[q][g * kGtU + u0 + 1][s]; }
                a[2 * g] = s0; a[2 * g + 1] = s1;
            }
            const float r0 = gt_sigmoid(xr.x + a[0] + bhr.x), r1 = gt_sigmoid(xr.y + a[1] + bhr.y);
            const float z0 = gt_sigmoid(xz.x + a[2] + bhz.x), z1 = gt_sigmoid(xz.y + a[3] + bhz.y);
            const float n0 = gt_tanh(xn.x + r0 * (a[4] + bhn.x)), n1 = gt_tanh(xn.y + r1 * (a[5] + bhn.y));
            hprev0 = (1.f - z0) * n0 + z0 * hprev0;
            hprev1 = (1.f - z1) * n1 + z1 * hprev1;
            unsigned short h0, l0, h1, l1;
            bf16_split(hprev0, h0, l0);
            bf16_split(hprev1, h1, l1);
            vhi = h0 | (uint32_t)h1 << 16;
            vlo = l0 | (uint32_t)l1 << 16;
            if (t + 1 < T) {
                if (XG) {
                    unsigned char *xp = p.xbuf + ((size_t)(group * 2 + (cur ^ 1)) * kGtC + rank) * Cfg::kPiece + (hoff - piece0);
                    *reinterpret_cast<uint32_t *>(xp) = vhi;
                    *reinterpret_cast<uint32_t *>(xp + Cfg::kPlane) = vlo;
                } else {
                    *reinterpret_cast<uint32_t *>(sm.h[cur ^ 1] + hoff) = vhi;
                    *reinterpret_cast<uint32_t *>(sm.h[cur ^ 1] + hoff + Cfg::kPlane) = vlo;
                }
            }
        }
        if (dbg_on) p.dbg[t * 8 + 3] = clock64();
        if (t + 1 < T) { if (XG) fence_proxy_async_global(); else fence_proxy_async(); }
        __syncthreads();
        if (t + 1 < T) {
            if (XG) {
                if (tid == 0) {
                    const unsigned char *xp = p.xbuf + ((size_t)(group * 2 + (cur ^ 1)) * kGtC + rank) * Cfg::kPiece;
                    bulk_load_multicast(smem_u32(sm.h[cur ^ 1]) + piece0, xp, Cfg::kPiece, smem_u32(&sm.bar_h[cur ^ 1]),
                                        (uint16_t)((1u << kGtC) - 1u));
                }
            } else if (lane == 0) {
                const uint32_t src = smem_u32(sm.h[cur ^ 1]) + piece0;
                for (int j = warp; j < kGtC - 1; j += kGtThreads / 32) {
                    const int peer = j + (j >= rank ? 1 : 0);
                    dsmem_bulk_copy(mapa_u32(src, peer), src, Cfg::kPiece, mapa_u32(smem_u32(&sm.bar_h[cur ^ 1]), peer));
                }
                if (warp == 0) mbar_arrive(&sm.bar_h[cur ^ 1]);
            }
        }
        if (dbg_on) p.dbg[t * 8 + 4] = clock64();
        if (active) {
            const int64_t o = ((int64_t)(b0 + s) * p.Ts + p.t0 + t) * H + gu;
            float2 ov = make_float2(hprev0, hprev1);
            if (p.hT && t + 1 == T) *reinterpret_cast<float2 *>(p.hT + (int64_t)(b0 + s) * H + gu) = ov;
            if (p.res) { const float2 rv = *reinterpret_cast<const float2 *>(p.res + o); ov.x += rv.x; ov.y += rv.y; }
            *reinterpret_cast<float2 *>(p.hout + o) = ov;
            if (p.hout_hi) {
                if (p.planes_res && p.res) bf16x2_split(ov.x, ov.y, vhi, vlo);
                *reinterpret_cast<uint32_t *>(p.hout_hi + o) = vhi;
                *reinterpret_cast<uint32_t *>(p.hout_lo + o) = vlo;
            }
        }
    }
    cluster.sync();
}

static unsigned char *gru_xbuf(cudaStream_t s, size_t bytes) {
    struct Ent { unsigned char *p = nullptr; size_t cap = 0; };
    static std::mutex mu;
    static std::map<std::pair<int, cudaStream_t>, Ent> pool;
    int dev = 0;
    cudaGetDevice(&dev);
    std::lock_guard<std::mutex> lk(mu);
    Ent &e = pool[{dev, s}];
    if (e.cap < bytes) {
        if (e.p) { cudaDeviceSynchronize(); cudaFree(e.p); e.p = nullptr; e.cap = 0; }
        const size_t want = (bytes + (1u << 20)) & ~size_t((1u << 20) - 1);
        if (cudaMalloc(&e.p, want) != cudaSuccess) { e.p = nullptr; return nullptr; }
        e.cap = want;
    }
    return e.p;
}

template <int NS, int HH, int XG>
static int gru_tc_config(cudaLaunchConfig_t &cfg, cudaLaunchAttribute (&at)[1]) {
    using Cfg = GtCfg<NS, HH>;
    static PerDeviceOnce attr_once;
    const int smem = (int)sizeof(GruTcSmem<NS, HH>) + 1024;
    if (auto once_guard = attr_once.first()) {
        if (Cfg::kC > 8) DFB_CUDA(cudaFuncSetAttribute(k_gru_tc<NS, HH, XG>, cudaFuncAttributeNonPortableClusterSizeAllowed, 1));
        DFB_CUDA(cudaFuncSetAttribute(k_gru_tc<NS, HH, XG>, cudaFuncAttributeMaxDynamicSharedMemorySize, smem));
    }
    cfg = cudaLaunchConfig_t{};
    cfg.blockDim = dim3(Cfg::kThreads);
    cfg.dynamicSmemBytes = smem;
    at[0].id = cudaLaunchAttributeClusterDimension;
    at[0].val.clusterDim.x = Cfg::kC; at[0].val.clusterDim.y = 1; at[0].val.clusterDim.z = 1;
    cfg.attrs = at; cfg.numAttrs = 1;
    return DFB_OK;
}

template <int NS, int HH, int XG>
static int gru_tc_max_clusters(int *out) {
    static std::atomic<int> cached[64];
    int dev = 0;
    DFB_CUDA(cudaGetDevice(&dev));
    int n = cached[dev & 63].load(std::memory_order_relaxed);
    if (n <= 0) {
        cudaLaunchConfig_t cfg;
        cudaLaunchAttribute at[1];
        int rc = gru_tc_config<NS, HH, XG>(cfg, at);
        if (rc) return rc;
        cfg.gridDim = dim3((unsigned)GtCfg<NS, HH>::kC);
        DFB_CUDA(cudaOccupancyMaxActiveClusters(&n, k_gru_tc<NS, HH, XG>, &cfg));
        cached[dev & 63].store(n, std::memory_order_relaxed);
    }
    *out = n;
    return DFB_OK;
}

template <int NS, int HH, int XG>
static int launch_gru_tc_n(cudaStream_t s, GruTcParams p) {
    using Cfg = GtCfg<NS, HH>;
    cudaLaunchConfig_t cfg;
    cudaLaunchAttribute at[1];
    int rc = gru_tc_config<NS, HH, XG>(cfg, at);
    if (rc) return rc;
    p.Bc = NS;
    const int ngroups = (p.B + NS - 1) / NS;
    cfg.gridDim = dim3((unsigned)(ngroups * Cfg::kC));
    cfg.stream = s;
    if (XG) {
        p.xbuf = gru_xbuf(s, (size_t)ngroups * 2 * Cfg::kC * Cfg::kPiece);
        if (!p.xbuf) return fail(DFB_ERR_OOM, "GRU exchange scratch");
    }
    DFB_PROF(HH == 256 ? "k_gru_tc" : "k_gru_tc512", s);
    DFB_CUDA(cudaLaunchKernelEx(&cfg, k_gru_tc<NS, HH, XG>, p));
    g_launches.fetch_add(1, std::memory_order_relaxed);
    return DFB_OK;
}

int launch_gru_tc(cudaStream_t s, const float *xproj, const float *whh, const float *bhh, const float *res, float *hout,
                  unsigned short *hout_hi, unsigned short *hout_lo, int B, int T, long long *dbg, int wide, int planes_res,
                  const GruWindow *w, int H) {
    GruTcParams p{xproj, whh, bhh, res, hout, hout_hi, hout_lo, planes_res, w ? w->h0 : nullptr, w ? w->hT : nullptr,
                  w ? w->t0 : 0, w ? w->Ts : T, B, T, 0, dbg};
    static const int force = getenv("DFB_GRU_NS") ? atoi(getenv("DFB_GRU_NS")) : 0;
    static const int xg = getenv("DFB_GRU_XG") ? atoi(getenv("DFB_GRU_XG")) : 7;
    if (H == 512) return (xg & 1) ? launch_gru_tc_n<16, 512, 1>(s, p) : launch_gru_tc_n<16, 512, 0>(s, p);
    if (H != 256) return fail(DFB_ERR_UNSUPPORTED, "tensor-core recurrence: hidden size %d", H);
    const bool use32 = force ? force == 32 : ((wide && B > 64) || B >= 256);
    static const int no48 = getenv("DFB_GRU_NO48") ? atoi(getenv("DFB_GRU_NO48")) : 0;
    if (use32 && !force && !no48) {
        int wave = 0, rc = gru_tc_max_clusters<32, 256, 1>(&wave);
        if (rc) return rc;
        if (B > wave * 32) return launch_gru_tc_n<48, 256, 1>(s, p);
    }
    if (use32 && (xg & 2)) return launch_gru_tc_n<32, 256, 1>(s, p);
    if (!use32 && (xg & 4)) return launch_gru_tc_n<16, 256, 1>(s, p);
    return use32 ? launch_gru_tc_n<32, 256, 0>(s, p) : launch_gru_tc_n<16, 256, 0>(s, p);
}

int cached_map_f32_sw128(CUtensorMap *out, const void *base, int64_t rows, int64_t cols, int64_t ld, int box_rows);

int launch_df_convp_tc(cudaStream_t s, const float *c0, const float *w_sw, const float *w2, const float *bias, float *coefs, int B, int T,
                       int Fd) {
    if ((int64_t)B * T >= (int64_t(1) << 31) - 256 || B > 65535) return fail(DFB_ERR_UNSUPPORTED, "df pathway conv: batch too large for one launch");
    CUtensorMap mc;
    int rc;
    if ((rc = cached_map_f32_sw128(&mc, c0, (int64_t)B * T, (int64_t)Fd * kCh, (int64_t)Fd * kCh, 128))) return rc;
    const int smem = 1024 + (int)kCvTail + 512 + 64;
    static PerDeviceOnce attr_once;
    if (auto once_guard = attr_once.first())
        DFB_CUDA(cudaFuncSetAttribute(k_df_convp_tc<5, 5>, cudaFuncAttributeMaxDynamicSharedMemorySize, smem));
    CvParams p{w_sw, w2, bias, coefs, T, Fd};
    dim3 grid((unsigned)((Fd + kCvBins - 1) / kCvBins), (unsigned)((T + kCvOut - 1) / kCvOut), (unsigned)B);
    DFB_PROF("k_df_convp_tc", s);
    k_df_convp_tc<5, 5><<<grid, kCvThreads, smem, s>>>(mc, p);
    DFB_LAUNCH_CHECK();
    return DFB_OK;
}

int cached_map_bf16(CUtensorMap *out, const void *base, int64_t rows, int64_t cols, int64_t ld, int box_rows);

int launch_gemm_bf16x3(cudaStream_t s, const void *x_hi, const void *x_lo, int64_t ldx, const void *w_hi, const void *w_lo,
                       const float *bias, float *y, int64_t ldy, int64_t M, int N, int K) {
    if (N % kBxBN || K % kBxBK || (ldx % 8) || M <= 0 || ldy % 2 || ((uintptr_t)w_hi & 15) || ((uintptr_t)w_lo & 15))
        return fail(DFB_ERR_UNSUPPORTED, "bf16x3 GEMM shape M=%lld N=%d K=%d", (long long)M, N, K);
    const int nslices = N / kBxBN;
    const int64_t ntiles = (M + kBxBM - 1) / kBxBM;
    if (ntiles * nslices > 0x7fffffff) return fail(DFB_ERR_UNSUPPORTED, "bf16x3 GEMM: M = %lld", (long long)M);
    CUtensorMap mxh, mxl, mwh, mwl;
    int rc;
    if ((rc = cached_map_bf16(&mxh, x_hi, M, K, ldx, kBxBM)) || (rc = cached_map_bf16(&mxl, x_lo, M, K, ldx, kBxBM)) ||
        (rc = cached_map_bf16(&mwh, w_hi, N, K, K, kBxBN)) || (rc = cached_map_bf16(&mwl, w_lo, N, K, K, kBxBN)))
        return rc;
    static PerDeviceOnce attr_once;
    const int smem = (int)sizeof(BxSmem) + 1024;
    if (auto once_guard = attr_once.first()) DFB_CUDA(cudaFuncSetAttribute(k_gemm_bf16x3, cudaFuncAttributeMaxDynamicSharedMemorySize, smem));
    DFB_PROF("k_gemm_bf16x3[gru_proj]", s);
    k_gemm_bf16x3<<<(unsigned)(ntiles * nslices), kBxThreads, smem, s>>>(mxh, mxl, mwh, mwl, bias, y, ldy, (int)M, K, nslices);
    DFB_LAUNCH_CHECK();
    return DFB_OK;
}

}
```

Before: 51320.

## Fuse df_conv0 into DF front kernels, dropping the c0 intermediate buffer

Adds a k_df_front kernel that recomputes the first DF-pathway conv (df_conv0) from the input spectrum in shared memory. In one variant it feeds the depthwise/pointwise df_conv1 and writes bf16 hi/lo planes. In the other it feeds the tensor-core df_convp coefficient computation. This removes the materialised c0 tensor and its global write/read, including the TMA-based convp path. The price is computing conv0 twice, once on each stream. The non-fused fallback path drops its TC-plane output and tensor-core convp options.

```diff
diff --git a/deepfilternet_b200/csrc/dfb_common.cuh b/deepfilternet_b200/csrc/dfb_common.cuh
--- a/deepfilternet_b200/csrc/dfb_common.cuh
+++ b/deepfilternet_b200/csrc/dfb_common.cuh
@@ -159,8 +159,20 @@
                  const float *res, int64_t ldr, float *y, int64_t ldy, unsigned short *y_hi, unsigned short *y_lo, int64_t ldp,
                  int64_t M, int G, int Ig, int Hg, int act, float oscale, float ooffset);
 bool gl_bx_geometry(int G, int Ig, int Hg, int *gpc_out, int *hgp_out, int *stages_out);
-int launch_df_convp_tc(cudaStream_t s, const float *c0, const float *w_sw, const float *w2, const float *bias, float *coefs, int B, int T,
-                       int Fd);
+struct FrontParams {
+    const float *x;
+    const float *w0, *b0;
+    const float *dw, *pw_sw, *b1;
+    const float *cv_sw, *cv_w2, *cv_b;
+    unsigned short *c1_hi, *c1_lo;
+    float *coefs;
+    const RaggedRow *rows;
+    int64_t W0;
+    int T, Fd, inp_kt, lookahead;
+    int Tsx, Tx;
+};
+enum FrontPart { FRONT_C1 = 1, FRONT_CONVP = 2 };
+int launch_df_front(cudaStream_t s, const FrontParams &p, int B, int conv_kt, int part);
 int launch_to_planes(cudaStream_t s, const float *x, int64_t ldx, int64_t M, int K, unsigned short *hi, unsigned short *lo);
 }
 
diff --git a/deepfilternet_b200/csrc/dfb_gl.cu b/deepfilternet_b200/csrc/dfb_gl.cu
--- a/deepfilternet_b200/csrc/dfb_gl.cu
+++ b/deepfilternet_b200/csrc/dfb_gl.cu
@@ -199,37 +199,6 @@
     CUresult r = enc(&m, CU_TENSOR_MAP_DATA_TYPE_BFLOAT16, 2, (void *)base, dims, strides, box, estr, CU_TENSOR_MAP_INTERLEAVE_NONE,
                      CU_TENSOR_MAP_SWIZZLE_128B, CU_TENSOR_MAP_L2_PROMOTION_L2_128B, CU_TENSOR_MAP_FLOAT_OOB_FILL_NONE);
     if (r != CUDA_SUCCESS) return fail(DFB_ERR_CUDA, "cuTensorMapEncodeTiled (bf16) failed (%d)", (int)r);
-    if (cache.size() > 4096) cache.clear();
-    cache[key] = m;
-    *out = m;
-    return DFB_OK;
-}
-
-int cached_map_f32_sw128(CUtensorMap *out, const void *base, int64_t rows, int64_t cols, int64_t ld, int box_rows) {
-    static std::mutex mu;
-    static std::map<std::tuple<int, const void *, int64_t, int64_t, int64_t, int>, CUtensorMap> cache;
-    static PFN_encodeTiled_gl enc = nullptr;
-    int dev = 0;
-    cudaGetDevice(&dev);
-    std::lock_guard<std::mutex> g(mu);
-    auto key = std::make_tuple(dev, base, rows, cols, ld, box_rows);
-    auto it = cache.find(key);
-    if (it != cache.end()) { *out = it->second; return DFB_OK; }
-    if (!enc) {
-        void *fp = nullptr;
-        cudaDriverEntryPointQueryResult q;
-        if (cudaGetDriverEntryPoint("cuTensorMapEncodeTiled", &fp, cudaEnableDefault, &q) != cudaSuccess || q != cudaDriverEntryPointSuccess)
-            return fail(DFB_ERR_CUDA, "cuTensorMapEncodeTiled entry point not available");
-        enc = (PFN_encodeTiled_gl)fp;
-    }
-    cuuint64_t dims[2] = {(cuuint64_t)cols, (cuuint64_t)rows};
-    cuuint64_t strides[1] = {(cuuint64_t)ld * 4};
-    cuuint32_t box[2] = {32u, (cuuint32_t)box_rows};
-    cuuint32_t estr[2] = {1, 1};
-    CUtensorMap m;
-    CUresult r = enc(&m, CU_TENSOR_MAP_DATA_TYPE_FLOAT32, 2, (void *)base, dims, strides, box, estr, CU_TENSOR_MAP_INTERLEAVE_NONE,
-                     CU_TENSOR_MAP_SWIZZLE_128B, CU_TENSOR_MAP_L2_PROMOTION_L2_128B, CU_TENSOR_MAP_FLOAT_OOB_FILL_NONE);
-    if (r != CUDA_SUCCESS) return fail(DFB_ERR_CUDA, "cuTensorMapEncodeTiled (fp32) failed (%d)", (int)r);
     if (cache.size() > 4096) cache.clear();
     cache[key] = m;
     *out = m;
diff --git a/deepfilternet_b200/csrc/dfb_model.cu b/deepfilternet_b200/csrc/dfb_model.cu
--- a/deepfilternet_b200/csrc/dfb_model.cu
+++ b/deepfilternet_b200/csrc/dfb_model.cu
@@ -1062,7 +1062,10 @@
     return bytes + 4096;
 }
 
-static size_t fwd_plan(const dfb_model_config &c, size_t M, Arena *a, FwdBufs *f) {
+static bool df_front_fused(const dfb_model *m) { return m->conv_tc != 0 && m->cfg.model_kind != 1; }
+
+static size_t fwd_plan(const dfb_model *m, size_t M, Arena *a, FwdBufs *f) {
+    const dfb_model_config &c = m->cfg;
     if (c.model_kind == 1 && !a) return fwd_plan_v1(c, M, nullptr, nullptr);
     const int E = c.nb_erb, Fd = c.nb_df, H = c.emb_hidden, Hd = c.df_hidden;
     const int ED = E / 4 * kCh;
@@ -1078,7 +1081,8 @@
     t.e0 = take(M * E * kCh); t.e1 = take(M * (E / 2) * kCh); t.e2 = take(M * (E / 4) * kCh);
     t.emb_in = take(M * emb_in_dim);
     t.e3 = c.enc_concat ? t.emb_in : take(M * ED);
-    t.c0 = take(M * Fd * kCh); t.c1 = take(M * (Fd / 2) * kCh);
+    t.c0 = df_front_fused(m) ? nullptr : take(M * Fd * kCh);
+    t.c1 = take(M * (Fd / 2) * kCh);
     t.emb = take(M * emb_dim);
     t.g_a = take(M * Hmax); t.g_b = take(M * Hmax); t.g_h = take(M * Hmax);
     t.xproj = take(M * 3 * Hmax);
@@ -1124,7 +1128,7 @@
     if (B64 <= 0 || T64 <= 0) return DFB_OK;
     if (B64 > 65535) return fail(DFB_ERR_INVALID, "more than 65535 streams per call");
     DFB_CUDA(cudaSetDevice(m->device));
-    int rc = m->arena.reserve(fwd_plan(m->cfg, (size_t)B64 * T64, nullptr, nullptr));
+    int rc = m->arena.reserve(fwd_plan(m, (size_t)B64 * T64, nullptr, nullptr));
     if (rc) return rc;
     m->arena.reset();
     rc = forward_impl(m, m->arena, d_feat_erb, d_feat_spec, (int)B64, (int)T64, d_m, d_coefs, d_lsnr, d_alpha,
@@ -1179,13 +1183,15 @@
     const int emb_in_dim = c.enc_concat ? 2 * ED : ED;
     const int emb_dim = c.model_kind == 2 ? H : ED;
     int rc;
+    const bool front = df_front_fused(m);
     FwdBufs f{};
-    fwd_plan(c, (size_t)M, &arena, &f);
+    fwd_plan(m, (size_t)M, &arena, &f);
     if (!f.gh2_lo || !f.dfskip || !f.dfc_lo) return fail(DFB_ERR_OOM, "forward workspace exhausted for %lld frames", (long long)M);
     m->dbg.clear();
     m->dbg["e0"] = {f.e0, M * E * kCh}; m->dbg["e1"] = {f.e1, M * (E / 2) * kCh}; m->dbg["e2"] = {f.e2, M * (E / 4) * kCh};
-    m->dbg["e3"] = {f.e3, c.enc_concat ? M * emb_in_dim : M * ED}; m->dbg["c0"] = {f.c0, M * Fd * kCh};
-    m->dbg["c1"] = {f.c1, M * (Fd / 2) * kCh}; m->dbg["emb_in"] = {f.emb_in, M * emb_in_dim};
+    m->dbg["e3"] = {f.e3, c.enc_concat ? M * emb_in_dim : M * ED};
+    if (!front) { m->dbg["c0"] = {f.c0, M * Fd * kCh}; m->dbg["c1"] = {f.c1, M * (Fd / 2) * kCh}; }
+    m->dbg["emb_in"] = {f.emb_in, M * emb_in_dim};
     m->dbg["emb"] = {f.emb, M * emb_dim}; m->dbg["dec_emb"] = {f.dec_emb, M * ED}; m->dbg["d3"] = {f.d3, M * ED};
     m->dbg["d2"] = {f.d2, M * (E / 2) * kCh}; m->dbg["d1"] = {f.d1, M * E * kCh}; m->dbg["dfc"] = {f.dfc, M * Hd};
     m->dbg["g_a"] = {f.g_a, M * (H > Hd ? H : Hd)}; m->dbg["g_b"] = {f.g_b, M * (H > Hd ? H : Hd)};
@@ -1255,7 +1261,27 @@
         p.lookahead = 0;
         return p;
     };
-    {
+    if (front) {
+        FrontParams q{};
+        DwPwParams p{};
+        if ((rc = need(m, "enc.df_conv0.w", c.inp_kt * 3 * 2 * kCh, &q.w0)) || (rc = need(m, "enc.df_conv0.b", kCh, &q.b0)) ||
+            (rc = blk("enc.df_conv1", p)) || (rc = need(m, "df_dec.df_convp.w_sw", kCh * kCh, &q.cv_sw)) ||
+            (rc = need(m, "df_dec.df_convp.w2", 4 * c.df_order * c.df_order, &q.cv_w2)) ||
+            (rc = need(m, "df_dec.df_convp.b", 2 * c.df_order, &q.cv_b)))
+            return rc;
+        if (c.df_order != 5 || c.df_pathway_kt != 5)
+            return fail(DFB_ERR_UNSUPPORTED, "df_order %d / df_pathway_kernel_size_t %d (built kernels: 5, 5)", c.df_order,
+                        c.df_pathway_kt);
+        q.x = d_feat_spec; q.dw = p.dw; q.pw_sw = pw_sw; q.b1 = p.bias;
+        q.c1_hi = pl_c1.hi; q.c1_lo = pl_c1.lo; q.coefs = d_coefs; q.rows = rows; q.W0 = W0;
+        q.T = T; q.Fd = Fd; q.inp_kt = c.inp_kt; q.lookahead = c.conv_lookahead; q.Tsx = Tsx; q.Tx = Tx;
+        if ((rc = launch_df_front(sa, q, B, c.conv_kt, FRONT_C1))) return rc;
+        pl_c1.ok = true;
+        DFB_CUDA(cudaEventRecord(L.ev_join_enc, sa));
+        DFB_CUDA(cudaStreamWaitEvent(sl, L.ev_fork_enc, 0));
+        if ((rc = launch_df_front(sl, q, B, c.conv_kt, FRONT_CONVP))) return rc;
+        DFB_CUDA(cudaEventRecord(L.ev_convp, sl));
+    } else {
         DwPwParams p{};
         {
             const float *w, *bb;
@@ -1268,12 +1294,7 @@
             DFB_CUDA(cudaEventRecord(L.ev_c0, sa));
         }
         p = mk(f.c0, Fd, (int64_t)Fd * kCh, f.c1, Fd / 2, (int64_t)Fd / 2 * kCh, c.conv_kt);
-        if ((rc = blk("enc.df_conv1", p))) return rc;
-        if (pw_sw && gl_tc) {
-            p.out = nullptr; p.out_hi = pl_c1.hi; p.out_lo = pl_c1.lo; pl_c1.ok = true;
-            m->dbg.erase("c1");
-        }
-        if ((rc = run_dwpw<DW_S2>(sa, p, B, pw_sw))) return rc;
+        if ((rc = blk("enc.df_conv1", p)) || (rc = run_dwpw<DW_S2>(sa, p, B))) return rc;
         DFB_CUDA(cudaEventRecord(L.ev_join_enc, sa));
         DFB_CUDA(cudaStreamWaitEvent(sl, L.ev_c0, 0));
         const int O2 = 2 * c.df_order;
@@ -1286,16 +1307,10 @@
                         c.df_pathway_kt);
         if (Fd % 2) return fail(DFB_ERR_UNSUPPORTED, "df pathway conv: odd nb_df");
         dim3 grid((unsigned)((Fd + 2 * kCpWarps - 1) / (2 * kCpWarps)), (unsigned)((T + kCpChunk - 1) / kCpChunk), (unsigned)B);
-        static const bool convp_ffma = getenv("DFB_CONVP_FFMA") && atoi(getenv("DFB_CONVP_FFMA"));
-        const float *w_sw = (m->conv_tc && !convp_ffma) ? m->get("df_dec.df_convp.w_sw") : nullptr;
-        if (w_sw) {
-            if ((rc = launch_df_convp_tc(sl, f.c0, w_sw, w2, bb, d_coefs, B, T, Fd))) return rc;
-        } else {
-            DFB_PROF("k_df_convp", sl);
-            const int smem = kCpWarps * kCpSlots * (512 + 8);
-            k_df_convp<5, 5, 3><<<grid, 32 * kCpWarps, smem, sl>>>(f.c0, w1, w2, bb, d_coefs, T, Fd);
-            DFB_LAUNCH_CHECK();
-        }
+        DFB_PROF("k_df_convp", sl);
+        const int smem = kCpWarps * kCpSlots * (512 + 8);
+        k_df_convp<5, 5, 3><<<grid, 32 * kCpWarps, smem, sl>>>(f.c0, w1, w2, bb, d_coefs, T, Fd);
+        DFB_LAUNCH_CHECK();
         DFB_CUDA(cudaEventRecord(L.ev_convp, sl));
     }
     {
@@ -1697,7 +1712,7 @@
     if (B <= 0 || T <= 0) return DFB_OK;
     if (B > 65535) return fail(DFB_ERR_INVALID, "more than 65535 streams per call");
     size_t extra = ((size_t)M * m->cfg.nb_erb + (size_t)M * m->cfg.nb_df * O2 + (size_t)M) * 4 + 8192;
-    int rc = m->arena.reserve(fwd_plan(m->cfg, (size_t)M, nullptr, nullptr) + extra);
+    int rc = m->arena.reserve(fwd_plan(m, (size_t)M, nullptr, nullptr) + extra);
     if (rc) return rc;
     m->arena.reset();
     float *mm = d_m ? d_m : m->arena.take<float>((size_t)M * m->cfg.nb_erb);
@@ -1784,10 +1799,11 @@
     return DFB_OK;
 }
 
-static size_t chunk_bytes_per_stream(const dfb_model_config &c, const dfb_state *st, int Tw) {
+static size_t chunk_bytes_per_stream(const dfb_model *m, const dfb_state *st, int Tw) {
+    const dfb_model_config &c = m->cfg;
     const ChunkGeom g = chunk_geom(c);
     const int E = c.nb_erb, Fd = c.nb_df, O2 = 2 * c.df_order, F = st->tb.F;
-    return (size_t)(Tw + g.Lmax) * (2 * F + E + 2 * Fd) * 4 + (size_t)Tw * (E + (size_t)Fd * O2 + 2) * 4 + fwd_plan(c, (size_t)Tw, nullptr, nullptr) +
+    return (size_t)(Tw + g.Lmax) * (2 * F + E + 2 * Fd) * 4 + (size_t)Tw * (E + (size_t)Fd * O2 + 2) * 4 + fwd_plan(m, (size_t)Tw, nullptr, nullptr) +
            16384;
 }
 
@@ -1895,7 +1911,7 @@
 }
 
 static int pick_chunk(const dfb_model *m, const dfb_state *st, int64_t B, int64_t Tf, int min_chunks, size_t cap) {
-    const size_t per_frame = chunk_bytes_per_stream(m->cfg, st, 1024) / 1024 + 1;
+    const size_t per_frame = chunk_bytes_per_stream(m, st, 1024) / 1024 + 1;
     const ChunkGeom g = chunk_geom(m->cfg);
     int64_t tw = (int64_t)(cap / ((size_t)B * per_frame)) - g.Lmax - 8;
     int64_t tc = tw - kHalo;
@@ -1982,7 +1998,7 @@
     }
     *group_out = group; *tc_out = tc; *pipelined_out = pipelined && tc < Tf;
     const ChunkGeom g = chunk_geom(m->cfg);
-    const size_t bytes = chunk_bytes_per_stream(m->cfg, st, tc + kHalo) * (size_t)group + ((size_t)g.Lmax << 10) + (2 << 20);
+    const size_t bytes = chunk_bytes_per_stream(m, st, tc + kHalo) * (size_t)group + ((size_t)g.Lmax << 10) + (2 << 20);
     int rc = m->arena.reserve(bytes);
     if (!rc && *pipelined_out) rc = m->arena1.reserve(bytes);
     return rc;
@@ -2253,7 +2269,7 @@
     if (e1n < S.e1) e1n = S.e1;
     const int64_t W0 = S.d1 > kHalo ? S.d1 - kHalo : 0;
     const int Tw = (int)(d1n - W0);
-    int rc = m->arena.reserve(chunk_bytes_per_stream(m->cfg, st, Tw + 1) * (size_t)B + (2 << 20));
+    int rc = m->arena.reserve(chunk_bytes_per_stream(m, st, Tw + 1) * (size_t)B + (2 << 20));
     if (rc) return rc;
     const int64_t f0 = (flush ? S.a1 : a0) - Ltot;
     if (f0 < 0 || e1n <= S.e1) DFB_CUDA(cudaMemsetAsync(d_out, 0, sizeof(float) * B * n_out * hop, s));
diff --git a/deepfilternet_b200/csrc/dfb_tc.cu b/deepfilternet_b200/csrc/dfb_tc.cu
--- a/deepfilternet_b200/csrc/dfb_tc.cu
+++ b/deepfilternet_b200/csrc/dfb_tc.cu
@@ -319,79 +319,163 @@
 template int launch_dwpw_tc<DW_S2>(cudaStream_t, DwPwParams, const float *, int);
 template int launch_dwpw_tc<DW_T2>(cudaStream_t, DwPwParams, const float *, int);
 
-constexpr int kCvThreads = 256, kCvOut = 124, kCvYld = 51 , kCvBins = 8;
-constexpr uint32_t kCvW = 32768, kCvRawOff = 49152, kCvYs = kCvRawOff + 32768, kCvTail = kCvYs + 128 * kCvYld * 4;
-
-struct CvParams {
-    const float *w_sw;
-    const float *w2;
-    const float *bias;
-    float *coefs;
-    int T, Fd;
-};
-
-template <int ORDER, int KTP>
-__global__ void __launch_bounds__(kCvThreads, 2) k_df_convp_tc(const __grid_constant__ CUtensorMap tmC0, CvParams p) {
-    constexpr int O2 = 2 * ORDER, NY = KTP * ORDER;
+constexpr int kFrJ = 4, kFrOut = 124, kFrKtp = 5, kFrOrder = 5;
+constexpr int kFrFld = 2 * (2 * kFrJ + 3);
+constexpr uint32_t kFrP1 = 32768, kFrWc = 65536, kFrWp = 81920, kFrW0 = 98304, kFrX = kFrW0 + 18 * 256,
+                   kFrW2 = kFrX + 130 * kFrFld * 4, kFrBar = kFrW2 + 448, kFrSmem = kFrBar + 16;
+
+template <int NR>
+__device__ __forceinline__ void front_conv0(float4 (&c)[NR], const float *s_x, const float *s_w0, float4 bias, int rb, int lf,
+                                            int cq, int kt0) {
+#pragma unroll
+    for (int i = 0; i < NR; i++) c[i] = bias;
+#pragma unroll
+    for (int dt = 0; dt < 3; dt++) {
+        if (dt < kt0) continue;
+#pragma unroll
+        for (int k = 0; k < 3; k++) {
+            const float4 wr = *reinterpret_cast<const float4 *>(s_w0 + ((dt - kt0) * 6 + 2 * k) * kCh + cq * 4);
+            const float4 wi = *reinterpret_cast<const float4 *>(s_w0 + ((dt - kt0) * 6 + 2 * k + 1) * kCh + cq * 4);
+#pragma unroll
+            for (int i = 0; i < NR; i++) {
+                const int r = i == 0 ? max(rb, 0) : rb + i;
+                const float2 x = *reinterpret_cast<const float2 *>(s_x + (r + dt) * kFrFld + 2 * (lf + k));
+                c[i] = f4_fma(make_float4(x.x, x.x, x.x, x.x), wr, c[i]);
+                c[i] = f4_fma(make_float4(x.y, x.y, x.y, x.y), wi, c[i]);
+            }
+        }
+    }
+#pragma unroll
+    for (int i = 0; i < NR; i++)
+        c[i] = make_float4(fmaxf(c[i].x, 0.f), fmaxf(c[i].y, 0.f), fmaxf(c[i].z, 0.f), fmaxf(c[i].w, 0.f));
+}
+
+__device__ __forceinline__ void front_planes(uint32_t base, int r, int cq, float4 v) {
+    uint32_t h0, l0, h1, l1;
+    bf16x2_split(v.x, v.y, h0, l0);
+    bf16x2_split(v.z, v.w, h1, l1);
+    const uint32_t off = base + sw128_off(r, cq >> 1) + (cq & 1) * 8;
+    sts64(off, h0, h1);
+    sts64(off + 16384, l0, l1);
+}
+
+template <int KT, int PART>
+__global__ void __launch_bounds__(256, 2) k_df_front(FrontParams p) {
+    constexpr bool C1 = PART == FRONT_C1, CV = PART == FRONT_CONVP;
+    constexpr int NR = C1 ? 8 + KT - 1 : 8, NY = kFrKtp * kFrOrder, O2 = 2 * kFrOrder;
     extern __shared__ __align__(1024) unsigned char tc_smem_raw[];
-    const uint32_t sb = (smem_u32(tc_smem_raw) + 1023u) & ~1023u;
+    const uint32_t sb = smem_u32(tc_smem_raw);
+    if (sb & 1023u) __trap();
+    float *s_x = reinterpret_cast<float *>(tc_smem_raw + kFrX);
+    const float *s_w0 = reinterpret_cast<const float *>(tc_smem_raw + kFrW0);
+    const uint32_t s_w2 = sb + kFrW2, bar_w = sb + kFrBar;
     const int tid = threadIdx.x, warp = tid >> 5, lane = tid & 31;
-    const int f_begin = blockIdx.x * kCvBins, f_end = min(f_begin + kCvBins, p.Fd);
-    const int b = blockIdx.z, t0 = blockIdx.y * kCvOut, r0 = t0 - (KTP - 1);
-    const uint32_t s_w2 = sb + kCvTail, bar_raw = s_w2 + 512, bar_w = bar_raw + 16;
-    const int row = b * p.T + r0;
-    auto load_bin = [&](int f) {
-        mbar_expect_tx_a(bar_raw, 32768);
-        asm volatile("cp.async.bulk.tensor.2d.shared::cluster.global.mbarrier::complete_tx::bytes [%0], [%1, {%2, %3}], [%4];"
-                     ::"r"(sb + kCvRawOff), "l"((uint64_t)&tmC0), "r"(f * 64), "r"(row), "r"(bar_raw) : "memory");
-        asm volatile("cp.async.bulk.tensor.2d.shared::cluster.global.mbarrier::complete_tx::bytes [%0], [%1, {%2, %3}], [%4];"
-                     ::"r"(sb + kCvRawOff + 16384), "l"((uint64_t)&tmC0), "r"(f * 64 + 32), "r"(row), "r"(bar_raw) : "memory");
-    };
+    const int j0 = blockIdx.x * kFrJ, b = blockIdx.z, r0 = blockIdx.y * kFrOut - (kFrKtp - 1);
+    const int Fh = p.Fd / 2;
     if (tid == 0) {
-        mbar_init_a(bar_raw, 1);
         mbar_init_a(bar_w, 1);
         fence_barrier_init();
         mbar_expect_tx_a(bar_w, 16384);
-        bulk_load(sb + kCvW, p.w_sw, 16384, bar_w);
-        load_bin(f_begin);
-    }
-    for (int i = tid; i < O2 * O2 + O2; i += kCvThreads)
-        asm volatile("st.shared.f32 [%0], %1;" ::"r"(s_w2 + 4 * i), "f"(i < O2 * O2 ? __ldg(p.w2 + i) : __ldg(p.bias + i - O2 * O2)) : "memory");
+        if (CV) bulk_load(sb + kFrWc, p.cv_sw, 16384, bar_w);
+        else bulk_load(sb + kFrWp, p.pw_sw, 16384, bar_w);
+    }
+    const int kt0 = 3 - p.inp_kt;
+    for (int i = tid; i < p.inp_kt * 6 * (kCh / 4); i += 256) sts128(sb + kFrW0 + 16 * i, __ldg(reinterpret_cast<const float4 *>(p.w0) + i));
+    if (CV)
+        for (int i = tid; i < O2 * O2 + O2; i += 256)
+            asm volatile("st.shared.f32 [%0], %1;" ::"r"(s_w2 + 4 * i), "f"(i < O2 * O2 ? __ldg(p.cv_w2 + i) : __ldg(p.cv_b + i - O2 * O2)) : "memory");
+    {
+        const int Tx = p.rows ? min(p.Tx, (int)(p.rows[b].Tf - p.W0)) : p.Tx;
+        for (int i = tid; i < 130 * kFrFld; i += 256) {
+            const int row = i / kFrFld, k = i - row * kFrFld;
+            const int f = 2 * j0 - 2 + (k >> 1), tp = r0 - 2 + row;
+            float v = 0.f;
+            if (f >= 0 && f < p.Fd && tp >= 0 && tp + p.lookahead < Tx)
+                v = __ldg(p.x + (((int64_t)b * p.Tsx + tp + p.lookahead) * p.Fd + f) * 2 + (k & 1));
+            s_x[i] = v;
+        }
+    }
+    const int cq = tid & 15, slot = tid >> 4;
+    const int ta = r0 + 8 * slot;
+    const float4 bias0 = __ldg(reinterpret_cast<const float4 *>(p.b0) + cq);
+    auto wd = [&](int dt, int df) { return __ldg(reinterpret_cast<const float4 *>(p.dw + (dt * 3 + df) * kCh) + cq); };
+    const float4 zero4 = make_float4(0.f, 0.f, 0.f, 0.f);
+    float4 acc[8];
+#pragma unroll
+    for (int i = 0; i < 8; i++) acc[i] = zero4;
     __syncthreads();
     mbar_wait_a(bar_w, 0);
-    const int r = tid & 127, half = tid >> 7;
-    const bool zero = r0 + r < 0;
-    for (int f = f_begin, it = 0; f < f_end; f++, it++) {
-        const uint32_t par = (uint32_t)(it & 1);
-        mbar_wait_a(bar_raw, par);
-        {
-            const uint32_t src = sb + kCvRawOff + (uint32_t)half * 16384u + (uint32_t)r * 128u;
-            float4 xs[8];
-#pragma unroll
-            for (int c = 0; c < 8; c++) xs[c] = lds128(src + (uint32_t)((c ^ (r & 7)) << 4));
-#pragma unroll
-            for (int c = 0; c < 8; c++) {
-                float4 x = xs[c];
-                if (zero) x = make_float4(0.f, 0.f, 0.f, 0.f);
-                uint32_t h0, l0, h1, l1;
-                bf16x2_split(x.x, x.y, h0, l0);
-                bf16x2_split(x.z, x.w, h1, l1);
-                const int cq = half * 8 + c;
-                const uint32_t off = sb + sw128_off(r, cq >> 1) + (cq & 1) * 8;
-                sts64(off, h0, h1);
-                sts64(off + 16384, l0, l1);
-            }
-        }
-        fence_proxy_async();
+    for (int lf = 0; lf <= 2 * kFrJ; lf++) {
+        const int f = 2 * j0 - 1 + lf;
+        if (f < 0 || (!C1 && lf == 0)) continue;
+        const bool fin = C1 && lf > 0 && !(lf & 1), open = C1 && !(lf & 1) && lf < 2 * kFrJ;
+        float4 c[NR];
+        front_conv0<NR>(c, s_x, s_w0, bias0, 8 * slot - (NR - 8), lf, cq, kt0);
+#pragma unroll
+        for (int i = 0; i < NR; i++)
+            if (ta - (NR - 8) + i < 0) c[i] = zero4;
+        if (C1 && lf > 0) {
+            const float4 w = wd(0, (lf & 1) ? 1 : 2);
+#pragma unroll
+            for (int i = 0; i < 8; i++)
+                if (KT == 1 || ta + i - 1 >= 0) acc[i] = f4_fma(c[i], w, acc[i]);
+        }
+        if (C1 && KT == 2 && fin) {
+#pragma unroll
+            for (int h = 0; h < 2; h++) {
+                float4 e[4];
+                if (f > 1) {
+                    front_conv0<4>(e, s_x, s_w0, bias0, 8 * slot + 4 * h, lf - 2, cq, kt0);
+                    const float4 w = wd(1, 0);
+#pragma unroll
+                    for (int i = 0; i < 4; i++) acc[4 * h + i] = f4_fma(e[i], w, acc[4 * h + i]);
+                }
+                front_conv0<4>(e, s_x, s_w0, bias0, 8 * slot + 4 * h, lf - 1, cq, kt0);
+                const float4 w1 = wd(1, 1), w2 = wd(1, 2);
+#pragma unroll
+                for (int i = 0; i < 4; i++) acc[4 * h + i] = f4_fma(c[4 * h + i + 1], w2, f4_fma(e[i], w1, acc[4 * h + i]));
+            }
+        }
+        if ((CV && lf > 0) || fin) __syncthreads();
+#pragma unroll
+        for (int i = 0; i < 8; i++) {
+            if (CV && lf > 0) front_planes(sb, 8 * slot + i, cq, c[i + NR - 8]);
+            if (fin) front_planes(sb + kFrP1, 8 * slot + i, cq, acc[i]);
+            if (open) acc[i] = (KT == 1 || ta + i - 1 >= 0) ? f4_fma(c[i], wd(0, 0), zero4) : zero4;
+        }
+        if (!(CV && lf > 0) && !fin) continue;
         __syncthreads();
-        if (tid == 0 && f + 1 < f_end) load_bin(f + 1);
-        {
-            float acc[1][8][4];
+        if (fin) {
+            float a1[1][8][4];
 #pragma unroll
             for (int nt = 0; nt < 8; nt++)
 #pragma unroll
-                for (int c = 0; c < 4; c++) acc[0][nt][c] = 0.f;
-            warp_mma_sw128_k64<1>(sb, sb + 16384, sb + kCvW, sb + kCvW + 8192, warp * 16, 0, acc);
+                for (int e = 0; e < 4; e++) a1[0][nt][e] = 0.f;
+            warp_mma_sw128_k64<1>(sb + kFrP1, sb + kFrP1 + 16384, sb + kFrWp, sb + kFrWp + 8192, warp * 16, 0, a1);
+            __syncwarp();
+#pragma unroll
+            for (int nt = 0; nt < 8; nt++) {
+                const int n = 8 * nt + 2 * (lane & 3);
+                const float b0 = __ldg(p.b1 + n), b1 = __ldg(p.b1 + n + 1);
+#pragma unroll
+                for (int h = 0; h < 2; h++) {
+                    const int rr = warp * 16 + (lane >> 2) + 8 * h;
+                    uint32_t hi, lo;
+                    bf16x2_split(fmaxf(a1[0][nt][2 * h] + b0, 0.f), fmaxf(a1[0][nt][2 * h + 1] + b1, 0.f), hi, lo);
+                    const uint32_t off = sb + kFrP1 + sw128_off(rr, n >> 3) + (n & 7) * 2;
+                    asm volatile("st.shared.b32 [%0], %1;" ::"r"(off), "r"(hi) : "memory");
+                    asm volatile("st.shared.b32 [%0], %1;" ::"r"(off + 16384), "r"(lo) : "memory");
+                }
+            }
+        }
+        if (CV) {
+            float ay[1][8][4];
+#pragma unroll
+            for (int nt = 0; nt < 8; nt++)
+#pragma unroll
+                for (int e = 0; e < 4; e++) ay[0][nt][e] = 0.f;
+            warp_mma_sw128_k64<1>(sb, sb + 16384, sb + kFrWc, sb + kFrWc + 8192, warp * 16, 0, ay);
+            __syncwarp();
 #pragma unroll
             for (int nt = 0; nt < 8; nt++)
 #pragma unroll
@@ -399,26 +483,28 @@
                     const int n = 8 * nt + 2 * (lane & 3) + (e & 1), g = n >> 5, j = n & 31;
                     const int rr = warp * 16 + (lane >> 2) + 8 * (e >> 1);
                     if (j < NY)
-                        asm volatile("st.shared.f32 [%0], %1;" ::"r"(sb + kCvYs + (uint32_t)(rr * kCvYld + g * NY + j) * 4u), "f"(acc[0][nt][e]) : "memory");
+                        asm volatile("st.shared.f32 [%0], %1;" ::"r"(sb + (uint32_t)(g * 16384 + rr * 128 + (((j + rr) & 31) << 2))),
+                                     "f"(ay[0][nt][e]) : "memory");
                 }
         }
         __syncthreads();
-        if (tid < 128) {
+        if (CV && tid < 128) {
             const int t = r0 + tid;
-            if (tid >= KTP - 1 && tid < KTP - 1 + kCvOut && t < p.T) {
+            if (tid >= kFrKtp - 1 && t < p.T) {
                 float z[O2];
 #pragma unroll
                 for (int g = 0; g < 2; g++)
 #pragma unroll
-                    for (int o = 0; o < ORDER; o++) {
+                    for (int o = 0; o < kFrOrder; o++) {
                         float a = 0.f;
 #pragma unroll
-                        for (int dt = 0; dt < KTP; dt++) {
+                        for (int dt = 0; dt < kFrKtp; dt++) {
+                            const int rr = tid - (kFrKtp - 1) + dt, j = dt * kFrOrder + o;
                             float y;
-                            asm volatile("ld.shared.f32 %0, [%1];" : "=f"(y) : "r"(sb + kCvYs + (uint32_t)((tid - (KTP - 1) + dt) * kCvYld + g * NY + dt * ORDER + o) * 4u));
+                            asm volatile("ld.shared.f32 %0, [%1];" : "=f"(y) : "r"(sb + (uint32_t)(g * 16384 + rr * 128 + (((j + rr) & 31) << 2))));
                             a += y;
                         }
-                        z[g * ORDER + o] = a;
+                        z[g * kFrOrder + o] = a;
                     }
                 float outv[O2];
 #pragma unroll
@@ -437,8 +523,41 @@
 #pragma unroll
                 for (int qo = 0; qo < O2; qo += 2) *reinterpret_cast<float2 *>(dst + qo) = make_float2(outv[qo], outv[qo + 1]);
             }
-        }
-    }
+        } else if (fin) {
+            const int j = (f - 1) / 2;
+            for (int q = tid; q < 128 * 16; q += 256) {
+                const int r = q >> 4, pl = (q >> 3) & 1, ck = q & 7, t = r0 + r;
+                if (r < kFrKtp - 1 || t >= p.T) continue;
+                const float4 v = lds128(sb + kFrP1 + (uint32_t)pl * 16384u + sw128_off(r, ck));
+                unsigned short *dst = (pl ? p.c1_lo : p.c1_hi) + (((int64_t)b * p.T + t) * Fh + j) * kCh + ck * 8;
+                *reinterpret_cast<float4 *>(dst) = v;
+            }
+        }
+    }
+}
+
+int launch_df_front(cudaStream_t s, const FrontParams &p, int B, int conv_kt, int part) {
+    if (p.Fd % (2 * kFrJ) || p.inp_kt < 1 || p.inp_kt > 3 || (conv_kt != 1 && conv_kt != 2) || (part != FRONT_C1 && part != FRONT_CONVP))
+        return fail(DFB_ERR_UNSUPPORTED, "df front kernel: nb_df %d, input conv kt %d, conv kt %d", p.Fd, p.inp_kt, conv_kt);
+    if (B > 65535) return fail(DFB_ERR_UNSUPPORTED, "df front kernel: more than 65535 streams");
+    static PerDeviceOnce attr_once;
+    if (auto once_guard = attr_once.first()) {
+        DFB_CUDA(cudaFuncSetAttribute(k_df_front<1, FRONT_C1>, cudaFuncAttributeMaxDynamicSharedMemorySize, (int)kFrSmem));
+        DFB_CUDA(cudaFuncSetAttribute(k_df_front<2, FRONT_C1>, cudaFuncAttributeMaxDynamicSharedMemorySize, (int)kFrSmem));
+        DFB_CUDA(cudaFuncSetAttribute(k_df_front<1, FRONT_CONVP>, cudaFuncAttributeMaxDynamicSharedMemorySize, (int)kFrSmem));
+    }
+    dim3 grid((unsigned)(p.Fd / (2 * kFrJ)), (unsigned)((p.T + kFrOut - 1) / kFrOut), (unsigned)B);
+    if (part == FRONT_CONVP) {
+        DFB_PROF("k_df_convp_tc", s);
+        k_df_front<1, FRONT_CONVP><<<grid, 256, kFrSmem, s>>>(p);
+        DFB_LAUNCH_CHECK();
+        return DFB_OK;
+    }
+    DFB_PROF("k_dwpw_df_front", s);
+    if (conv_kt == 1) k_df_front<1, FRONT_C1><<<grid, 256, kFrSmem, s>>>(p);
+    else k_df_front<2, FRONT_C1><<<grid, 256, kFrSmem, s>>>(p);
+    DFB_LAUNCH_CHECK();
+    return DFB_OK;
 }
 
 namespace cg = cooperative_groups;
@@ -769,26 +888,6 @@
     return use32 ? launch_gru_tc_n<32, 256, 0>(s, p) : launch_gru_tc_n<16, 256, 0>(s, p);
 }
 
-int cached_map_f32_sw128(CUtensorMap *out, const void *base, int64_t rows, int64_t cols, int64_t ld, int box_rows);
-
-int launch_df_convp_tc(cudaStream_t s, const float *c0, const float *w_sw, const float *w2, const float *bias, float *coefs, int B, int T,
-                       int Fd) {
-    if ((int64_t)B * T >= (int64_t(1) << 31) - 256 || B > 65535) return fail(DFB_ERR_UNSUPPORTED, "df pathway conv: batch too large for one launch");
-    CUtensorMap mc;
-    int rc;
-    if ((rc = cached_map_f32_sw128(&mc, c0, (int64_t)B * T, (int64_t)Fd * kCh, (int64_t)Fd * kCh, 128))) return rc;
-    const int smem = 1024 + (int)kCvTail + 512 + 64;
-    static PerDeviceOnce attr_once;
-    if (auto once_guard = attr_once.first())
-        DFB_CUDA(cudaFuncSetAttribute(k_df_convp_tc<5, 5>, cudaFuncAttributeMaxDynamicSharedMemorySize, smem));
-    CvParams p{w_sw, w2, bias, coefs, T, Fd};
-    dim3 grid((unsigned)((Fd + kCvBins - 1) / kCvBins), (unsigned)((T + kCvOut - 1) / kCvOut), (unsigned)B);
-    DFB_PROF("k_df_convp_tc", s);
-    k_df_convp_tc<5, 5><<<grid, kCvThreads, smem, s>>>(mc, p);
-    DFB_LAUNCH_CHECK();
-    return DFB_OK;
-}
-
 int cached_map_bf16(CUtensorMap *out, const void *base, int64_t rows, int64_t cols, int64_t ld, int box_rows);
 
 int launch_gemm_bf16x3(cudaStream_t s, const void *x_hi, const void *x_lo, int64_t ldx, const void *w_hi, const void *w_lo,
```

Result: no change. 51670, median of 6 (+0.7%).
